# zixunh/vipe

Hardware: AMD Instinct MI355X
Metric: dense-BA+flow update iters/s, 512x384 48-KF graph (higher is better)
Workload: dtype f16 (correlation, GRU; fp32 accumulate) + f32 geometry/BA (fp64 reduced system)

## Files before the change

include/vipe_amd.h:

```cpp
#ifndef VIPE_AMD_H
#define VIPE_AMD_H

#include <stdint.h>

#ifdef __cplusplus
extern "C" {
#endif

#define VIPE_F16 0
#define VIPE_F32 1
#define VIPE_F64 2
#define VIPE_U8 3

#define VIPE_OK 0
#define VIPE_EINVAL (-1)
#define VIPE_ENOSPACE (-2)
#define VIPE_EUNSUPPORTED (-3)

#define VIPE_PYRAMID_REFERENCE 0
#define VIPE_PYRAMID_BLOCKED 1

#define VIPE_CAM_PINHOLE 0
#define VIPE_CAM_MEI 1

// ... 80 lines not shown
int vipe_lie_adjT_backward(int group_id, const void* grad, const void* X, const void* a, void* dX, void* da,
                           int64_t n, int dtype, int on_device, void* stream);
int vipe_lie_act_backward(int group_id, const void* grad, const void* X, const void* p, void* dX, void* dp,
                          int64_t n, int dtype, int on_device, void* stream);
int vipe_lie_act4_backward(int group_id, const void* grad, const void* X, const void* p, void* dX, void* dp,
                           int64_t n, int dtype, int on_device, void* stream);


int vipe_reproject(const float* d_poses, const float* d_disps, const float* d_intrinsics, const float* d_rig,
                   const int64_t* d_pi, const int64_t* d_qi, const int64_t* d_pj, const int64_t* d_qj,
                   const int64_t* d_di, float* d_coords, float* d_valid, int M, int ht, int wd, int n_views,
                   int camera, float intr_factor, void* stream);

int vipe_reproject_motion(const float* d_poses, const float* d_disps, const float* d_intrinsics, const float* d_rig,
                          const int64_t* d_pi, const int64_t* d_qi, const int64_t* d_pj, const int64_t* d_qj,
                          const int64_t* d_di, const float* d_target, float* d_coords, void* d_motn, int M, int ht,
                          int wd, int n_views, int camera, float intr_factor, int motn_dtype, void* stream);
int vipe_reproject_motion_nhwc(const float* d_poses, const float* d_disps, const float* d_intrinsics,
                               const float* d_rig, const int64_t* d_pi, const int64_t* d_qi, const int64_t* d_pj,
                               const int64_t* d_qj, const int64_t* d_di, const float* d_target, float* d_coords,
                               void* d_motn, int M, int ht, int wd, int n_views, int camera, float intr_factor,
                               void* stream);

typedef int (*vipe_overlap_fn)(void* user, int piece, int n_pieces, void* stream);

typedef struct {
  int n_poses;
  int n_views;
  int ht, wd;
  int M;
  int t0, t1;
  int n_iters;
  float pose_damping, pose_ep;
  int motion_only;
  int limited_disp;
  int optimize_intrinsics;
  int optimize_rig_rotation;
  int camera;
  float alpha;
  float weight_scale;
  float intr_factor;
  int reuse_plan;
  int path_hint;
  void* overlap_stream;
  vipe_overlap_fn overlap_fn;
  void* overlap_user;
  int solver_options;
  void* profile_ev0;
  void* profile_ev1;
  int profile_iter;
} vipe_ba_params;
#define VIPE_BA_OPT_ONE_CHAIN 1
#define VIPE_BA_OPT_GENERAL_ACCUMULATE 2

int64_t vipe_dense_ba_workspace_bytes(const vipe_ba_params* p);
int vipe_dense_ba(const vipe_ba_params* p, float* d_poses, float* d_disps, const float* d_disps_sens,
                  float* d_intrinsics, float* d_rig, const float* d_target, const float* d_weight,
                  const float* d_disp_damping, const int64_t* d_pi, const int64_t* d_qi, const int64_t* d_pj,
                  const int64_t* d_qj, const int64_t* d_di, void* d_workspace, int64_t workspace_bytes,
                  int* d_info, void* stream);

int vipe_dense_ba_linearize(const vipe_ba_params* p, const float* d_poses, const float* d_disps, const float* d_disps_sens,
                            const float* d_intrinsics, const float* d_rig, const float* d_target, const float* d_weight,
                            const float* d_disp_damping, const int64_t* d_pi, const int64_t* d_qi, const int64_t* d_pj,
                            const int64_t* d_qj, const int64_t* d_di, void* d_workspace, int64_t workspace_bytes,
                            double* d_S_out, int ld_out, int* d_info, void* stream);
int vipe_dense_ba_marginals(const vipe_ba_params* p, void* d_workspace, const double* d_Sinv, int ld, float* d_disp_var,
                            double* d_pose_cov, void* stream);

int64_t vipe_ba_workspace_bytes(int n_poses, int ht, int wd, int E);
int vipe_ba(float* d_poses, float* d_disps, const float* d_intrinsics, const float* d_disps_sens,
            const float* d_targets, const float* d_weights, const float* d_eta, const int64_t* d_ii,
            const int64_t* d_jj, int n_poses, int ht, int wd, int E, int n_eta, int t0, int t1, int iterations,
            float lm, float ep, int motion_only, float* d_dx, float* d_dz, void* d_workspace,
            int64_t workspace_bytes, void* stream);

int vipe_frame_distance(const float* d_poses, const float* d_disps, const float* d_intrinsics, const int64_t* d_pi,
                        const int64_t* d_pj, const int64_t* d_qi, const int64_t* d_qj, const int64_t* d_di,
                        float* d_dist, int M, int ht, int wd, float beta, void* stream);

int vipe_frame_distance_rig(const float* d_poses, const float* d_rig, const float* d_disps, const float* d_intrinsics,
                            int intr_dim, float intr_factor, const int64_t* d_pi, const int64_t* d_qi, const int64_t* d_pj,
                            const int64_t* d_qj, float* d_dist, int M, int n_views, int ht, int wd, float beta,
                            int bidirectional, void* stream);

int vipe_depth_filter(const float* d_poses, const float* d_disps, const float* d_intrinsics, const int64_t* d_inds,
                      const float* d_thresh, float* d_counter, int n, int num, int ht, int wd, void* stream);

int vipe_projmap(const float* d_poses, const float* d_disps, const float* d_intrinsics, const int64_t* d_ii,
                 const int64_t* d_jj, float* d_coords, float* d_valid, int E, int ht, int wd, void* stream);

int vipe_iproj(const float* d_poses, const float* d_disps, const float* d_intrinsics, float* d_points, int n, int ht,
               int wd, void* stream);

int vipe_scatter(const void* d_src, const int64_t* d_index, void* d_out, int64_t* d_arg_out, int64_t outer,
                 int64_t src_dim, int64_t inner, int64_t out_dim, int reduce, int dtype, void* stream);
int vipe_scatter_rows(const void* d_src, const int64_t* d_index, void* d_out, int64_t* d_arg_out, int64_t outer,
                      int64_t src_dim, int64_t inner, int64_t out_dim, int reduce, int dtype, void* stream);

int vipe_scatter_host(const void* h_src, const int64_t* h_index, void* h_out, int64_t* h_arg_out, int64_t outer,
                      int64_t src_dim, int64_t inner, int64_t out_dim, int reduce, int dtype);

int vipe_scatter_mean_rows_f16(const void* d_src, const int64_t* d_ix, void* d_out, int E, int n_out, int64_t inner,
                               void* stream);

int vipe_segment_mean_nhwc_f16(const void* d_src, int src_ctot, int src_coff, const int* d_order, const int* d_rowptr,
// ... 25 lines not shown
                                 void* d_grad_value, void* d_grad_sampling_loc, void* d_grad_attn_weight, int64_t bs,
                                 int64_t Lv, int heads, int C, int L, int64_t Lq, int P, int dtype, void* stream);

#define VIPE_ACT_NONE 0
#define VIPE_ACT_RELU 1
#define VIPE_ACT_SIGMOID 2
#define VIPE_ACT_TANH 3
int vipe_conv_pack_weights(const void* d_w_oihw, void* d_w_packed, int Cout, int Cin, int KH, int KW, int src_dtype,
                           void* stream);
int vipe_conv2d_nhwc_f16(const void* d_x, const void* d_w_packed, const float* d_bias, const float* d_extra,
                         void* d_y, int B, int H, int W, int Cin, int cin_total, int cin_off, int Cout,
                         int cout_total, int cout_off, int KH, int KW, int act, void* stream);

int vipe_conv_packed_dims(int Cout, int Cin, int KH, int KW, int* cout_pad, int* cin_pad, int* k_pad);

#define VIPE_CONV_PARTIAL 6
#define VIPE_CONV_ACCINIT_F32 0x100
int vipe_conv2d_fused(const void* d_x0, int x0_ctot, int x0_coff, const void* d_x1, int x1_ctot, int x1_coff,
                      int split, const void* d_w_packed, const float* d_bias, const float* d_extra, int extra_stride,
                      int extra_off, void* d_y, int y_ctot, int y_coff, void* d_y2, int y2_ctot, int y2_coff,
                      const void* d_net, int net_ctot, int net_coff, const void* d_z, float* d_fout,
                      const void* d_accinit, int ai_ctot, int ai_coff, int B, int H, int W, int Cin, int Cout, int KH,
                      int KW, int act, int mode, void* stream);

typedef struct {
  const void *corr0_w, *corr2_w, *flow0_w, *flow2_w, *gw_w, *zr_w, *q_w, *zr_s_w, *q_s_w, *heads0_w, *heads2_w, *agg2_w, *eta_w;
  const void *zr_n_w, *zr_x_w;
  const float *corr0_b, *corr2_b, *flow0_b, *flow2_b, *gw_b, *zr_b, *q_b, *heads0_b, *heads2_b, *agg2_b, *eta_b;
  const float* glo_wT;
  const float* glo_b;
} vipe_update_weights;
typedef struct {
  int E, H, W, n_src;
  const void* levels[4];
  const float* coords;
  const int* slots;
  int h2, w2, pyramid_layout;
  const void* corr;
  const void* motn;
  const void* net;
  void* net_out;
  void* xbuf;
  const void* pgate;
  void *c1, *f1, *zb, *rnet;
  void* hbuf;
  float* dw;
  float *glo, *extra;
  const int *order, *rowptr;
  void *agg, *a2;
  float* eta;
  void* side_stream;
  float* pzr;
  int gate_state;
} vipe_update_buffers;
int vipe_update_operator(const vipe_update_weights* weights, const vipe_update_buffers* buffers, void* stream);

int vipe_update_gate_state(const vipe_update_weights* weights, const vipe_update_buffers* buffers, const void* d_net,
                           int parts, void* stream);
typedef struct {
  const vipe_update_weights* weights;
  const vipe_update_buffers* buffers;
  const void* net;
  const int* bounds;
  int n_bounds;
} vipe_gate_state_job;
int vipe_update_gate_state_piece(void* user, int piece, int n_pieces, void* stream);

int vipe_glo_context(const float* d_glo_sum, const float* d_wT, const float* d_bias, float* d_extra, int E, int hw,
                     void* stream);

typedef struct {
  const void* src;
  void* dst;
  const int64_t* idx;
  int64_t src_row_pitch, dst_row_pitch;
  int64_t seg_bytes, seg_pitch;
  int n_seg;
  int n_rows;
  int dst_row0;
} vipe_rows_job;
int vipe_rows_gather(const vipe_rows_job* jobs, int n_jobs, void* stream);
typedef struct {
  const void* src;
  const int64_t* frame;
  void* dst;
  int64_t dst_row_pitch;
  int dst_ctot, dst_coff;
  int dst_row0;
} vipe_nhwc_job;
int vipe_gather_nchw_to_nhwc_f16(const vipe_nhwc_job* jobs, int n_jobs, int n_rows, int C, int P, void* stream);

int vipe_flow_score(const float* d_dw, const unsigned char* d_invalid, float* d_score, int n_views, int P, void* stream);

int vipe_update_finish(const float* d_coords1, const float* d_dw, const unsigned char* d_mask, float* d_target,
                       float* d_weight, const float* d_eta, const int64_t* d_du, float* d_damping, int E, int n_src, int ht,
                       int wd, void* stream);

int vipe_enc_prep(const float* d_img, void* d_x4, int V, int H, int W, void* stream);
int vipe_enc_stem(const void* d_x4, const void* d_w, const float* d_bias, void* d_y, float* d_out_stats, int B, int H,
                  int W, int relu, void* stream);
int vipe_enc_conv(const void* d_x, const float* d_in_stats, const void* d_w, const float* d_bias, const void* d_res,
                  void* d_y, float* d_out_stats, int B, int H, int W, int Cin, int Cout, int ksize, int stride,
                  int relu, int nchw, int tanh_split, void* stream);
int vipe_enc_finish(const void* d_raw, const float* d_raw_stats, const void* d_res, const float* d_res_stats,
                    void* d_out, int B, int HW, int C, void* stream);

// ... 12 lines not shown
```

vipe_amd/csrc/ba.hip:

```cpp
#include <stdlib.h>

#include "term_geom.cuh"

namespace {

#include "ba_common.cuh"
#include "ba_plan.inc"
#include "ba_accumulate.inc"
#include "ba_solve_band.inc"
#include "ba_solve_dense.inc"
#include "ba_solve_global.inc"
#include "ba_retract.inc"
#include "ba_marginals.inc"

hipEvent_t overlap_event() {
  static thread_local hipEvent_t ev[64] = {};
  int d = 0;
  (void)hipGetDevice(&d);
  hipEvent_t& e = ev[d & 63];
  if (!e && hipEventCreateWithFlags(&e, hipEventDisableTiming) != hipSuccess) e = nullptr;
  return e;
}

int overlap_piece(const vipe_ba_params& p, hipEvent_t ev, int piece, int n_pieces, bool gated) {
// ... 2 lines not shown
  return p.overlap_fn(p.overlap_user, piece, n_pieces, p.overlap_stream);
}

template <int CAM, int F>
void launch_accumulate(const BAArgs& a, hipStream_t s) {
  const int tiles = (a.P + TILE - 1) / TILE;
  static std::atomic<uint64_t> tmpl_set{0};
  vipe_once_per_device(tmpl_set, [] {
    (void)hipFuncSetAttribute((const void*)ba_accum_mfma_kernel<CAM, F>, hipFuncAttributeMaxDynamicSharedMemorySize, (int)accum_mfma_lds());
    (void)hipFuncSetAttribute((const void*)ba_walk_kernel<CAM, F>, hipFuncAttributeMaxDynamicSharedMemorySize, (int)walk_lds());
    (void)hipFuncSetAttribute((const void*)ba_walk_rig_kernel<CAM, 4>, hipFuncAttributeMaxDynamicSharedMemorySize, (int)walk_rig_lds());
    (void)hipFuncSetAttribute((const void*)ba_walk_rig_kernel<CAM, RG_VMAX>, hipFuncAttributeMaxDynamicSharedMemorySize, (int)walk_rig_lds());
  });
  if (a.mv) {
    if (a.p.n_views <= 4) ba_walk_rig_kernel<CAM, 4><<<dim3(tiles, a.nF), TILE, walk_rig_lds(), s>>>(a);
    else ba_walk_rig_kernel<CAM, RG_VMAX><<<dim3(tiles, a.nF), TILE, walk_rig_lds(), s>>>(a);
    ba_schur_kernel<0><<<dim3(SC_GRID, a.nF), TILE, 0, s>>>(a);
    return;
  }
  const int hint = a.force_general ? 0 : a.p.path_hint;
  if (!(hint & 2)) ba_accum_mfma_kernel<CAM, F><<<dim3(tiles, a.nF), TILE, accum_mfma_lds(), s>>>(a);
  if (!(hint & 1)) {
    ba_walk_kernel<CAM, F><<<dim3(tiles, a.nF), TILE, walk_lds(), s>>>(a);
    ba_schur_kernel<F><<<dim3(SC_GRID, a.nF), TILE, 0, s>>>(a);
  }
}

template <int CAM, int F>
int run_iters(const BAArgs& a, hipStream_t s, int* pieces_done) {
  const int tiles = (a.P + TILE - 1) / TILE;
  const size_t sbytes = sizeof(double) * (size_t)a.w.ld * a.w.ld;
  const size_t nmax = (size_t)a.w.ld - 1;
  const size_t fixed = ((sizeof(SolveLds) + 15) / 16) * 16;
  int panel_cap = (int)std::min<size_t>(nmax + 1, (150 * 1024 - fixed) / (NB * sizeof(double)));
  panel_cap = (panel_cap + 3) & ~3;
  const size_t solve_lds = fixed + (size_t)NB * panel_cap * sizeof(double);
  const size_t band_lds = 158 * 1024;
  static std::atomic<uint64_t> attr_set{0};
  vipe_once_per_device(attr_set, [] {
    (void)hipFuncSetAttribute((const void*)ba_solve_band_kernel, hipFuncAttributeMaxDynamicSharedMemorySize, 160 * 1024);
    (void)hipFuncSetAttribute((const void*)ba_solve_kernel, hipFuncAttributeMaxDynamicSharedMemorySize, 160 * 1024);
    (void)hipFuncSetAttribute((const void*)ba_solve_dense_kernel, hipFuncAttributeMaxDynamicSharedMemorySize, 160 * 1024);
    (void)hipFuncSetAttribute((const void*)chol_backsub_kernel, hipFuncAttributeMaxDynamicSharedMemorySize, 64 * 1024);
  });
  const bool retract_clears = !a.p.motion_only;
  const bool overlap = a.p.overlap_stream && a.p.overlap_fn;
  hipEvent_t ev = overlap ? overlap_event() : nullptr;
  for (int it = 0; it < a.p.n_iters; ++it) {
    if (!(retract_clears && (it > 0 || a.p.reuse_plan))) {
      hipError_t e1 = hipMemsetAsync(a.w.S, 0, sbytes, s);
      hipError_t e2 = hipMemsetAsync(a.w.Hd, 0, sizeof(double) * nmax, s);
      if (e1 != hipSuccess || e2 != hipSuccess) return (int)(e1 != hipSuccess ? e1 : e2);
    }
    if (a.mv) {
      launch_accumulate<CAM, F>(a, s);
      if (ev && hipEventRecord(ev, s) != hipSuccess) return VIPE_EINVAL;
      ba_solve_kernel<<<1, SOLVE_T, solve_lds, s>>>(a, panel_cap);
      launch_tiled_cholesky(a, s);
      if (overlap) {
        const int rc = overlap_piece(a.p, ev, it, a.p.n_iters, true);
        if (rc != VIPE_OK) return rc;
        ++*pieces_done;
      }
      if (!a.p.motion_only) ba_retract_kernel<0><<<dim3(tiles, a.nF), TILE, 0, s>>>(a);
      continue;
    }
    const int hint = a.force_general ? 0 : a.p.path_hint;
    const bool prof = a.p.profile_ev0 && a.p.profile_ev1 &&
                      it == (a.p.profile_iter < 0 || a.p.profile_iter >= a.p.n_iters ? a.p.n_iters - 1 : a.p.profile_iter);
    if (prof && hipEventRecord((hipEvent_t)a.p.profile_ev0, s) != hipSuccess) return VIPE_EINVAL;
    launch_accumulate<CAM, F>(a, s);
    if (prof && hipEventRecord((hipEvent_t)a.p.profile_ev1, s) != hipSuccess) return VIPE_EINVAL;
    if (ev && hipEventRecord(ev, s) != hipSuccess) return VIPE_EINVAL;
    if (!(hint & 8)) ba_solve_band_kernel<<<1, 2 * BAND_T, band_lds, s>>>(a, (int)(band_lds / sizeof(double)));
    if (!(hint & 16)) ba_solve_dense_kernel<<<1, DN_T, band_lds, s>>>(a, (int)(band_lds / sizeof(double)));
    if (!(hint & 4)) {
      ba_solve_kernel<<<1, SOLVE_T, solve_lds, s>>>(a, panel_cap);
      launch_tiled_cholesky(a, s);
    }
    if (overlap) {
      const int rc = overlap_piece(a.p, ev, it, a.p.n_iters, true);
      if (rc != VIPE_OK) return rc;
      ++*pieces_done;
    }
    if (!a.p.motion_only) ba_retract_kernel<F><<<dim3(tiles, a.nF), TILE, 0, s>>>(a);
  }
  return vipe_launch_status();
}

BAArgs live_args(const vipe_ba_params& p) {
  BAArgs a = {};
  a.p = p;
  a.P = p.ht * p.wd;
  a.nF = p.n_poses * p.n_views;
  a.D = p.camera == VIPE_CAM_MEI ? 1 : 0;
  a.mv = is_multiview(p) ? 1 : 0;
  a.nintr = tail_intr(p);
  a.ntail = a.nintr + tail_rig(p);
  a.force_general = (p.solver_options & VIPE_BA_OPT_GENERAL_ACCUMULATE) != 0;
  a.band2 = !(p.solver_options & VIPE_BA_OPT_ONE_CHAIN);
  a.droid = 0;
  a.dz_out = nullptr;
  return a;
}

}

VIPE_EXPORT int64_t vipe_dense_ba_workspace_bytes(const vipe_ba_params* p) {
  if (!p || p->n_poses <= 0 || p->n_views <= 0 || p->ht <= 0 || p->wd <= 0 || p->M < 0) return VIPE_EINVAL;
  return (int64_t)carve(*p, nullptr, nullptr);
}

VIPE_EXPORT int vipe_dense_ba(const vipe_ba_params* p, float* d_poses, float* d_disps, const float* d_disps_sens,
                              float* d_intrinsics, float* d_rig, const float* d_target, const float* d_weight,
                              const float* d_disp_damping, const int64_t* d_pi, const int64_t* d_qi,
                              const int64_t* d_pj, const int64_t* d_qj, const int64_t* d_di, void* d_workspace,
                              int64_t workspace_bytes, int* d_info, void* stream) {
  VIPE_CHECK_ARG(p && d_poses && d_disps && d_disps_sens && d_intrinsics && d_rig && d_disp_damping && d_workspace);
  VIPE_CHECK_ARG(p->n_poses > 0 && p->n_views > 0 && p->ht > 0 && p->wd > 0 && p->M >= 0 && p->n_iters >= 0);
  VIPE_CHECK_ARG(p->t0 <= p->t1 && p->intr_factor > 0);
  VIPE_CHECK_ARG(p->camera == VIPE_CAM_PINHOLE || p->camera == VIPE_CAM_MEI);
  VIPE_CHECK_ARG(p->M == 0 || (d_target && d_weight && d_pi && d_qi && d_pj && d_qj && d_di));
  if (is_multiview(*p) && p->n_views > RG_VMAX) return VIPE_EUNSUPPORTED;
  if ((int64_t)p->n_poses * p->n_views > 65535) return VIPE_EINVAL;
  BAArgs a = live_args(*p);
  if ((int64_t)carve(*p, (char*)d_workspace, &a.w) > workspace_bytes) return VIPE_ENOSPACE;
  a.poses = d_poses; a.disps = d_disps; a.intr = d_intrinsics; a.rig = d_rig;
  a.sens = d_disps_sens; a.target = d_target; a.weight = d_weight; a.eta = d_disp_damping;
  a.pi = d_pi; a.qi = d_qi; a.pj = d_pj; a.qj = d_qj; a.di = d_di;
  hipStream_t s = as_stream(stream);
  int rc = VIPE_OK, pieces_done = 0;
  if (p->M > 0 && p->n_iters > 0) {
    ba_sens_kernel<<<a.nF, 256, 0, s>>>(d_disps_sens, a.w.sens_sum, a.P, a.w.info);
    if (!p->reuse_plan) ba_plan_kernel<<<1, 1024, 0, s>>>(a);
    const int F = p->optimize_intrinsics ? 1 + a.D : 0;
    if (p->camera == VIPE_CAM_PINHOLE) rc = F ? run_iters<VIPE_CAM_PINHOLE, 1>(a, s, &pieces_done) : run_iters<VIPE_CAM_PINHOLE, 0>(a, s, &pieces_done);
    else rc = F ? run_iters<VIPE_CAM_MEI, 2>(a, s, &pieces_done) : run_iters<VIPE_CAM_MEI, 0>(a, s, &pieces_done);
    if (rc != VIPE_OK) return rc;
    if (d_info) {
      hipError_t e = hipMemcpyAsync(d_info, a.w.info, 8 * sizeof(int), hipMemcpyDeviceToDevice, s);
      if (e != hipSuccess) return (int)e;
    }
  }
  if (p->overlap_stream && p->overlap_fn) {
    const int n_pieces = p->n_iters > 0 ? p->n_iters : 1;
    for (; pieces_done < n_pieces; ++pieces_done) {
      rc = overlap_piece(*p, nullptr, pieces_done, n_pieces, false);
      if (rc != VIPE_OK) return rc;
    }
  }
  const int64_t nd = (int64_t)a.nF * a.P;
  clamp_min_kernel<<<(int)std::min<int64_t>((nd + 255) / 256, 2048), 256, 0, s>>>(d_disps, nd, 1e-3f);
  return vipe_launch_status();
}

VIPE_EXPORT int vipe_dense_ba_linearize(const vipe_ba_params* p, const float* d_poses, const float* d_disps,
                                        const float* d_disps_sens, const float* d_intrinsics, const float* d_rig,
                                        const float* d_target, const float* d_weight, const float* d_disp_damping,
                                        const int64_t* d_pi, const int64_t* d_qi, const int64_t* d_pj, const int64_t* d_qj,
                                        const int64_t* d_di, void* d_workspace, int64_t workspace_bytes, double* d_S_out,
                                        int ld_out, int* d_info, void* stream) {
  VIPE_CHECK_ARG(p && d_poses && d_disps && d_disps_sens && d_intrinsics && d_rig && d_disp_damping && d_workspace && d_S_out);
  VIPE_CHECK_ARG(p->n_poses > 0 && p->n_views > 0 && p->ht > 0 && p->wd > 0 && p->M >= 0);
  VIPE_CHECK_ARG(p->t0 <= p->t1 && p->intr_factor > 0);
  VIPE_CHECK_ARG(p->camera == VIPE_CAM_PINHOLE || p->camera == VIPE_CAM_MEI);
  VIPE_CHECK_ARG(p->M == 0 || (d_target && d_weight && d_pi && d_qi && d_pj && d_qj && d_di));
  if (is_multiview(*p) && p->n_views > RG_VMAX) return VIPE_EUNSUPPORTED;
  if ((int64_t)p->n_poses * p->n_views > 65535) return VIPE_EINVAL;
  BAArgs a = live_args(*p);
  if ((int64_t)carve(*p, (char*)d_workspace, &a.w) > workspace_bytes) return VIPE_ENOSPACE;
  VIPE_CHECK_ARG(ld_out >= 6 * p->n_poses + a.ntail);
  a.poses = const_cast<float*>(d_poses); a.disps = const_cast<float*>(d_disps);
  a.intr = const_cast<float*>(d_intrinsics); a.rig = const_cast<float*>(d_rig);
  a.sens = d_disps_sens; a.target = d_target; a.weight = d_weight; a.eta = d_disp_damping;
  a.pi = d_pi; a.qi = d_qi; a.pj = d_pj; a.qj = d_qj; a.di = d_di;
  hipStream_t s = as_stream(stream);
  ba_sens_kernel<<<a.nF, 256, 0, s>>>(d_disps_sens, a.w.sens_sum, a.P, a.w.info);
  if (!(p->reuse_plan && p->M > 0)) ba_plan_kernel<<<1, 1024, 0, s>>>(a);
  if (!(p->reuse_plan && !p->motion_only && p->M > 0)) {
    hipError_t e1 = hipMemsetAsync(a.w.S, 0, sizeof(double) * (size_t)a.w.ld * a.w.ld, s);
    hipError_t e2 = hipMemsetAsync(a.w.Hd, 0, sizeof(double) * ((size_t)a.w.ld - 1), s);
    if (e1 != hipSuccess || e2 != hipSuccess) return (int)(e1 != hipSuccess ? e1 : e2);
  }
  if (p->M > 0) {
    ba_term_slot_kernel<<<(p->M + 255) / 256, 256, 0, s>>>(a);
    const int F = p->optimize_intrinsics ? 1 + a.D : 0;
    if (p->camera == VIPE_CAM_PINHOLE) F ? launch_accumulate<VIPE_CAM_PINHOLE, 1>(a, s) : launch_accumulate<VIPE_CAM_PINHOLE, 0>(a, s);
    else F ? launch_accumulate<VIPE_CAM_MEI, 2>(a, s) : launch_accumulate<VIPE_CAM_MEI, 0>(a, s);
  }
  const int64_t nn = (int64_t)(a.w.ld - 1) * (a.w.ld - 1);
  ba_export_reduced_kernel<<<(int)std::min<int64_t>((nn + 255) / 256, 2048), 256, 0, s>>>(a, d_S_out, ld_out);
  if (d_info) {
    hipError_t e = hipMemcpyAsync(d_info, a.w.info, 8 * sizeof(int), hipMemcpyDeviceToDevice, s);
    if (e != hipSuccess) return (int)e;
  }
  return vipe_launch_status();
}

VIPE_EXPORT int vipe_dense_ba_marginals(const vipe_ba_params* p, void* d_workspace, const double* d_Sinv, int ld,
                                        float* d_disp_var, double* d_pose_cov, void* stream) {
  VIPE_CHECK_ARG(p && d_workspace);
  VIPE_CHECK_ARG(p->n_poses > 0 && p->n_views > 0 && p->ht > 0 && p->wd > 0 && p->M >= 0 && ld >= 0);
  VIPE_CHECK_ARG(p->camera == VIPE_CAM_PINHOLE || p->camera == VIPE_CAM_MEI);
  if (is_multiview(*p) && p->n_views > RG_VMAX) return VIPE_EUNSUPPORTED;
  if ((int64_t)p->n_poses * p->n_views > 65535) return VIPE_EINVAL;
  BAArgs a = live_args(*p);
  carve(*p, (char*)d_workspace, &a.w);
  hipStream_t s = as_stream(stream);
  const int tiles = (a.P + TILE - 1) / TILE;
  if (p->M > 0 && !p->motion_only && d_disp_var) {
    VIPE_CHECK_ARG(d_Sinv || ld == 0);
    ba_disp_variance_kernel<<<dim3(tiles, a.nF), TILE, 0, s>>>(a, d_Sinv, ld, d_disp_var);
  }
  const int64_t ns = (int64_t)a.w.ld * a.w.ld;
  ba_marginals_finish_kernel<<<(int)std::min<int64_t>((ns + 255) / 256, 2048), 256, 0, s>>>(a, ld > 0 ? d_Sinv : nullptr, ld, d_pose_cov);
  return vipe_launch_status();
}

namespace {
size_t droid_extra_bytes(int E) { return align_up(8 * (size_t)(E + 1)) + align_up(7 * 4); }
vipe_ba_params droid_params(int n_poses, int ht, int wd, int E, int t0, int t1, int iterations, float lm, float ep,
                            int motion_only) {
  vipe_ba_params p = {};
  p.n_poses = n_poses; p.n_views = 1; p.ht = ht; p.wd = wd; p.M = E; p.t0 = t0; p.t1 = t1; p.n_iters = iterations;
  p.pose_damping = lm; p.pose_ep = ep; p.motion_only = motion_only; p.limited_disp = 0; p.optimize_intrinsics = 0;
  p.optimize_rig_rotation = 0; p.camera = VIPE_CAM_PINHOLE; p.alpha = 0.05f; p.weight_scale = 0.001f; p.intr_factor = 1.0f;
  p.reuse_plan = 0; p.path_hint = 0;
  return p;
}
}

VIPE_EXPORT int64_t vipe_ba_workspace_bytes(int n_poses, int ht, int wd, int E) {
  if (n_poses <= 0 || ht <= 0 || wd <= 0 || E < 0) return VIPE_EINVAL;
  const vipe_ba_params p = droid_params(n_poses, ht, wd, E, 0, 0, 0, 0.f, 0.f, 0);
  return (int64_t)(carve(p, nullptr, nullptr) + droid_extra_bytes(E));
}

VIPE_EXPORT int vipe_ba(float* d_poses, float* d_disps, const float* d_intrinsics, const float* d_disps_sens,
                        const float* d_targets, const float* d_weights, const float* d_eta, const int64_t* d_ii,
                        const int64_t* d_jj, int n_poses, int ht, int wd, int E, int n_eta, int t0, int t1,
                        int iterations, float lm, float ep, int motion_only, float* d_dx, float* d_dz,
                        void* d_workspace, int64_t workspace_bytes, void* stream) {
  VIPE_CHECK_ARG(d_poses && d_disps && d_intrinsics && d_disps_sens && d_eta && d_workspace && d_dx && d_dz);
  VIPE_CHECK_ARG(n_poses > 0 && ht > 0 && wd > 0 && E >= 0 && iterations >= 0 && n_eta >= 0);
  VIPE_CHECK_ARG(0 <= t0 && t0 <= t1 && t1 <= n_poses);
  VIPE_CHECK_ARG(E == 0 || (d_targets && d_weights && d_ii && d_jj));
  if (n_poses > 65535) return VIPE_EINVAL;
  BAArgs a;
  a.p = droid_params(n_poses, ht, wd, E, t0, t1, iterations, lm, ep, motion_only);
  const size_t base = carve(a.p, (char*)d_workspace, &a.w);
  if ((int64_t)(base + droid_extra_bytes(E)) > workspace_bytes) return VIPE_ENOSPACE;
  int64_t* zeros = (int64_t*)((char*)d_workspace + base);
  float* rig = (float*)((char*)d_workspace + base + align_up(8 * (size_t)(E + 1)));
  hipStream_t s = as_stream(stream);
  const float rig_id[7] = {0, 0, 0, 0, 0, 0, 1};
  hipError_t e0 = hipMemsetAsync(zeros, 0, 8 * (size_t)(E + 1), s);
  hipError_t e1 = hipMemcpyAsync(rig, rig_id, sizeof(rig_id), hipMemcpyHostToDevice, s);
  const int64_t P = (int64_t)ht * wd;
  hipError_t e2 = hipMemsetAsync(d_dx, 0, sizeof(float) * 6 * (size_t)(t1 - t0), s);
  hipError_t e3 = hipMemsetAsync(d_dz, 0, sizeof(float) * (size_t)n_eta * P, s);
  if (e0 != hipSuccess || e1 != hipSuccess || e2 != hipSuccess || e3 != hipSuccess) return VIPE_EINVAL;
  a.poses = d_poses; a.disps = d_disps; a.intr = (float*)d_intrinsics; a.rig = rig;
  a.sens = d_disps_sens; a.target = d_targets; a.weight = d_weights; a.eta = d_eta;
  a.pi = d_ii; a.qi = zeros; a.pj = d_jj; a.qj = zeros; a.di = d_ii;
  a.P = ht * wd; a.nF = n_poses; a.D = 0;
  a.mv = 0; a.nintr = 0; a.ntail = 0;
  a.force_general = 0;
  a.band2 = 1;
  a.droid = 1;
  a.dz_out = d_dz;
  if (iterations == 0 || t1 == t0) return VIPE_OK;
  ba_sens_kernel<<<a.nF, 256, 0, s>>>(d_disps_sens, a.w.sens_sum, a.P, a.w.info);
  ba_plan_kernel<<<1, 1024, 0, s>>>(a);
  int pieces_done = 0;
  const int rc = run_iters<VIPE_CAM_PINHOLE, 0>(a, s, &pieces_done);
  if (rc != VIPE_OK) return rc;
  hipError_t e4 = hipMemcpyAsync(d_dx, a.w.dx, sizeof(float) * 6 * (size_t)(t1 - t0), hipMemcpyDeviceToDevice, s);
  return e4 == hipSuccess ? vipe_launch_status() : (int)e4;
}
```

vipe_amd/csrc/ba_accumulate.inc:

```
constexpr int AM_ROWS = 48;
constexpr int AM_P1 = 130;
constexpr int AM_P2 = 66;
constexpr int AM_P2H = 34;
constexpr int AM_WBUF = 16 * AM_P1;
static_assert(AM_ROWS * AM_P2H <= AM_WBUF, "R2 half image must fit the wave buffer");
constexpr int AM_SP = AM_ROWS + 1;

struct TermGeomM {
  TermGeom g;
  float Mi[36];
};

constexpr size_t accum_mfma_lds() {
  return sizeof(float) * (NWAVE * AM_WBUF + AM_ROWS * AM_SP + AM_DMAX * 256 + 64) + AM_DMAX * sizeof(TermGeomM);
}

typedef float float4m __attribute__((ext_vector_type(4)));


__device__ __forceinline__ void term_setup_m(const BAArgs& a, int e, TermGeomM& m) {
  TermGeom& g = m.g;
  term_setup(a, e, g);
#pragma unroll
  for (int c = 0; c < 6; ++c) {
// ... 221 lines not shown
        atomicAdd(&accI[42 + q * FF + f], hif);
      }
    } else if (F > 0 && lane < 42 + 6 * F + F * F) {
      const int i2 = lane - 42 - 6 * F, f = i2 / FF, f2 = i2 % FF;
      if (f >= f2) atomicAdd(&accI[42 + 6 * FF + f * FF + f2], Gm[(7 + f) * 16 + 7 + f2]);
    } else if (F > 0 && lane < 42 + 6 * F + F * F + F) {
      const int f = lane - 42 - 6 * F - F * F;
      atomicAdd(&accI[42 + 6 * FF + FF * FF + f], -Gm[(7 + f) * 16 + 6]);
    }
    __builtin_amdgcn_fence(__ATOMIC_RELEASE, "wavefront");
    __builtin_amdgcn_wave_barrier();
    if (fi && lane < 36) {
      const int r = lane / 6, c = lane % 6;
      float hii = 0.f;
#pragma unroll
      for (int q = 0; q < 6; ++q) hii += T1[r * 8 + q] * Mi[c * 6 + q];
      atomicAdd(&accI[r * 6 + c], hii);
    }
    __builtin_amdgcn_wave_barrier();
  }
}

template <int F>
__device__ __forceinline__ void flush_frame_blocks(const BAWs& w, const float* accI, int si, int nrow, int foff) {
  constexpr int FF = F > 0 ? F : 1;
  const int tid = threadIdx.x;
  const bool fi = si >= 0;
  const int bi = 6 * si;
  if (tid < 36) {
    const int r = tid / 6, c = tid % 6;
    if (fi && r >= c) {
      const double s = (double)accI[r * 6 + c];
      s_add(w, bi + r, bi + c, s);
      if (r == c) atomicAdd(&w.Hd[bi + r], s);
    }
  } else if (tid < 42) {
    if (fi) atomicAdd(&w.S[(int64_t)nrow * w.ld + bi + (tid - 36)], (double)accI[tid]);
  } else if (F > 0 && tid < 42 + 6 * F) {
    const int q = (tid - 42) / FF, f = (tid - 42) % FF;
    if (fi) s_add(w, foff + f, bi + q, (double)accI[tid]);
  } else if (F > 0 && tid < 42 + 6 * F + F * F) {
    const int i2 = tid - 42 - 6 * F, f = i2 / FF, f2 = i2 % FF;
    if (f >= f2) {
      const double s = (double)accI[tid];
      s_add(w, foff + f, foff + f2, s);
      if (f == f2) atomicAdd(&w.Hd[foff + f], s);
    }
  } else if (F > 0 && tid < 42 + 6 * F + F * F + F) {
    atomicAdd(&w.S[(int64_t)nrow * w.ld + foff + (tid - 42 - 6 * F - F * F)], (double)accI[tid]);
  }
}

template <int NF, int F>
__device__ __forceinline__ void store_disp_block(const BAArgs& a, int k, int flags, WalkPixel<F>& px) {
  static_assert(NF <= WalkPixel<F>::FF, "E_f rows come from px.Efr");
  const BAWs& w = a.w;
  const int P = a.P, p = px.p;
  const int64_t kp = (int64_t)k * P + p;
  finish_disp(a, k, p, P, flags, px.d, px.C, px.wz);
  if (px.inb) {
    w.C[kp] = px.C;
    w.wv[kp] = px.wz;
#pragma unroll
    for (int q = 0; q < 6; ++q) w.Ekk[((int64_t)k * 6 + q) * P + p] = px.Ei[q];
#pragma unroll
    for (int f = 0; f < NF; ++f) w.Ef[((int64_t)k * 2 + f) * P + p] = px.Efr[f];
  }
}

template <int CAM, int F>
__global__ __launch_bounds__(TILE) __attribute__((amdgpu_waves_per_eu(3, 3))) void ba_accum_mfma_kernel(BAArgs a) {
  const vipe_ba_params& prm = a.p;
  const BAWs& w = a.w;
  if (a.force_general || w.info[6] > AM_DMAX) return;
  const int k = blockIdx.y;
  const int beg = w.rowptr[k], end = w.rowptr[k + 1];
  if (beg == end) return;
  const int deg = end - beg;
  const int P = a.P, V = prm.n_views, tid = threadIdx.x, lane = tid & 63, wave = tid >> 6;
  const int flags = w.fflags[k];
  const bool dfree = flags & 2;
  const int pose_i = k / V, qi = k % V;
  const int si = w.pose_slot[pose_i];
  const bool fi = si >= 0;
  const int n_free = w.info[0], nrow = w.info[3];
  const int foff = 6 * n_free;

  extern __shared__ __align__(16) float am_smem[];
  float* wbuf = am_smem + wave * AM_WBUF;
  float* accS = am_smem + NWAVE * AM_WBUF;
  float* acc1 = accS + AM_ROWS * AM_SP;
  float* accI = acc1 + AM_DMAX * 256;
  TermGeomM* tg = reinterpret_cast<TermGeomM*>(accI + 64);

  for (int i = tid; i < AM_ROWS * AM_SP + AM_DMAX * 256 + 64; i += TILE) accS[i] = 0.0f;
  if (tid < deg) {
    TermGeomM m;
    term_setup_m(a, w.order[beg + tid], m);
    tg[tid] = m;
  }
  __syncthreads();

  WalkPixel<F> px = walk_pixel<CAM, F>(a, k, qi);
  const int l16 = lane & 15, kq = lane >> 4;
  walk_tile<CAM, F>(a, tg, deg, dfree, wbuf, acc1, px);

  const int NR = 6 * (deg + 1) + F + 1;
  if (dfree) {
    store_disp_block<F>(a, k, flags, px);
    const float sq = px.inb ? __builtin_amdgcn_rsqf(px.C) : 0.0f;
    float ej[AM_DMAX][6];
#pragma unroll
    for (int t = 0; t < AM_DMAX; ++t) {
      const bool on = t < deg && tg[min(t, deg - 1)].g.sj >= 0 && px.inb;
      const int64_t eb = (int64_t)tg[min(t, deg - 1)].g.e * 6 * P + px.p;
#pragma unroll
      for (int q = 0; q < 6; ++q) ej[t][q] = on ? w.Ej[eb + (int64_t)q * P] : 0.0f;
    }
    constexpr int NPAIR = 6;
    float4m g4[NPAIR];
#pragma unroll
    for (int i = 0; i < NPAIR; ++i) g4[i] = float4m{0.f, 0.f, 0.f, 0.f};
    const int RT = (NR + 15) >> 4;
#pragma unroll
    for (int half = 0; half < 2; ++half) {
      if ((lane >> 5) == half) {
        float* col = wbuf + (lane & 31);
#pragma unroll
        for (int q = 0; q < 6; ++q) col[q * AM_P2H] = fi ? px.Ei[q] * sq : 0.0f;
#pragma unroll
        for (int t = 0; t < AM_DMAX; ++t) {
          if (t < deg) {
#pragma unroll
            for (int q = 0; q < 6; ++q) col[(6 * (t + 1) + q) * AM_P2H] = ej[t][q] * sq;
          }
        }
        if constexpr (F > 0) {
#pragma unroll
          for (int f = 0; f < F; ++f) col[(6 * (deg + 1) + f) * AM_P2H] = px.Efr[f] * sq;
        }
        col[(NR - 1) * AM_P2H] = px.wz * sq;
        for (int r = NR; r < ((NR + 15) & ~15); ++r) col[r * AM_P2H] = 0.0f;
      }
      __builtin_amdgcn_fence(__ATOMIC_RELEASE, "wavefront");
      __builtin_amdgcn_wave_barrier();
#pragma unroll
      for (int ta = 0; ta < 3; ++ta)
#pragma unroll
        for (int tb = 0; tb <= ta; ++tb) {
          if (ta < RT) {
            const float* ar = wbuf + (16 * ta + l16) * AM_P2H + kq;
            const float* br = wbuf + (16 * tb + l16) * AM_P2H + kq;
            float4m acc = g4[ta * (ta + 1) / 2 + tb];
#pragma unroll
            for (int s = 0; s < 8; ++s) acc = __builtin_amdgcn_mfma_f32_16x16x4f32(ar[4 * s], br[4 * s], acc, 0, 0, 0);
            g4[ta * (ta + 1) / 2 + tb] = acc;
          }
        }
      __builtin_amdgcn_fence(__ATOMIC_RELEASE, "wavefront");
      __builtin_amdgcn_wave_barrier();
    }
#pragma unroll
    for (int ta = 0; ta < 3; ++ta)
#pragma unroll
      for (int tb = 0; tb <= ta; ++tb) {
        if (ta < RT) {
#pragma unroll
          for (int r = 0; r < 4; ++r) {
            const int row = 16 * ta + 4 * kq + r, cc = 16 * tb + l16;
            if (row < NR && cc <= row) atomicAdd(&accS[row * AM_SP + cc], g4[ta * (ta + 1) / 2 + tb][r]);
          }
        }
      }
  }
  __syncthreads();

  flush_term_blocks<F>(w, tg, deg, acc1, accI, wbuf, si, nrow, foff);
  __syncthreads();

  flush_frame_blocks<F>(w, accI, si, nrow, foff);
  if (dfree) {
    auto gmap = [&](int row) -> int {
      if (row >= 6 * (deg + 1)) return foff + (row - 6 * (deg + 1));
      const int m = row / 6, q = row % 6;
      const int sl = m == 0 ? si : tg[m - 1].g.sj;
      return sl >= 0 ? 6 * sl + q : -1;
    };
    for (int i = tid; i < NR * NR; i += TILE) {
      const int row = i / NR, cc = i % NR;
      if (cc > row || cc == NR - 1) continue;
      const int gc = gmap(cc);
      if (gc < 0) continue;
      const float val = accS[row * AM_SP + cc];
      if (row == NR - 1) {
        atomicAdd(&w.S[(int64_t)nrow * w.ld + gc], -(double)val);
      } else {
        const int gr = gmap(row);
        if (gr >= 0) s_add(w, gr, gc, (gr == gc && row != cc) ? -2.0 * (double)val : -(double)val);
      }
    }
  }
}

constexpr int WK_CH = 8;
constexpr int WK_CH1 = 12;
constexpr size_t walk_lds() {
  return sizeof(float) * (NWAVE * 16 * AM_P1 + WK_CH1 * 256 + 64) + WK_CH1 * sizeof(TermGeomM);
}

template <int CAM, int F>
__global__ __launch_bounds__(TILE) void ba_walk_kernel(BAArgs a) {
  constexpr int WBUF = 16 * AM_P1;
  const vipe_ba_params& prm = a.p;
  const BAWs& w = a.w;
  if (!a.force_general && w.info[6] <= AM_DMAX) return;
  const int k = blockIdx.y;
  const int beg = w.rowptr[k], end = w.rowptr[k + 1];
  if (beg == end) return;
  const int deg_all = end - beg;
  const int V = prm.n_views, tid = threadIdx.x, wave = tid >> 6;
  const int flags = w.fflags[k];
  const bool dfree = flags & 2;
  const int pose_i = k / V, qi = k % V;
  const int si = w.pose_slot[pose_i];
  const int n_free = w.info[0], nrow = w.info[3];
  const int foff = 6 * n_free;

  extern __shared__ __align__(16) float am_smem[];
  float* wbuf = am_smem + wave * WBUF;
  float* acc1 = am_smem + NWAVE * WBUF;
  float* accI = acc1 + WK_CH1 * 256;
  TermGeomM* tg = reinterpret_cast<TermGeomM*>(accI + 64);
  if (tid < 64) accI[tid] = 0.0f;

  WalkPixel<F> px = walk_pixel<CAM, F>(a, k, qi);

  for (int cb = 0; cb < deg_all; cb += WK_CH1) {
    const int deg = min(WK_CH1, deg_all - cb);
    __syncthreads();
    for (int i = tid; i < WK_CH1 * 256; i += TILE) acc1[i] = 0.0f;
    if (tid < deg) {
      TermGeomM m;
      term_setup_m(a, w.order[beg + cb + tid], m);
      tg[tid] = m;
    }
    __syncthreads();

    walk_tile<CAM, F>(a, tg, deg, dfree, wbuf, acc1, px);

    __syncthreads();
    flush_term_blocks<F>(w, tg, deg, acc1, accI, wbuf, si, nrow, foff);

  }
  __syncthreads();

  flush_frame_blocks<F>(w, accI, si, nrow, foff);
  if (dfree) store_disp_block<F>(a, k, flags, px);
}

constexpr int RG_NB = 10;
constexpr int RG_NL = 28;
struct TermGeomR {
  TermGeom g;
  int qj, same_view;
  int gcol[RG_NL];
  float Lm[RG_NL][RG_NB];
};
constexpr size_t walk_rig_lds() {
  return sizeof(float) * (NWAVE * 16 * AM_P1 + WK_CH * 256) + WK_CH * sizeof(TermGeomR);
}
__device__ __forceinline__ int rg_tile_row(int b) { return b < 6 ? b : b + 1; }

template <int CAM, int VM>
__global__ __launch_bounds__(TILE) void ba_walk_rig_kernel(BAArgs a) {
  constexpr int WBUF = 16 * AM_P1;
  constexpr int F = CAM == VIPE_CAM_MEI ? 2 : 1;
  const vipe_ba_params& prm = a.p;
  const BAWs& w = a.w;
  const int k = blockIdx.y;
  const int beg = w.rowptr[k], end = w.rowptr[k + 1];
  if (beg == end) return;
  const int deg_all = end - beg;
  const int P = a.P, V = prm.n_views, tid = threadIdx.x, lane = tid & 63, wave = tid >> 6;
  const int flags = w.fflags[k];
  const bool dfree = flags & 2;
  const int pose_i = k / V, qi = k % V;
  const int si = w.pose_slot[pose_i];
  const int n_free = w.info[0], nrow = w.info[3];
  const int foff = 6 * n_free, roff = foff + a.nintr;
  const bool oi = prm.optimize_intrinsics, orr = prm.optimize_rig_rotation;

  extern __shared__ __align__(16) float am_smem[];
  float* wbuf = am_smem + wave * WBUF;
  float* acc1 = am_smem + NWAVE * WBUF;
  TermGeomR* tg = reinterpret_cast<TermGeomR*>(acc1 + WK_CH * 256);

  WalkPixel<F> px = walk_pixel<CAM, F>(a, k, qi);
  const int p = px.p;
  const bool inb = px.inb;
  float ErA[6] = {0, 0, 0, 0, 0, 0};
  float Efv[VM][F] = {}, Erv[VM][6] = {};
  const int l16 = lane & 15, kq = lane >> 4;

  for (int cb = 0; cb < deg_all; cb += WK_CH) {
    const int deg = min(WK_CH, deg_all - cb);
    __syncthreads();
    for (int i = tid; i < WK_CH * 256; i += TILE) acc1[i] = 0.0f;
    if (tid < deg) {
      TermGeomR& m = tg[tid];
      const int e = w.order[beg + cb + tid];
      const int pi = (int)a.pi[e], pj = (int)a.pj[e], qj = (int)a.qj[e];
      term_transforms(a.poses, a.rig, pi, qi, pj, qj, m.g.T, m.g.G, m.g.Rr);
      m.g.Ij = cam::load_scaled(a.intr + qj * (4 + a.D), a.D, 1.0f / prm.intr_factor);
      m.g.e = e;
      m.g.merge = (pi == pj);
      m.g.rig_adj = !(m.g.Rr.t[0] == 0.f && m.g.Rr.t[1] == 0.f && m.g.Rr.t[2] == 0.f && m.g.Rr.R[0] == 1.f &&
                      m.g.Rr.R[4] == 1.f && m.g.Rr.R[8] == 1.f);
      m.g.sj = m.g.merge ? -1 : w.pose_slot[pj];
      m.qj = qj;
      m.same_view = (qj == qi);
      const int sjj = w.pose_slot[pj];
      for (int c = 0; c < RG_NL; ++c)
        for (int b = 0; b < RG_NB; ++b) m.Lm[c][b] = 0.0f;
      for (int c = 0; c < 6; ++c) {
        float ec[6] = {0, 0, 0, 0, 0, 0}, col[6];
        ec[c] = 1.0f;
        adjT_apply(m.g.G, ec, col);
        for (int r = 0; r < 6; ++r) {
          m.Lm[r][c] = -col[r];
          m.Lm[16 + r][c] = col[r];
        }
        m.Lm[6 + c][c] = 1.0f;
        m.Lm[22 + c][c] = -1.0f;
      }
      for (int f = 0; f < 2; ++f) {
        m.Lm[12 + f][6 + f] = 1.0f;
        m.Lm[14 + f][8 + f] = 1.0f;
      }
      for (int q = 0; q < 6; ++q) {
        m.gcol[q] = si >= 0 ? 6 * si + q : -1;
        m.gcol[6 + q] = sjj >= 0 ? 6 * sjj + q : -1;
        m.gcol[16 + q] = (orr && qi >= 1) ? roff + 6 * (qi - 1) + q : -1;
        m.gcol[22 + q] = (orr && qj >= 1) ? roff + 6 * (qj - 1) + q : -1;
      }
      for (int f = 0; f < 2; ++f) {
        m.gcol[12 + f] = (oi && f < F) ? foff + qi * F + f : -1;
        m.gcol[14 + f] = (oi && f < F && qj != qi) ? foff + qj * F + f : -1;
      }
    }
// ... 54 lines not shown
#pragma unroll
              for (int f = 0; f < F; ++f) Efv[vv][f] += JfB[f] * wJz;
#pragma unroll
              for (int q = 0; q < 6; ++q) Erv[vv][q] -= Jj[q] * wJz;
            }
          }
        }
      }
      if (dfree && G.sj >= 0 && inb) {
#pragma unroll
        for (int q = 0; q < 6; ++q) w.Ej[((int64_t)e * 6 + q) * P + p] = Ejv[q];
      }
      const float4m g4 = gram_r1(wbuf, l16, kq);
#pragma unroll
      for (int r = 0; r < 4; ++r) atomicAdd(&acc1[t * 256 + (4 * kq + r) * 16 + l16], g4[r]);
      __builtin_amdgcn_wave_barrier();
    }

    __syncthreads();
    for (int t = wave; t < deg; t += NWAVE) {
      const TermGeomR& TG = tg[t];
      const float* Gm = acc1 + t * 256;
      float* T1 = wbuf;
      for (int i = lane; i < RG_NL * RG_NB; i += 64) {
        const int c = i / RG_NB, b = i % RG_NB;
        float acc = 0.f;
#pragma unroll
        for (int b2 = 0; b2 < RG_NB; ++b2) acc += TG.Lm[c][b2] * Gm[rg_tile_row(b2) * 16 + rg_tile_row(b)];
        T1[i] = acc;
      }
      if (lane < RG_NL && TG.gcol[lane] >= 0) {
        float acc = 0.f;
#pragma unroll
        for (int b2 = 0; b2 < RG_NB; ++b2) acc += TG.Lm[lane][b2] * Gm[rg_tile_row(b2) * 16 + 6];
        atomicAdd(&w.S[(int64_t)nrow * w.ld + TG.gcol[lane]], -(double)acc);
      }
      __builtin_amdgcn_fence(__ATOMIC_RELEASE, "wavefront");
      __builtin_amdgcn_wave_barrier();
      for (int i = lane; i < RG_NL * RG_NL; i += 64) {
        const int ca = i / RG_NL, cb2 = i % RG_NL;
        const int ga = TG.gcol[ca], gb = TG.gcol[cb2];
        if (ga < 0 || gb < 0 || ga < gb) continue;
        float acc = 0.f;
#pragma unroll
        for (int b = 0; b < RG_NB; ++b) acc += T1[ca * RG_NB + b] * TG.Lm[cb2][b];
        atomicAdd(&w.S[(int64_t)ga * w.ld + gb], (double)acc);
        if (ga == gb) atomicAdd(&w.Hd[ga], (double)acc);
      }
      __builtin_amdgcn_wave_barrier();
    }
  }

  if (dfree) {
    store_disp_block<0>(a, k, flags, px);
    if (inb) {
      float* et = w.Et + (int64_t)k * a.ntail * P + p;
      if (oi) {
#pragma unroll
        for (int vv = 0; vv < VM; ++vv) {
          if (vv < V) {
#pragma unroll
            for (int f = 0; f < F; ++f) et[(int64_t)(vv * F + f) * P] = Efv[vv][f] + (vv == qi ? px.Efr[f] : 0.0f);
          }
        }
      }
      if (orr) {
#pragma unroll
        for (int vv = 1; vv < VM; ++vv) {
          if (vv < V) {
#pragma unroll
            for (int q = 0; q < 6; ++q)
              et[(int64_t)(a.nintr + 6 * (vv - 1) + q) * P] = Erv[vv][q] + (vv == qi ? ErA[q] : 0.0f);
          }
        }
      }
    }
  }
}

constexpr int SC_GRID = 96;

template <int F>
__global__ __launch_bounds__(TILE) void ba_schur_kernel(BAArgs a) {
  const BAWs& w = a.w;
  if (!a.mv && !a.force_general && w.info[6] <= AM_DMAX) return;
  const int k = blockIdx.y;
  const int flags = w.fflags[k];
  const int beg = w.rowptr[k], end = w.rowptr[k + 1];
  if (!(flags & 2) || beg == end) return;
  const int deg = end - beg, P = a.P, V = a.p.n_views;
  const int NT = a.mv ? a.ntail : F;
  const int NR = 6 * (deg + 1) + NT + 1, RT = (NR + 15) >> 4, npairs = RT * (RT + 1) / 2;
  const int tid = threadIdx.x, lane = tid & 63, wave = tid >> 6, l16 = lane & 15, kq = lane >> 4;
  const int si = w.pose_slot[k / V];
  const int n_free = w.info[0], nrow = w.info[3], foff = 6 * n_free;
  __shared__ float tile[NWAVE][2][16 * AM_P2];
  __shared__ float red[NWAVE][256];
  __shared__ const float* rowp[32];
  __shared__ float rowm[32];
  __shared__ int rowg[32];
  auto resolve = [&](int r, const float*& ptr, int& g) {
    ptr = nullptr; g = -1;
    if (r >= NR) return;
    if (r == NR - 1) { ptr = w.wv + (int64_t)k * P; g = -2; return; }
    if (r >= 6 * (deg + 1)) {
      const int f = r - 6 * (deg + 1);
      ptr = a.mv ? w.Et + ((int64_t)k * NT + f) * P : w.Ef + ((int64_t)k * 2 + f) * P;
// ... 81 lines not shown
```

vipe_amd/csrc/ba_common.cuh:

```cuda

constexpr int TILE = 256;
constexpr int NWAVE = TILE / WAVE;
constexpr int TCHUNK = 8;
constexpr int AM_DMAX = 6;

struct BAWs {
  int* rowptr;
  int* order;
  int* pose_slot;
  int* slot_pose;
  int* fflags;
  int* scratch;
  int* info;
  float* sens_sum;
  float* C;
  float* wv;
  float* Ekk;
  float* Ef;
  float* Et;
  float* Ej;
  double* S;
  double* Hd;
  float* dx;
  double* Wi;
  int* krow;
  int* mslot;
  int ld;
};

struct BAArgs {
  vipe_ba_params p;
  float *poses, *disps, *intr, *rig;
  const float *sens, *target, *weight, *eta;
  const int64_t *pi, *qi, *pj, *qj, *di;
  BAWs w;
  int P, nF, D;
  int mv, nintr, ntail;
  int force_general;
  int band2;
  int droid;
  float* dz_out;
};

inline size_t align_up(size_t x, size_t a = 256) { return (x + a - 1) / a * a; }

constexpr int RG_VMAX = 8;
inline bool is_multiview(const vipe_ba_params& p) { return p.n_views > 1; }
inline int tail_intr(const vipe_ba_params& p) {
  const int F = 1 + (p.camera == VIPE_CAM_MEI ? 1 : 0);
  return p.optimize_intrinsics ? (is_multiview(p) ? p.n_views * F : F) : 0;
}
inline int tail_rig(const vipe_ba_params& p) { return p.optimize_rig_rotation ? 6 * (p.n_views - 1) : 0; }

size_t carve(const vipe_ba_params& p, char* base, BAWs* out) {
  const size_t nP = p.n_poses, nF = (size_t)p.n_poses * p.n_views, P = (size_t)p.ht * p.wd, M = p.M;
  const size_t ntail_max = is_multiview(p) ? (size_t)p.n_views * 2 + 6 * (size_t)(p.n_views - 1) : 2;
  const size_t nmax = 6 * nP + ntail_max;
  size_t off = 0;
  auto take = [&](size_t bytes) {
    char* ptr = base ? base + off : nullptr;
    off += align_up(bytes);
    return ptr;
  };
  BAWs w;
  w.rowptr = (int*)take(4 * (nF + 1));
  w.order = (int*)take(4 * (M + 1));
  w.pose_slot = (int*)take(4 * nP);
  w.slot_pose = (int*)take(4 * nP);
  w.fflags = (int*)take(4 * nF);
  w.scratch = (int*)take(4 * (2 * nP + nF));
  w.info = (int*)take(4 * 8);
  w.sens_sum = (float*)take(4 * nF);
  w.C = (float*)take(4 * nF * P);
  w.wv = (float*)take(4 * nF * P);
  w.Ekk = (float*)take(4 * nF * 6 * P);
  w.Ef = (float*)take(4 * nF * 2 * P);
  w.Et = (float*)take(is_multiview(p) ? 4 * nF * ntail_max * P : 0);
  w.Ej = (float*)take(4 * (M + 1) * 6 * P);
  w.S = (double*)take(8 * (nmax + 1) * (nmax + 1));
  w.Hd = (double*)take(8 * (nmax + 16));
  w.dx = (float*)take(4 * nmax);
  w.Wi = (double*)take(8 * 64 * 64 * ((nmax + 63) / 64));
  w.krow = (int*)take(4 * (nF + 1));
  w.mslot = (int*)take(4 * (M + 1));
  w.ld = (int)(nmax + 1);
  if (out) *out = w;
  return off;
}

__device__ __forceinline__ void load_tw(const BAArgs& a, int e, int p, int P, float2& tgt, float2& wg) {
  if (a.droid) {
    const int64_t o = (int64_t)e * 2 * P + p;
    tgt = make_float2(a.target[o], a.target[o + P]);
    wg = make_float2(a.weight[o], a.weight[o + P]);
  } else {
    const int64_t o2 = ((int64_t)e * P + p) * 2;
    tgt = *reinterpret_cast<const float2*>(a.target + o2);
    wg = *reinterpret_cast<const float2*>(a.weight + o2);
  }
}
__device__ __forceinline__ float valid_weight(const BAArgs& a, float Z, bool inb) {
  const bool ok = a.droid ? !(Z < 0.25f) : (Z > cam::MIN_DEPTH);
  return (inb && ok) ? a.p.weight_scale : 0.0f;
}
__device__ __forceinline__ void term_setup(const BAArgs& a, int e, TermGeom& g) {
  const int pi = (int)a.pi[e], pj = (int)a.pj[e], qj = (int)a.qj[e];
  term_transforms(a.poses, a.rig, pi, (int)a.qi[e], pj, qj, g.T, g.G, g.Rr);
  g.Ij = cam::load_scaled(a.intr + qj * (4 + a.D), a.D, 1.0f / a.p.intr_factor);
  g.e = e;
  g.merge = (pi == pj);
  if (a.droid && pi == pj) {
    g.merge = 2;
    for (int i = 0; i < 9; ++i) g.T.R[i] = g.G.R[i] = (i % 4 == 0) ? 1.0f : 0.0f;
    g.T.t[0] = g.G.t[0] = -0.1f;
    g.T.t[1] = g.T.t[2] = g.G.t[1] = g.G.t[2] = 0.0f;
  }
  g.rig_adj = !(g.Rr.t[0] == 0.f && g.Rr.t[1] == 0.f && g.Rr.t[2] == 0.f && g.Rr.R[0] == 1.f &&
                g.Rr.R[4] == 1.f && g.Rr.R[8] == 1.f);
  g.sj = g.merge ? -1 : a.w.pose_slot[pj];
}
__device__ __forceinline__ void finish_disp(const BAArgs& a, int k, int p, int P, int flags, float d, float& C, float& wz) {
  const int64_t kp = (int64_t)k * P + p;
  if (a.droid) {
    const float sv = a.sens[kp];
    if (sv > 0.0f) { C += a.p.alpha; wz -= a.p.alpha * (d - sv); }
    else C += a.eta[(int64_t)a.w.krow[k] * P + p];
  } else {
    if (a.w.sens_sum[k] > 0.0f) {
      C += a.p.alpha;
      wz -= a.p.alpha * (d - a.sens[kp]);
    }
    C += 1e-7f + (0.2f * a.eta[kp] + 1e-7f);
  }
}

__device__ __forceinline__ void s_add(const BAWs& w, int row, int col, double v) {
  if (row < col) { int tmp = row; row = col; col = tmp; }
  atomicAdd(&w.S[(int64_t)row * w.ld + col], v);
}

__device__ __forceinline__ double rsqrt_nr(double x) {
  double r = __builtin_amdgcn_rsq(x);
  const double hx = 0.5 * x;
  r = r * __builtin_fma(-hx * r, r, 1.5);
  r = r * __builtin_fma(-hx * r, r, 1.5);
  return r;
}


__device__ __forceinline__ double readlane_f64(double v, int lane) {
  const unsigned long long u = __builtin_bit_cast(unsigned long long, v);
  const unsigned lo = (unsigned)__builtin_amdgcn_readlane((int)u, lane);
  const unsigned hi = (unsigned)__builtin_amdgcn_readlane((int)(u >> 32), lane);
  return __builtin_bit_cast(double, ((unsigned long long)hi << 32) | lo);
}

__device__ __forceinline__ void tri_index(int q, int& i, int& j) {
  i = (int)((sqrtf(8.0f * (float)q + 1.0f) - 1.0f) * 0.5f);
  while ((i + 1) * (i + 2) / 2 <= q) ++i;
  while (i * (i + 1) / 2 > q) --i;
  j = q - i * (i + 1) / 2;
}

__device__ __forceinline__ double damped_diag(const BAArgs& a, int r, int npr, double v, double hd) {
  const bool pose = r < npr, rigrow = a.mv && r >= npr + a.nintr;
  const double ep = pose ? (double)a.p.pose_ep : (rigrow ? 1e-4 : 1e-6);
  const double lam = pose ? (double)a.p.pose_damping : (rigrow ? 1e-4 : 1e-6);
  return v + (ep + lam * (a.droid ? v : hd));
}

__device__ __forceinline__ void store_step(const BAWs& w, int dd, double x, bool bad) {
  if (bad || !(x == x)) x = 0.0;
  w.dx[dd] = (float)x;
}

__device__ __forceinline__ void apply_retraction(const BAArgs& a, int t, int nthreads, int n_free) {
  const BAWs& w = a.w;
  for (int sl = t; sl < n_free; sl += nthreads) {
    const int pidx = w.slot_pose[sl];
    float xi[6];
    for (int q = 0; q < 6; ++q) xi[q] = w.dx[6 * sl + q];
    lie::SE3<float> X(a.poses + 7 * pidx);
    (lie::SE3<float>::exp(xi) * X).store(a.poses + 7 * pidx);
  }
  if (a.mv) {
    const int F = 1 + a.D, V = a.p.n_views;
// ... 22 lines not shown
```

vipe_amd/csrc/ba_plan.inc:

```

__global__ __launch_bounds__(256) void ba_sens_kernel(const float* __restrict__ sens, float* __restrict__ out, int P,
                                                      int* __restrict__ info) {
  const int k = blockIdx.x;
  if (k == 0 && threadIdx.x == 0) {
    info[2] = 0;
    info[5] = 0;
  }
  float s = 0.f;
  for (int p = threadIdx.x; p < P; p += blockDim.x) s += sens[(int64_t)k * P + p];
  s = wave_sum(s);
  __shared__ float red[NWAVE];
  if (lane_id() == 0) red[wave_id()] = s;
  __syncthreads();
  if (threadIdx.x == 0) out[k] = red[0] + red[1] + red[2] + red[3];
}

__device__ int block_scan_excl(int* v, int n, int* lds ) {
  const int t = threadIdx.x;
  const int per = (n + 1023) / 1024;
  const int b = t * per;
  int s = 0;
  for (int i = b; i < b + per && i < n; ++i) s += v[i];
  lds[t] = s;
  __syncthreads();
  for (int o = 1; o < 1024; o <<= 1) {
    int x = t >= o ? lds[t - o] : 0;
    __syncthreads();
    lds[t] += x;
    __syncthreads();
  }
  int run = t > 0 ? lds[t - 1] : 0;
  const int total = lds[1023];
  for (int i = b; i < b + per && i < n; ++i) {
    int c = v[i];
    v[i] = run;
    run += c;
  }
  __syncthreads();
  return total;
}

__global__ __launch_bounds__(1024) void ba_plan_kernel(BAArgs a) {
  const vipe_ba_params& p = a.p;
  const int t = threadIdx.x;
  const int nP = p.n_poses, nF = a.nF, M = p.M, V = p.n_views;
  int* cnt = a.w.scratch;
  int* is_src = cnt + nF;
  int* used = is_src + nP;
  __shared__ int lds[1024];
  __shared__ int stage[4096];
  for (int i = t; i < nF; i += 1024) cnt[i] = 0;
  for (int i = t; i < nP; i += 1024) { is_src[i] = 0; used[i] = 0; }
  __syncthreads();
  for (int e = t; e < M; e += 1024) {
    atomicAdd(&cnt[(int)a.di[e]], 1);
    is_src[(int)a.pi[e]] = 1;
    used[(int)a.pi[e]] = 1;
    used[(int)a.pj[e]] = 1;
  }
  __syncthreads();
  const bool all_fixed = !(p.t0 < p.t1);
  int nfd_local = 0;
  for (int k = t; k < nF; k += 1024) {
    const int pose = k / V;
    int f = cnt[k] > 0 ? 1 : 0;
    if (a.droid) {
      const bool inkx = f || (k >= p.t0 && k < p.t1);
// ... 72 lines not shown
```

vipe_amd/csrc/ba_retract.inc:

```

template <int F>
__global__ __launch_bounds__(TILE) void ba_retract_kernel(BAArgs a) {
  const BAWs& w = a.w;
  {
    const int64_t nthr = (int64_t)gridDim.x * gridDim.y * TILE;
    const int64_t gid = ((int64_t)blockIdx.y * gridDim.x + blockIdx.x) * TILE + threadIdx.x;
    const int64_t ns = (int64_t)w.ld * w.ld;
    for (int64_t i = gid; i < ns; i += nthr) w.S[i] = 0.0;
    for (int64_t i = gid; i < (int64_t)w.ld - 1; i += nthr) w.Hd[i] = 0.0;
  }
  const int k = blockIdx.y;
  const int flags = w.fflags[k];
  if (!(flags & 2)) return;
  const int P = a.P, V = a.p.n_views;
  const int p = blockIdx.x * TILE + threadIdx.x;
  if (p >= P) return;
  const int64_t kp = (int64_t)k * P + p;
  if (flags & 8) {
    float C = 0.f, wz = 0.f;
    finish_disp(a, k, p, P, flags, a.disps[kp], C, wz);
    const float dz = wz / C;
    a.disps[kp] += dz;
    if (a.dz_out) a.dz_out[(int64_t)w.krow[k] * P + p] = dz;
    return;
  }
  const int beg = w.rowptr[k], end = w.rowptr[k + 1];
  float rhs = w.wv[kp];
  const int si = w.pose_slot[k / V];
  const int n_free = w.info[0];
  const int smin = a.droid ? 1 : 0;
  if (si >= smin) {
#pragma unroll
    for (int q = 0; q < 6; ++q) rhs -= w.Ekk[((int64_t)k * 6 + q) * P + p] * w.dx[6 * si + q];
  }
  for (int c = beg; c < end; ++c) {
    const int e = w.order[c];
    const int pj = (int)a.pj[e];
    const int sj = ((int)a.pi[e] == pj) ? -1 : w.pose_slot[pj];
    if (sj < smin) continue;
#pragma unroll
    for (int q = 0; q < 6; ++q) rhs -= w.Ej[((int64_t)e * 6 + q) * P + p] * w.dx[6 * sj + q];
  }
  if constexpr (F > 0) {
#pragma unroll
    for (int f = 0; f < F; ++f) rhs -= w.Ef[((int64_t)k * 2 + f) * P + p] * w.dx[6 * n_free + f];
  }
  if (a.mv) {
    for (int f = 0; f < a.ntail; ++f) rhs -= w.Et[((int64_t)k * a.ntail + f) * P + p] * w.dx[6 * n_free + f];
  }
  float dz = rhs / w.C[kp];
  if (!a.droid && dz > 10.0f) dz = 0.0f;
  a.disps[kp] += dz;
  if (a.dz_out) a.dz_out[(int64_t)w.krow[k] * P + p] = dz;
}

__global__ void clamp_min_kernel(float* __restrict__ x, int64_t n, float lo) {
  for (int64_t i = (int64_t)blockIdx.x * blockDim.x + threadIdx.x; i < n; i += (int64_t)gridDim.x * blockDim.x)
    x[i] = fmaxf(x[i], lo);
}
```

vipe_amd/csrc/common.cuh:

```cuda
#pragma once
#include <hip/hip_runtime.h>
#include <hip/hip_fp16.h>
#include <stdint.h>

#include <atomic>
#include <mutex>

#include "../../include/vipe_amd.h"

#define VIPE_EXPORT extern "C" __attribute__((visibility("default")))

#define VIPE_CHECK_ARG(cond) \
  do {                       \
    if (!(cond)) return VIPE_EINVAL; \
  } while (0)

static inline int vipe_launch_status() {
  hipError_t e = hipGetLastError();
  return e == hipSuccess ? VIPE_OK : (int)e;
}

template <typename F>
static inline void vipe_once_per_device(std::atomic<uint64_t>& done, F&& fn) {
  int d = 0;
  (void)hipGetDevice(&d);
  const uint64_t bit = 1ull << (d & 63);
  if (done.load(std::memory_order_acquire) & bit) return;
  static std::mutex mu;
  std::lock_guard<std::mutex> lock(mu);
  if (done.load(std::memory_order_relaxed) & bit) return;
  fn();
  done.fetch_or(bit, std::memory_order_release);
}

static inline hipStream_t as_stream(void* s) { return (hipStream_t)s; }

constexpr int WAVE = 64;

template <typename T>
__device__ __forceinline__ T wave_sum(T v) {
#pragma unroll
  for (int o = 32; o > 0; o >>= 1) v += __shfl_xor(v, o, WAVE);
  return v;
}

__device__ __forceinline__ float wave_sum_to_lane63(float v) {
#define VIPE_DPP_ADD(ctrl, rmask)                                                                          \
  v += __builtin_bit_cast(float, __builtin_amdgcn_update_dpp(0, __builtin_bit_cast(int, v), ctrl, rmask, 0xf, true))
  VIPE_DPP_ADD(0xB1, 0xf);
  VIPE_DPP_ADD(0x4E, 0xf);
  VIPE_DPP_ADD(0x141, 0xf);
  VIPE_DPP_ADD(0x140, 0xf);
  VIPE_DPP_ADD(0x142, 0xa);
  VIPE_DPP_ADD(0x143, 0xc);
#undef VIPE_DPP_ADD
  return v;
}

__device__ __forceinline__ int lane_id() { return threadIdx.x & (WAVE - 1); }
__device__ __forceinline__ int wave_id() { return threadIdx.x >> 6; }

using half_t = _Float16;
__device__ __forceinline__ float h2f(half_t h) { return (float)h; }
__device__ __forceinline__ half_t f2h(float f) { return (half_t)f; }

__device__ __forceinline__ int xcd_remap(int bid, int nwg) {
  const int nx = 8;
  int q = nwg / nx, r = nwg % nx;
  int xcd = bid % nx;
  int base = xcd < r ? xcd * (q + 1) : r * (q + 1) + (xcd - r) * q;
  return base + bid / nx;
}
```

vipe_amd/csrc/conv_epilogue.inc:

```
#pragma unroll
  for (int j = 0; j < TN; ++j) {
    const int64_t m = pix0 + (wn * TN + j) * 32 + lrow;
    const bool mok = m < M;
    const int e = mok ? (int)(m / HW) : 0;
#pragma unroll
    for (int i = 0; i < TM; ++i) {
#pragma unroll
      for (int g = 0; g < 4; ++g) {
        const int co = cout0 + (wm * TM + i) * 32 + 8 * g + 4 * lhalf;
        float v[4];
#pragma unroll
        for (int q = 0; q < 4; ++q) {
          v[q] = acc[i][j][4 * g + q];
          if (co + q < a.Cout) {
            v[q] += a.bias[co + q];
            if (a.extra) v[q] += a.extra[(int64_t)e * a.extra_stride + a.extra_off + co + q];
          }
        }
        if (a.epi == EPI_PLAIN) {
          if (mok && co < a.Cout) {
            half4 o;
#pragma unroll
            for (int q = 0; q < 4; ++q) o[q] = (half_t)act_apply(v[q], a.act);
            if (co + 3 < a.Cout) {
// ... 3 lines not shown
            }
          }
        } else if (a.epi == EPI_GLO) {
          float s4[4] = {0, 0, 0, 0};
          if (mok) {
            const half4 nv = *reinterpret_cast<const half4*>(a.net + m * a.net_ctot + a.net_coff + co);
#pragma unroll
            for (int q = 0; q < 4; ++q) s4[q] = (float)(half_t)act_apply(v[q], VIPE_ACT_SIGMOID) * (float)nv[q];
          }
          const int e_first = (int)(pix0 / HW);
          const int64_t last = (pix0 + BNP - 1 < M ? pix0 + BNP - 1 : M - 1);
          const bool one_image = (int)(last / HW) == e_first;
          if (one_image) {
#pragma unroll
            for (int q = 0; q < 4; ++q) {
              float t = s4[q];
#pragma unroll
              for (int o = 16; o > 0; o >>= 1) t += __shfl_xor(t, o, WAVE);
              if (lrow == 0) atomicAdd(a.fout + (int64_t)e_first * a.Cout + co + q, t);
            }
          } else if (mok) {
#pragma unroll
            for (int q = 0; q < 4; ++q) atomicAdd(a.fout + (int64_t)e * a.Cout + co + q, s4[q]);
          }
        } else if (a.epi == EPI_ZR) {
          if (mok) {
            half4 o;
            if (co < 128) {
#pragma unroll
              for (int q = 0; q < 4; ++q) o[q] = (half_t)act_apply(v[q], VIPE_ACT_SIGMOID);
              *reinterpret_cast<half4*>(a.y + m * a.y_ctot + a.y_coff + co) = o;
            } else {
              const half4 nv = *reinterpret_cast<const half4*>(a.net + m * a.net_ctot + a.net_coff + co - 128);
#pragma unroll
              for (int q = 0; q < 4; ++q)
                o[q] = (half_t)((float)(half_t)act_apply(v[q], VIPE_ACT_SIGMOID) * (float)nv[q]);
              *reinterpret_cast<half4*>(a.y2 + m * a.y2_ctot + a.y2_coff + co - 128) = o;
            }
          }
        } else if (a.epi == EPI_Q) {
          if (mok) {
            const half4 nv = *reinterpret_cast<const half4*>(a.net + m * a.net_ctot + a.net_coff + co);
            const half4 zv = *reinterpret_cast<const half4*>(a.zbuf + m * 128 + co);
            half4 o;
#pragma unroll
            for (int q = 0; q < 4; ++q) {
              const float qq = (float)(half_t)tanhf(v[q]);
              const float z = (float)zv[q];
              o[q] = (half_t)((1.0f - z) * (float)nv[q] + z * qq);
            }
            *reinterpret_cast<half4*>(a.y + m * a.y_ctot + a.y_coff + co) = o;
          }
        } else if (a.epi == EPI_HEADS) {
          if (mok && co == 0) {
            float4 o = make_float4((float)(half_t)v[0], (float)(half_t)v[1],
                                   (float)(half_t)act_apply(v[2], VIPE_ACT_SIGMOID),
                                   (float)(half_t)act_apply(v[3], VIPE_ACT_SIGMOID));
            *reinterpret_cast<float4*>(a.fout + m * 4) = o;
          }
        } else if (a.epi == EPI_ETA) {
          if (mok && co == 0) {
            const float x = v[0];
            const float sp = x > 20.0f ? x : log1pf(__expf(x));
            a.fout[m] = 0.01f * (float)(half_t)sp;
          }
        }
      }
    }
  }
```

vipe_amd/csrc/conv_mfma.hip:

```cpp
#include <stdlib.h>

#include <type_traits>

#include "common.cuh"

namespace {

typedef _Float16 half8 __attribute__((ext_vector_type(8)));
typedef _Float16 half4 __attribute__((ext_vector_type(4)));
typedef float float16v __attribute__((ext_vector_type(16)));
typedef float float4v __attribute__((ext_vector_type(4)));

enum Epi { EPI_PLAIN = 0, EPI_GLO = 1, EPI_ZR = 2, EPI_Q = 3, EPI_HEADS = 4, EPI_ETA = 5, EPI_PARTIAL = 6 };

struct ConvArgs {
  const half_t* x0; int x0_ctot, x0_coff;
  const half_t* x1; int x1_ctot, x1_coff;
  int split;
  const half_t* w;
  const float* bias;
  const float* extra;
  int extra_stride, extra_off;
  half_t* y; int y_ctot, y_coff;
  int B, H, W, Cin, Cin_pad, Cout, Cout_pad, KH, KW, nsteps;
  int act, epi;
  const half_t* net; int net_ctot, net_coff;
  const half_t* zbuf;
  half_t* y2; int y2_ctot, y2_coff;
  float* fout;
  const half_t* accinit; int ai_ctot, ai_coff;
  int ai_f32;
  int f_wp, f_hwp, f_tiles, f_pieces, f_xbytes, f_p1lo, f_p1hi;
  unsigned f_magic;
};

constexpr int BNP = 128;
constexpr int BK = 64;

__device__ __forceinline__ int swz(int row, int k8) { return row * 128 + ((k8 ^ ((row >> 1) & 7)) << 4); }

__device__ __forceinline__ float act_apply(float v, int act) {
  switch (act) {
    case VIPE_ACT_RELU: return fmaxf(v, 0.0f);
    case VIPE_ACT_SIGMOID: return 1.0f / (1.0f + __expf(-v));
    case VIPE_ACT_TANH: return tanhf(v);
    default: return v;
  }
}

template <int BMC, int WAVES_M, int WAVES_N, bool SMALLCIN>
__global__ __launch_bounds__(256) void conv_mfma_kernel(ConvArgs a) {
  constexpr int TM = BMC / (WAVES_M * 32);
  constexpr int TN = BNP / (WAVES_N * 32);
  static_assert(WAVES_M * WAVES_N == 4, "4 waves");
  constexpr int W_ITEMS = BMC * 8 / 256;
  constexpr int X_ITEMS = BNP * 8 / 256;

  extern __shared__ __align__(16) unsigned char lds[];
  unsigned char* ldsW = lds;
  unsigned char* ldsX = lds + 2 * BMC * 128;

  const int tid = threadIdx.x, lane = tid & 63, wave = tid >> 6;
  const int wm = wave / WAVES_N, wn = wave % WAVES_N;
  const int64_t M = (int64_t)a.B * a.H * a.W;
  const int64_t pix0 = (int64_t)blockIdx.x * BNP;
  const int cout0 = blockIdx.y * BMC;
  const int HW = a.H * a.W;

  const int k8 = tid & 7;
  int xe[X_ITEMS], xy[X_ITEMS], xx[X_ITEMS];
  bool xvalid[X_ITEMS];
#pragma unroll
  for (int j = 0; j < X_ITEMS; ++j) {
    const int64_t m = pix0 + (tid >> 3) + 32 * j;
    xvalid[j] = m < M;
    const int64_t mm = xvalid[j] ? m : 0;
    xe[j] = (int)(mm / HW);
    const int rem = (int)(mm % HW);
    xy[j] = rem / a.W;
    xx[j] = rem % a.W;
  }
  const int ph = a.KH / 2, pw = a.KW / 2;
  const int csteps = a.Cin_pad / BK;

  half8 wreg[W_ITEMS], xreg[X_ITEMS];

  auto issue_loads = [&](int s) {
    const half_t* wb = a.w + ((int64_t)s * a.Cout_pad + cout0) * BK;
#pragma unroll
    for (int j = 0; j < W_ITEMS; ++j) {
      const int row = (tid >> 3) + 32 * j;
      wreg[j] = *reinterpret_cast<const half8*>(wb + row * BK + k8 * 8);
    }
    if constexpr (!SMALLCIN) {
      const int tap = s / csteps, c0 = (s % csteps) * BK;
      const int dy = tap / a.KW - ph, dx = tap % a.KW - pw;
      const int c = c0 + k8 * 8;
      const bool cok = c < a.Cin;
      const bool s0 = c < a.split;
// ... 587 lines not shown
#pragma unroll
        for (int q = 0; q < 8; ++q) {
          const float z = (float)zvv[it][q];
          o[q] = (half_t)((1.0f - z) * (float)nvv[it][q] + z * (float)sv[q]);
        }
        dst = a.y + m * a.y_ctot + a.y_coff + co;
      }
      if (dst) {
        if (co + 8 <= a.Cout) {
          *reinterpret_cast<half8*>(dst) = o;
        } else {
          for (int q = 0; q < 8 && co + q < a.Cout; ++q) dst[q] = o[q];
        }
      }
    }
    if (a.epi == EPI_GLO) {
      float* red = reinterpret_cast<float*>(lds);
      __syncthreads();
#pragma unroll
      for (int q = 0; q < 8; ++q) red[(tid / CPP) * (BMC + 1) + ch + q] = gsum[q];
      __syncthreads();
      if (tid < BMC) {
        float t = 0.0f;
        for (int r = 0; r < 512 / CPP; ++r) t += red[r * (BMC + 1) + tid];
        if (cout0 + tid < a.Cout) atomicAdd(a.fout + (int64_t)e * a.Cout + cout0 + tid, t);
      }
    }
  } else {
    constexpr int PITCH = BMC + 4;
    float* stage = reinterpret_cast<float*>(lds);
#pragma unroll
    for (int i = 0; i < MI; ++i)
#pragma unroll
      for (int j = 0; j < NJ; ++j)
        *reinterpret_cast<float4*>(stage + (wn * 64 + pxh + j * 16 + l16) * PITCH + i * 16 + 4 * lk) =
            make_float4(acc16[i][j][0], acc16[i][j][1], acc16[i][j][2], acc16[i][j][3]);
    __syncthreads();
    float bv[8];
#pragma unroll
    for (int q = 0; q < 8; ++q) {
      bv[q] = a.bias[co + q];
      if (a.extra && co + q < a.Cout) bv[q] += a.extra[(int64_t)e * a.extra_stride + a.extra_off + co + q];
    }
#pragma unroll
    for (int it = 0; it < NIT; ++it) {
      const int pl = pl0 + PSTEP * it;
      const int64_t m = pix_of(pl);
      if (FLAT && m < 0) continue;
      const float4 v0 = *reinterpret_cast<const float4*>(stage + pl * PITCH + ch);
      const float4 v1 = *reinterpret_cast<const float4*>(stage + pl * PITCH + ch + 4);
      const float v[8] = {v0.x + bv[0], v0.y + bv[1], v0.z + bv[2], v0.w + bv[3],
                          v1.x + bv[4], v1.y + bv[5], v1.z + bv[6], v1.w + bv[7]};
      if (a.epi == EPI_HEADS) {
        if (ch == 0)
          *reinterpret_cast<float4*>(a.fout + m * 4) =
              make_float4((float)(half_t)v[0], (float)(half_t)v[1], (float)(half_t)act_apply(v[2], VIPE_ACT_SIGMOID),
                          (float)(half_t)act_apply(v[3], VIPE_ACT_SIGMOID));
      } else if (a.epi == EPI_ETA) {
        if (ch == 0) {
          const float sp = v[0] > 20.0f ? v[0] : log1pf(__expf(v[0]));
          a.fout[m] = 0.01f * (float)(half_t)sp;
        }
      } else {
        half_t* dst = a.y + m * a.y_ctot + a.y_coff + co;
        half8 o;
#pragma unroll
        for (int q = 0; q < 8; ++q) o[q] = (half_t)act_apply(v[q], a.act);
        if (co + 8 <= a.Cout) {
          *reinterpret_cast<half8*>(dst) = o;
        } else {
          for (int q = 0; q < 8 && co + q < a.Cout; ++q) dst[q] = o[q];
        }
      }
    }
  }
}

constexpr int NRW_WBYTES = 9 * 1024;

template <bool FLAT>
__global__ __launch_bounds__(512) __attribute__((amdgpu_waves_per_eu(4, 4))) void conv_halo32_narrow_kernel(ConvArgs a) {
  extern __shared__ __align__(16) unsigned char lds[];
  const int tid = threadIdx.x, lane = tid & 63, wave = __builtin_amdgcn_readfirstlane(tid >> 6);
  const int wn = wave & 3, pxh = (wave >> 2) * 32;
  const int tile = xcd_remap(blockIdx.x, gridDim.x);
  const int xsegs = a.W / HALO_TW, tiles_per_img = FLAT ? a.f_tiles : (a.H / HALO_TH) * xsegs;
  const int e = tile / tiles_per_img, trem = tile % tiles_per_img;
  const int y0 = (trem / xsegs) * HALO_TH, x0 = (trem % xsegs) * HALO_TW;
  const int q0 = trem * (HALO_TH * HALO_TW);
  const int pitch = FLAT ? a.f_wp : HALO_PITCH, xbytes = FLAT ? a.f_xbytes : H32_XBYTES;
  const int npieces = FLAT ? a.f_pieces : H32_PIECES;
  auto pix_of = [&](int pl) -> int64_t {
    if constexpr (FLAT) return flat_pixel(q0 + pl, e, a.H, a.W, a.f_wp, a.f_hwp, a.f_magic);
    else return ((int64_t)(e * a.H + y0 + (pl >> 6))) * a.W + x0 + (pl & 63);
  };
  const int cs32 = a.Cin_pad / H32_BK, cs64 = a.Cin_pad / 64;
  const int r16 = lane >> 2, sl = lane & 3, l16 = lane & 15, lk = lane >> 4;
  const unsigned ldsW_a = lds_address(lds), ldsX_a = ldsW_a + 2 * NRW_WBYTES;
  const unsigned char* ldsW = lds;
  const unsigned char* ldsX = lds + 2 * NRW_WBYTES;
  const half_t* zp = reinterpret_cast<const half_t*>(g_zero_page);

  int xpix[H32_XP];
  const int xk = (sl ^ swzf(r16)) * 8;
#pragma unroll
  for (int i = 0; i < H32_XP; ++i) {
    const int pce = wave + 8 * i;
    const int r = pce * 16 + r16;
    if constexpr (FLAT) {
      xpix[i] = pce < npieces ? flat_pixel(q0 - pitch - 1 + r, e, a.H, a.W, a.f_wp, a.f_hwp, a.f_magic) : -1;
    } else {
      const int hy = r / HALO_PITCH, hx = r % HALO_PITCH;
      const int y = y0 + hy - 1, x = x0 + hx - 1;
      const bool ok = pce < H32_PIECES && r < HALO_ROWS && y >= 0 && y < a.H && x >= 0 && x < a.W;
      xpix[i] = ok ? (e * a.H + y) * a.W + x : -1;
// ... 17 lines not shown
    const half_t* wb = a.w + ((int64_t)(wave * cs64 + (c >> 1)) * a.Cout_pad) * BK + (c & 1) * H32_BK;
    glds16_off(wb, woff, ldsW_a + buf * NRW_WBYTES + wave * 1024);
    if (wave == 0) {
      const half_t* w8 = a.w + ((int64_t)(8 * cs64 + (c >> 1)) * a.Cout_pad) * BK + (c & 1) * H32_BK;
      glds16_off(w8, woff, ldsW_a + buf * NRW_WBYTES + 8 * 1024);
    }
  };

  float4v acc[2] = {float4v{0.f, 0.f, 0.f, 0.f}, float4v{0.f, 0.f, 0.f, 0.f}};
  const int wa0 = swz32(l16, lk);
  const int Rl0 = (FLAT ? wn * HALO_TW : wn * HALO_PITCH) + pxh + l16;
  issue(0, 0);
  asm volatile("s_waitcnt vmcnt(0)" ::: "memory");
  __syncthreads();
  for (int c = 0; c < cs32; ++c) {
    if (c + 1 < cs32) issue(c + 1, (c + 1) & 1);
    const unsigned char* bw = ldsW + (c & 1) * NRW_WBYTES;
    const unsigned char* bx = ldsX + (c & 1) * xbytes;
#pragma unroll
    for (int tap = 0; tap < 9; ++tap) {
      const int rb = Rl0 + (tap / 3) * pitch + (tap % 3);
      const int xa0 = swz32(rb, lk);
      const half8 wf = *reinterpret_cast<const half8*>(bw + (wa0 + tap * 1024));
#pragma unroll
      for (int j = 0; j < 2; ++j) {
        const half8 xf = *reinterpret_cast<const half8*>(bx + (xa0 + j * 1024));
        acc[j] = __builtin_amdgcn_mfma_f32_16x16x32_f16(wf, xf, acc[j], 0, 0, 0);
      }
    }
    asm volatile("s_waitcnt vmcnt(0)" ::: "memory");
    __syncthreads();
  }
  constexpr int PITCH = 20;
  float* stage = reinterpret_cast<float*>(lds);
#pragma unroll
  for (int j = 0; j < 2; ++j)
    *reinterpret_cast<float4*>(stage + (wn * 64 + pxh + j * 16 + l16) * PITCH + 4 * lk) =
        make_float4(acc[j][0], acc[j][1], acc[j][2], acc[j][3]);
  __syncthreads();
  const int64_t m = tid < HALO_TH * HALO_TW ? pix_of(tid) : -1;
  if (tid < HALO_TH * HALO_TW && (!FLAT || m >= 0)) {
    float v[16];
#pragma unroll
    for (int q = 0; q < 4; ++q) {
      const float4 t4 = *reinterpret_cast<const float4*>(stage + tid * PITCH + 4 * q);
      v[4 * q] = t4.x; v[4 * q + 1] = t4.y; v[4 * q + 2] = t4.z; v[4 * q + 3] = t4.w;
    }
#pragma unroll
    for (int q = 0; q < 16; ++q) {
      v[q] += a.bias[q];
      if (a.extra && q < a.Cout) v[q] += a.extra[(int64_t)e * a.extra_stride + a.extra_off + q];
    }
    if (a.epi == EPI_HEADS) {
      *reinterpret_cast<float4*>(a.fout + m * 4) =
          make_float4((float)(half_t)v[0], (float)(half_t)v[1], (float)(half_t)act_apply(v[2], VIPE_ACT_SIGMOID),
                      (float)(half_t)act_apply(v[3], VIPE_ACT_SIGMOID));
    } else if (a.epi == EPI_ETA) {
      const float sp = v[0] > 20.0f ? v[0] : log1pf(__expf(v[0]));
      a.fout[m] = 0.01f * (float)(half_t)sp;
    } else {
      half_t* dst = a.y + m * a.y_ctot + a.y_coff;
      for (int q = 0; q < a.Cout; ++q) dst[q] = (half_t)act_apply(v[q], a.act);
    }
  }
}

constexpr int GLO_PITCH = 136;
constexpr size_t GLO_LDS = 256 * GLO_PITCH * 2 + 128 * 4;

__global__ __launch_bounds__(512) __attribute__((amdgpu_waves_per_eu(4, 4))) void conv1x1_glo_kernel(ConvArgs a) {
  extern __shared__ __align__(16) unsigned char lds[];
  half_t* xt = reinterpret_cast<half_t*>(lds);
  float* gacc = reinterpret_cast<float*>(lds + 256 * GLO_PITCH * 2);
  const int tid = threadIdx.x, lane = tid & 63, wave = tid >> 6;
  const int l16 = lane & 15, kg = lane >> 4;
  const int wq = wave & 3, wp = wave >> 2;
  const int HW = a.H * a.W;
  const int tpi = (HW + 255) / 256;
  const int e = blockIdx.x / tpi, p0 = (blockIdx.x % tpi) * 256;
  const int64_t pix0 = (int64_t)e * HW + p0;
  if (tid < 128) gacc[tid] = 0.0f;
#pragma unroll
  for (int it = 0; it < 8; ++it) {
    const int i = tid + 512 * it, px = i >> 4, ck = i & 15;
    half8 v = {0, 0, 0, 0, 0, 0, 0, 0};
    if (p0 + px < HW) v = *reinterpret_cast<const half8*>(a.x0 + (pix0 + px) * a.x0_ctot + a.x0_coff + ck * 8);
    *reinterpret_cast<half8*>(xt + px * GLO_PITCH + ck * 8) = v;
  }
  half8 af[2][4];
#pragma unroll
  for (int i = 0; i < 2; ++i)
#pragma unroll
    for (int s2 = 0; s2 < 4; ++s2) {
      const int k = 32 * s2 + 8 * kg, r = 32 * wq + 16 * i + l16;
      af[i][s2] = *reinterpret_cast<const half8*>(a.w + ((int64_t)(k >> 6) * a.Cout_pad + r) * 64 + (k & 63));
    }
  float4 bv[2];
#pragma unroll
  for (int i = 0; i < 2; ++i) bv[i] = *reinterpret_cast<const float4*>(a.bias + 32 * wq + 16 * i + 4 * kg);
  __syncthreads();
  float gs[2][4] = {{0, 0, 0, 0}, {0, 0, 0, 0}};
#pragma unroll 2
  for (int j = 0; j < 8; ++j) {
    const int pxb = wp * 128 + j * 16 + l16;
    float4v acc[2] = {float4v{0.f, 0.f, 0.f, 0.f}, float4v{0.f, 0.f, 0.f, 0.f}};
#pragma unroll
    for (int s2 = 0; s2 < 4; ++s2) {
      const half8 xf = *reinterpret_cast<const half8*>(xt + pxb * GLO_PITCH + 32 * s2 + 8 * kg);
#pragma unroll
      for (int i = 0; i < 2; ++i) acc[i] = __builtin_amdgcn_mfma_f32_16x16x32_f16(af[i][s2], xf, acc[i], 0, 0, 0);
    }
#pragma unroll
// ... 303 lines not shown
      conv7x7_c4_kernel<true><<<dim3(a.B * a.f_tiles * gy), 512, lds, s>>>(a, gy);
      return vipe_launch_status();
    }
  }
  const bool glds = !small && a.KH * a.KW <= 32;
  static std::atomic<uint64_t> s1{0}, s2{0}, s3{0};
  allow_lds(conv_mfma_kernel<128, 2, 2, false>, s1, 65536);
  allow_lds(conv_mfma_kernel<128, 2, 2, true>, s2, 65536);
  allow_lds(conv_mfma_glds_kernel<128, 2, 2>, s3, 65536);
  if (cp >= 128) {
    const size_t lds = 2 * (128 + BNP) * 128;
    const int gy = cp / 128;
    if (small) conv_mfma_kernel<128, 2, 2, true><<<dim3(gx, gy), 256, lds, s>>>(a);
    else if (glds) conv_mfma_glds_kernel<128, 2, 2><<<dim3(gx * gy), 256, lds, s>>>(a, gy);
    else conv_mfma_kernel<128, 2, 2, false><<<dim3(gx, gy), 256, lds, s>>>(a);
  } else if (cp == 64) {
    const size_t lds = 2 * (64 + BNP) * 128;
    if (small) return VIPE_EUNSUPPORTED;
    if (glds) conv_mfma_glds_kernel<64, 1, 4><<<dim3(gx), 256, lds, s>>>(a, 1);
    else conv_mfma_kernel<64, 1, 4, false><<<dim3(gx, 1), 256, lds, s>>>(a);
  } else {
    const size_t lds = 2 * (32 + BNP) * 128;
    if (small) return VIPE_EUNSUPPORTED;
    if (glds) conv_mfma_glds_kernel<32, 1, 4><<<dim3(gx), 256, lds, s>>>(a, 1);
    else conv_mfma_kernel<32, 1, 4, false><<<dim3(gx, 1), 256, lds, s>>>(a);
  }
  return vipe_launch_status();
}

}

extern "C" {

VIPE_EXPORT int vipe_conv2d_nhwc_f16(const void* d_x, const void* d_w_packed, const float* d_bias,
                                     const float* d_extra, void* d_y, int B, int H, int W, int Cin, int cin_total,
                                     int cin_off, int Cout, int cout_total, int cout_off, int KH, int KW, int act,
                                     void* stream) {
  VIPE_CHECK_ARG(d_x && d_w_packed && d_bias && d_y);
  VIPE_CHECK_ARG(B >= 0 && H > 0 && W > 0 && Cin > 0 && Cout > 0 && (KH & 1) && (KW & 1));
  VIPE_CHECK_ARG((Cin == 4 || Cin % 8 == 0) && cin_total % 4 == 0 && cin_off % 4 == 0 && cout_total % 4 == 0 &&
                 cout_off % 4 == 0);
  VIPE_CHECK_ARG(Cin == 4 || (cin_total % 8 == 0 && cin_off % 8 == 0));
  VIPE_CHECK_ARG(act >= 0 && act <= 3);
  ConvArgs a = {};
  a.x0 = (const half_t*)d_x; a.x0_ctot = cin_total; a.x0_coff = cin_off;
  a.x1 = a.x0; a.x1_ctot = cin_total; a.x1_coff = cin_off; a.split = Cin;
  a.w = (const half_t*)d_w_packed; a.bias = d_bias; a.extra = d_extra; a.extra_stride = Cout; a.extra_off = 0;
  a.y = (half_t*)d_y; a.y_ctot = cout_total; a.y_coff = cout_off;
  a.B = B; a.H = H; a.W = W; a.Cin = Cin; a.Cout = Cout; a.KH = KH; a.KW = KW;
  a.act = act; a.epi = EPI_PLAIN;
  return launch_conv(a, as_stream(stream));
}

VIPE_EXPORT int vipe_conv2d_fused(const void* d_x0, int x0_ctot, int x0_coff, const void* d_x1, int x1_ctot,
                                  int x1_coff, int split, const void* d_w_packed, const float* d_bias,
                                  const float* d_extra, int extra_stride, int extra_off, void* d_y, int y_ctot,
                                  int y_coff, void* d_y2, int y2_ctot, int y2_coff, const void* d_net, int net_ctot,
                                  int net_coff, const void* d_z, float* d_fout, const void* d_accinit, int ai_ctot,
                                  int ai_coff, int B, int H, int W, int Cin, int Cout, int KH, int KW, int act, int mode,
                                  void* stream) {
  VIPE_CHECK_ARG(d_x0 && d_w_packed && d_bias);
  VIPE_CHECK_ARG(!d_accinit || (ai_ctot % 4 == 0 && ai_coff % 4 == 0 && ai_coff + Cout <= ai_ctot));
  VIPE_CHECK_ARG(B >= 0 && H > 0 && W > 0 && Cin > 0 && Cout > 0 && (KH & 1) && (KW & 1));
  if (Cin == 4) {
    VIPE_CHECK_ARG(split >= Cin && x0_ctot % 4 == 0 && x0_coff % 4 == 0);
  } else {
    VIPE_CHECK_ARG(Cin % 8 == 0 && x0_ctot % 8 == 0 && x0_coff % 8 == 0);
    VIPE_CHECK_ARG(split >= Cin || (split % 64 == 0 && d_x1 && x1_ctot % 8 == 0 && x1_coff % 8 == 0));
  }
  const int ai_f32 = (mode & VIPE_CONV_ACCINIT_F32) != 0;
  mode &= ~VIPE_CONV_ACCINIT_F32;
  VIPE_CHECK_ARG(mode >= EPI_PLAIN && mode <= EPI_PARTIAL);
  if (mode == EPI_PARTIAL) VIPE_CHECK_ARG(d_fout && y_ctot % 4 == 0 && y_coff % 4 == 0 && y_coff + Cout <= y_ctot && !d_extra);
  if (mode == EPI_PLAIN) VIPE_CHECK_ARG(d_y && y_ctot % 4 == 0 && y_coff % 4 == 0);
  if (mode == EPI_GLO) VIPE_CHECK_ARG(d_net && d_fout);
  if (mode == EPI_ZR) VIPE_CHECK_ARG(d_y && d_y2 && d_net && Cout == 256);
  if (mode == EPI_Q) VIPE_CHECK_ARG(d_y && d_net && d_z && Cout == 128);
  if (mode == EPI_HEADS) VIPE_CHECK_ARG(d_fout && Cout == 4);
  if (mode == EPI_ETA) VIPE_CHECK_ARG(d_fout && Cout == 1);
  ConvArgs a = {};
  a.x0 = (const half_t*)d_x0; a.x0_ctot = x0_ctot; a.x0_coff = x0_coff;
  a.x1 = (const half_t*)(d_x1 ? d_x1 : d_x0); a.x1_ctot = d_x1 ? x1_ctot : x0_ctot; a.x1_coff = d_x1 ? x1_coff : x0_coff;
  a.split = split > Cin ? Cin : split;
  a.w = (const half_t*)d_w_packed; a.bias = d_bias; a.extra = d_extra; a.extra_stride = extra_stride; a.extra_off = extra_off;
  a.y = (half_t*)d_y; a.y_ctot = y_ctot; a.y_coff = y_coff;
  a.y2 = (half_t*)d_y2; a.y2_ctot = y2_ctot; a.y2_coff = y2_coff;
  a.net = (const half_t*)d_net; a.net_ctot = net_ctot; a.net_coff = net_coff;
  a.zbuf = (const half_t*)d_z; a.fout = d_fout;
  a.accinit = (const half_t*)d_accinit; a.ai_ctot = ai_ctot; a.ai_coff = ai_coff; a.ai_f32 = ai_f32;
  a.B = B; a.H = H; a.W = W; a.Cin = Cin; a.Cout = Cout; a.KH = KH; a.KW = KW;
  a.act = act; a.epi = mode;
  return launch_conv(a, as_stream(stream));
}

}
```

vipe_amd/csrc/update_op.hip:

```cpp
#include "common.cuh"

namespace {

__global__ __launch_bounds__(384) void glo_gemm_kernel(const float* __restrict__ glo, const float* __restrict__ wT ,
                                                       const float* __restrict__ b, float* __restrict__ extra, float inv_hw) {
  __shared__ float g[128];
  const int e = blockIdx.x, t = threadIdx.x;
  if (t < 128) g[t] = glo[(int64_t)e * 128 + t] * inv_hw;
  __syncthreads();
  float acc = b[t];
#pragma unroll 8
  for (int k = 0; k < 128; ++k) acc = __builtin_fmaf(g[k], wT[k * 384 + t], acc);
  extra[(int64_t)e * 384 + t] = acc;
}

__global__ __launch_bounds__(256) void update_finish_kernel(const float* __restrict__ coords1, const float* __restrict__ dw,
                                                            const unsigned char* __restrict__ mask, float* __restrict__ target,
                                                            float* __restrict__ weight, const float* __restrict__ eta,
                                                            const int64_t* __restrict__ du, float* __restrict__ damping,
                                                            int64_t n_px, int64_t n_eta, int P) {
  const int64_t i = (int64_t)blockIdx.x * 256 + threadIdx.x;
  if (i < n_px) {
    const float2 c = reinterpret_cast<const float2*>(coords1)[i];
    const float4 d = reinterpret_cast<const float4*>(dw)[i];
    const bool m = mask && mask[i];
    reinterpret_cast<float2*>(target)[i] = make_float2(c.x + d.x, c.y + d.y);
    reinterpret_cast<float2*>(weight)[i] = m ? make_float2(0.f, 0.f) : make_float2(d.z, d.w);
  }
  if (i < n_eta) damping[du[i / P] * P + i % P] = eta[i];
}

}

namespace {
hipEvent_t* operator_events() {
  static thread_local hipEvent_t ev[64][4] = {};
  int d = 0;
  (void)hipGetDevice(&d);
  hipEvent_t* e = ev[d & 63];
  for (int i = 0; i < 4; ++i)
    if (!e[i] && hipEventCreateWithFlags(&e[i], hipEventDisableTiming) != hipSuccess) return nullptr;
  return e;
}
}

extern "C" {

VIPE_EXPORT int vipe_update_operator(const vipe_update_weights* wt, const vipe_update_buffers* b, void* stream) {
  VIPE_CHECK_ARG(wt && b && b->E >= 0 && b->H > 0 && b->W > 0);
  if (b->E == 0) return VIPE_OK;
  const int E = b->E, H = b->H, W = b->W;
  hipStream_t s = as_stream(stream);
  int rc;
#define RUN(call)              \
  do {                         \
    rc = (call);               \
    if (rc != VIPE_OK) return rc; \
  } while (0)
  hipStream_t s2 = (hipStream_t)b->side_stream;
  hipEvent_t* ev = s2 ? operator_events() : nullptr;
  if (s2 && !ev) return VIPE_EINVAL;
  void* const stream2 = s2 ? b->side_stream : stream;
#define FORK(i)                                                                                              \
  do {                                                                                                       \
    if (s2 && (hipEventRecord(ev[i], s) != hipSuccess || hipStreamWaitEvent(s2, ev[i], 0) != hipSuccess)) return VIPE_EINVAL; \
  } while (0)
#define JOIN(i)                                                                                              \
  do {                                                                                                       \
    if (s2 && (hipEventRecord(ev[i], s2) != hipSuccess || hipStreamWaitEvent(s, ev[i], 0) != hipSuccess)) return VIPE_EINVAL; \
  } while (0)
  FORK(0);
  if (b->levels[0]) {
    RUN(vipe_corr_lookup_conv1x1(b->levels, b->coords, wt->corr0_w, wt->corr0_b, b->c1, 128, 0, E, H, W, b->h2, b->w2, 128,
                                 VIPE_ACT_RELU, b->slots, b->pyramid_layout, stream));
  } else {
    VIPE_CHECK_ARG(b->corr);
    RUN(vipe_conv2d_fused(b->corr, 200, 0, nullptr, 0, 0, 200, wt->corr0_w, wt->corr0_b, nullptr, 0, 0, b->c1, 128, 0, nullptr,
                          0, 0, nullptr, 0, 0, nullptr, nullptr, nullptr, 0, 0, E, H, W, 200, 128, 1, 1, VIPE_ACT_RELU, 0, stream));
  }
  RUN(vipe_conv2d_fused(b->c1, 128, 0, nullptr, 0, 0, 128, wt->corr2_w, wt->corr2_b, nullptr, 0, 0, b->xbuf, 320, 128, nullptr,
                        0, 0, nullptr, 0, 0, nullptr, nullptr, nullptr, 0, 0, E, H, W, 128, 128, 3, 3, VIPE_ACT_RELU, 0, stream));
  RUN(vipe_conv2d_fused(b->motn, 4, 0, nullptr, 0, 0, 4, wt->flow0_w, wt->flow0_b, nullptr, 0, 0, b->f1, 128, 0, nullptr, 0, 0,
                        nullptr, 0, 0, nullptr, nullptr, nullptr, 0, 0, E, H, W, 4, 128, 7, 7, VIPE_ACT_RELU, 0, stream2));
  RUN(vipe_conv2d_fused(b->f1, 128, 0, nullptr, 0, 0, 128, wt->flow2_w, wt->flow2_b, nullptr, 0, 0, b->xbuf, 320, 256, nullptr,
                        0, 0, nullptr, 0, 0, nullptr, nullptr, nullptr, 0, 0, E, H, W, 128, 64, 3, 3, VIPE_ACT_RELU, 0, stream2));
  JOIN(1);
  const int Es = b->gate_state;
  const bool staged = Es != 0;
  if (staged) VIPE_CHECK_ARG(Es > 0 && Es <= E && b->pgate && b->pzr && wt->zr_x_w);
  if (!staged) {
    if (hipMemsetAsync(b->glo, 0, sizeof(float) * 128 * (size_t)E, s) != hipSuccess) return VIPE_EINVAL;
    RUN(vipe_conv2d_fused(b->net, 128, 0, nullptr, 0, 0, 128, wt->gw_w, wt->gw_b, nullptr, 0, 0, nullptr, 0, 0, nullptr, 0, 0,
                          b->net, 128, 0, nullptr, b->glo, nullptr, 0, 0, E, H, W, 128, 128, 1, 1, VIPE_ACT_NONE, 1, stream));
    glo_gemm_kernel<<<E, 384, 0, s>>>(b->glo, wt->glo_wT, wt->glo_b, b->extra, 1.0f / (float)(H * W));
  }
  if (staged) {
    RUN(vipe_conv2d_fused(b->xbuf, 320, 128, nullptr, 0, 0, 192, wt->zr_x_w, wt->zr_b, b->extra, 384, 0, b->zb, 128, 0, b->rnet,
                          128, 0, b->net, 128, 0, nullptr, nullptr, b->pzr, 256, 0, Es, H, W, 192, 256, 3, 3, VIPE_ACT_NONE,
                          2 | VIPE_CONV_ACCINIT_F32, stream));
    if (Es < E) {
      const int64_t px = (int64_t)Es * H * W;
      auto h16 = [&](const void* p, int c) { return (const void*)((const char*)p + px * c * 2); };
      RUN(vipe_conv2d_fused(h16(b->net, 128), 128, 0, h16(b->xbuf, 320), 320, 128, 128, wt->zr_s_w, wt->zr_b,
                            b->extra + (int64_t)Es * 384, 384, 0, (void*)h16(b->zb, 128), 128, 0, (void*)h16(b->rnet, 128), 128, 0,
                            h16(b->net, 128), 128, 0, nullptr, nullptr, h16(b->pgate, 384), 384, 0, E - Es, H, W, 320, 256, 3, 3,
                            VIPE_ACT_NONE, 2, stream));
    }
    RUN(vipe_conv2d_fused(b->rnet, 128, 0, b->xbuf, 320, 128, 128, wt->q_s_w, wt->q_b, b->extra, 384, 256, b->net_out, 128, 0,
                          nullptr, 0, 0, b->net, 128, 0, b->zb, nullptr, b->pgate, 384, 256, E, H, W, 320, 128, 3, 3,
                          VIPE_ACT_NONE, 3, stream));
  } else if (b->pgate) {
    RUN(vipe_conv2d_fused(b->net, 128, 0, b->xbuf, 320, 128, 128, wt->zr_s_w, wt->zr_b, b->extra, 384, 0, b->zb, 128, 0, b->rnet,
                          128, 0, b->net, 128, 0, nullptr, nullptr, b->pgate, 384, 0, E, H, W, 320, 256, 3, 3, VIPE_ACT_NONE, 2,
                          stream));
    RUN(vipe_conv2d_fused(b->rnet, 128, 0, b->xbuf, 320, 128, 128, wt->q_s_w, wt->q_b, b->extra, 384, 256, b->net_out, 128, 0,
                          nullptr, 0, 0, b->net, 128, 0, b->zb, nullptr, b->pgate, 384, 256, E, H, W, 320, 128, 3, 3,
                          VIPE_ACT_NONE, 3, stream));
  } else {
    RUN(vipe_conv2d_fused(b->net, 128, 0, b->xbuf, 320, 0, 128, wt->zr_w, wt->zr_b, b->extra, 384, 0, b->zb, 128, 0, b->rnet, 128,
                          0, b->net, 128, 0, nullptr, nullptr, nullptr, 0, 0, E, H, W, 448, 256, 3, 3, VIPE_ACT_NONE, 2, stream));
    RUN(vipe_conv2d_fused(b->rnet, 128, 0, b->xbuf, 320, 0, 128, wt->q_w, wt->q_b, b->extra, 384, 256, b->net_out, 128, 0, nullptr,
                          0, 0, b->net, 128, 0, b->zb, nullptr, nullptr, 0, 0, E, H, W, 448, 128, 3, 3, VIPE_ACT_NONE, 3, stream));
  }
  RUN(vipe_conv2d_fused(b->net_out, 128, 0, nullptr, 0, 0, 128, wt->heads0_w, wt->heads0_b, nullptr, 0, 0, b->hbuf, 384, 0,
                        nullptr, 0, 0, nullptr, 0, 0, nullptr, nullptr, nullptr, 0, 0, E, H, W, 128, 384, 3, 3, VIPE_ACT_RELU, 0,
                        stream));
  const bool two_tails = s2 && b->n_src > 0;
  if (two_tails) FORK(2);
  RUN(vipe_conv2d_fused(b->hbuf, 384, 0, nullptr, 0, 0, 256, wt->heads2_w, wt->heads2_b, nullptr, 0, 0, nullptr, 0, 0, nullptr, 0,
                        0, nullptr, 0, 0, nullptr, b->dw, nullptr, 0, 0, E, H, W, 256, 4, 3, 3, VIPE_ACT_NONE, 4,
                        two_tails ? stream2 : stream));
  if (b->n_src > 0) {
    VIPE_CHECK_ARG(b->order && b->rowptr && b->agg && b->a2 && b->eta);
    RUN(vipe_segment_mean_nhwc_f16(b->hbuf, 384, 256, b->order, b->rowptr, b->agg, b->n_src, (int64_t)H * W, 128, stream));
    RUN(vipe_conv2d_fused(b->agg, 128, 0, nullptr, 0, 0, 128, wt->agg2_w, wt->agg2_b, nullptr, 0, 0, b->a2, 128, 0, nullptr, 0, 0,
                          nullptr, 0, 0, nullptr, nullptr, nullptr, 0, 0, b->n_src, H, W, 128, 128, 3, 3, VIPE_ACT_RELU, 0,
                          stream));
    RUN(vipe_conv2d_fused(b->a2, 128, 0, nullptr, 0, 0, 128, wt->eta_w, wt->eta_b, nullptr, 0, 0, nullptr, 0, 0, nullptr, 0, 0,
                          nullptr, 0, 0, nullptr, b->eta, nullptr, 0, 0, b->n_src, H, W, 128, 1, 3, 3, VIPE_ACT_NONE, 5, stream));
  }
  if (two_tails) JOIN(3);
#undef FORK
#undef JOIN
#undef RUN
  return vipe_launch_status();
}

VIPE_EXPORT int vipe_update_gate_state(const vipe_update_weights* wt, const vipe_update_buffers* b, const void* d_net,
                                       int parts, void* stream) {
  VIPE_CHECK_ARG(wt && b && b->E >= 0 && b->H > 0 && b->W > 0 && parts >= 1 && parts <= 3);
  if (b->E == 0) return VIPE_OK;
  VIPE_CHECK_ARG(d_net && (!(parts & 1) || (b->glo && b->extra)) && (!(parts & 2) || (b->pgate && b->pzr && wt->zr_n_w)));
  const int E = b->E, H = b->H, W = b->W;
  hipStream_t s = as_stream(stream);
  int rc;
  if (parts & 1) {
    if (hipMemsetAsync(b->glo, 0, sizeof(float) * 128 * (size_t)E, s) != hipSuccess) return VIPE_EINVAL;
    rc = vipe_conv2d_fused(d_net, 128, 0, nullptr, 0, 0, 128, wt->gw_w, wt->gw_b, nullptr, 0, 0, nullptr, 0, 0, nullptr, 0, 0,
                           d_net, 128, 0, nullptr, b->glo, nullptr, 0, 0, E, H, W, 128, 128, 1, 1, VIPE_ACT_NONE, 1, stream);
    if (rc != VIPE_OK) return rc;
    glo_gemm_kernel<<<E, 384, 0, s>>>(b->glo, wt->glo_wT, wt->glo_b, b->extra, 1.0f / (float)(H * W));
  }
  if (parts & 2) {
    rc = vipe_conv2d_fused(d_net, 128, 0, nullptr, 0, 0, 128, wt->zr_n_w, wt->zr_b, nullptr, 0, 0, nullptr, 256, 0, nullptr, 0,
                           0, nullptr, 0, 0, nullptr, b->pzr, b->pgate, 384, 0, E, H, W, 128, 256, 3, 3, VIPE_ACT_NONE,
                           VIPE_CONV_PARTIAL, stream);
    if (rc != VIPE_OK) return rc;
  }
  return vipe_launch_status();
}

VIPE_EXPORT int vipe_update_gate_state_piece(void* user, int piece, int n_pieces, void* stream) {
  const vipe_gate_state_job* j = (const vipe_gate_state_job*)user;
  VIPE_CHECK_ARG(j && j->weights && j->buffers && j->net && n_pieces > 0 && piece >= 0 && piece < n_pieces);
  const vipe_update_buffers* b = j->buffers;
  VIPE_CHECK_ARG(b->E >= 0 && b->H > 0 && b->W > 0 && b->pgate && b->pzr);
  int64_t e0 = (int64_t)b->E * piece / n_pieces, e1 = (int64_t)b->E * (piece + 1) / n_pieces;
  if (j->bounds && j->n_bounds == n_pieces + 1) {
    e0 = j->bounds[piece];
    e1 = j->bounds[piece + 1];
    VIPE_CHECK_ARG(j->bounds[0] == 0 && j->bounds[n_pieces] == b->E && e0 >= 0 && e0 <= e1 && e1 <= b->E);
  }
  if (e1 <= e0) return VIPE_OK;
  const int64_t px = (int64_t)b->H * b->W;
  vipe_update_buffers sub = *b;
  sub.E = (int)(e1 - e0);
  sub.pgate = (const char*)b->pgate + e0 * px * 384 * 2;
  sub.pzr = b->pzr + e0 * px * 256;
  return vipe_update_gate_state(j->weights, &sub, (const char*)j->net + e0 * px * 128 * 2, 2, stream);
}

VIPE_EXPORT int vipe_glo_context(const float* d_glo_sum, const float* d_wT, const float* d_bias, float* d_extra, int E, int hw,
                                 void* stream) {
  VIPE_CHECK_ARG(E >= 0 && hw > 0);
  if (E == 0) return VIPE_OK;
  VIPE_CHECK_ARG(d_glo_sum && d_wT && d_bias && d_extra);
  glo_gemm_kernel<<<E, 384, 0, as_stream(stream)>>>(d_glo_sum, d_wT, d_bias, d_extra, 1.0f / (float)hw);
  return vipe_launch_status();
}

VIPE_EXPORT int vipe_update_finish(const float* d_coords1, const float* d_dw, const unsigned char* d_mask, float* d_target,
                                   float* d_weight, const float* d_eta, const int64_t* d_du, float* d_damping, int E,
                                   int n_src, int ht, int wd, void* stream) {
  VIPE_CHECK_ARG(E >= 0 && n_src >= 0 && ht > 0 && wd > 0);
  if (E == 0) return VIPE_OK;
  VIPE_CHECK_ARG(d_coords1 && d_dw && d_target && d_weight && (n_src == 0 || (d_eta && d_du && d_damping)));
  const int P = ht * wd;
  const int64_t n_px = (int64_t)E * P, n_eta = (int64_t)n_src * P;
  const int64_t n = n_px > n_eta ? n_px : n_eta;
  update_finish_kernel<<<(unsigned)((n + 255) / 256), 256, 0, as_stream(stream)>>>(d_coords1, d_dw, d_mask, d_target, d_weight,
                                                                                  d_eta, d_du, d_damping, n_px, n_eta, P);
  return vipe_launch_status();
}

// ... 2 lines not shown
```

vipe_amd/ext/slam_ext.py:

```python

import ctypes

import torch

from .._lib import CAMERA_CODE, BAParams, check, check_gpu_contig, lib, ptr, require, stream_ptr

_WS = {}


def _workspace(device, nbytes):
    key = (device.type, device.index)
    ws = _WS.get(key)
    if ws is None or ws.numel() < nbytes:
        ws = torch.empty(int(nbytes * 1.25) + 1024, dtype=torch.uint8, device=device)
        _WS[key] = ws
    return ws


def _i64(t):
    require(t.dtype == torch.int64, "index tensors must be int64")
    return t


def reproject(poses, disps, intrinsics, rig, pi, qi, pj, qj, di, camera="pinhole", intr_factor=8.0, want_valid=True):
    check_gpu_contig(poses, disps, intrinsics, rig, pi, qi, pj, qj, di)
    M = pi.shape[0]
    _, ht, wd = disps.shape
    coords = torch.empty((M, ht, wd, 2), dtype=torch.float32, device=poses.device)
    valid = torch.empty((M, ht, wd, 1), dtype=torch.float32, device=poses.device) if want_valid else None
    check(lib().vipe_reproject(ptr(poses), ptr(disps), ptr(intrinsics), ptr(rig), ptr(_i64(pi)), ptr(_i64(qi)),
                               ptr(_i64(pj)), ptr(_i64(qj)), ptr(_i64(di)), ptr(coords), ptr(valid), M, ht, wd,
                               rig.shape[0], CAMERA_CODE[camera], float(intr_factor), stream_ptr(poses)), "reproject")
    return coords, valid


def reproject_motion(poses, disps, intrinsics, rig, pi, qi, pj, qj, di, target, camera="pinhole", intr_factor=8.0,
                     motn_dtype=torch.float16):
    check_gpu_contig(poses, disps, intrinsics, rig, pi, qi, pj, qj, di, target)
    M = pi.shape[0]
    _, ht, wd = disps.shape
    require(target.numel() == M * ht * wd * 2 and target.dtype == torch.float32, "target must be [M,ht,wd,2] float32")
    coords = torch.empty((M, ht, wd, 2), dtype=torch.float32, device=poses.device)
    motn = torch.empty((M, 4, ht, wd), dtype=motn_dtype, device=poses.device)
    code = {torch.float16: 0, torch.float32: 1}[motn_dtype]
    check(lib().vipe_reproject_motion(ptr(poses), ptr(disps), ptr(intrinsics), ptr(rig), ptr(_i64(pi)), ptr(_i64(qi)),
                                      ptr(_i64(pj)), ptr(_i64(qj)), ptr(_i64(di)), ptr(target), ptr(coords), ptr(motn),
                                      M, ht, wd, rig.shape[0], CAMERA_CODE[camera], float(intr_factor), code,
                                      stream_ptr(poses)), "reproject_motion")
    return coords, motn


def reproject_motion_nhwc(poses, disps, intrinsics, rig, pi, qi, pj, qj, di, target, camera="pinhole", intr_factor=8.0,
                          out=None):
    check_gpu_contig(poses, disps, intrinsics, rig, pi, qi, pj, qj, di, target)
    M = pi.shape[0]
    _, ht, wd = disps.shape
    require(target.numel() == M * ht * wd * 2 and target.dtype == torch.float32, "target must be [M,ht,wd,2] float32")
    if out is not None:
        coords, motn = out
        require(tuple(coords.shape) == (M, ht, wd, 2) and coords.dtype == torch.float32 and coords.is_contiguous()
                and tuple(motn.shape) == (M, ht, wd, 4) and motn.dtype == torch.float16 and motn.is_contiguous(), "bad out buffers")
    else:
        coords = torch.empty((M, ht, wd, 2), dtype=torch.float32, device=poses.device)
        motn = torch.empty((M, ht, wd, 4), dtype=torch.float16, device=poses.device)
    check(lib().vipe_reproject_motion_nhwc(ptr(poses), ptr(disps), ptr(intrinsics), ptr(rig), ptr(_i64(pi)),
                                           ptr(_i64(qi)), ptr(_i64(pj)), ptr(_i64(qj)), ptr(_i64(di)), ptr(target),
                                           ptr(coords), ptr(motn), M, ht, wd, rig.shape[0], CAMERA_CODE[camera],
                                           float(intr_factor), stream_ptr(poses)), "reproject_motion_nhwc")
    return coords, motn


def update_finish(coords1, dw, mask, target, weight, eta, du, damping):
    E, ht, wd, _ = coords1.shape
    n_src = 0 if eta is None else int(eta.shape[0])
    require(target.is_contiguous() and weight.is_contiguous() and target.numel() == E * ht * wd * 2, "target / weight: contiguous [1,E,h,w,2]")
    check(lib().vipe_update_finish(ptr(coords1), ptr(dw), ptr(mask), ptr(target), ptr(weight), ptr(eta), ptr(du), ptr(damping),
                                   E, n_src, ht, wd, stream_ptr(coords1)), "update_finish")


BA_OPT_ONE_CHAIN, BA_OPT_GENERAL_ACCUMULATE = 1, 2
PROFILE_EVENTS = None
PLAN_REUSE = True


def dense_ba(poses, disps, disps_sens, intrinsics, rig, target, weight, disp_damping, pi, qi, pj, qj, di, t0, t1,
             n_iters, pose_damping, pose_ep, motion_only=False, limited_disp=False, optimize_intrinsics=False,
             optimize_rig_rotation=False, camera="pinhole", alpha=0.001, n_poses=None, want_info=False, state=None,
             plan_key=None, overlap=None, solver_options=0, profile_events=None):
    check_gpu_contig(poses, disps, disps_sens, intrinsics, rig, target, weight, disp_damping, pi, qi, pj, qj, di)
    for t in (poses, disps, disps_sens, intrinsics, rig, target, weight, disp_damping):
        require(t.dtype == torch.float32, "dense_ba works in float32 (the reference's BA dtype)")
    V = rig.shape[0]
    n_poses = poses.shape[0] if n_poses is None else int(n_poses)
    require(disps.dim() == 3 and disps.shape[0] >= n_poses * V, "disps must be [n_poses*V,ht,wd]")
    _, ht, wd = disps.shape
    M = pi.shape[0]
    require(target.numel() == M * ht * wd * 2 and weight.numel() == M * ht * wd * 2, "target/weight must be [M,P,2]")
    p = BAParams(n_poses=n_poses, n_views=V, ht=ht, wd=wd, M=M, t0=int(t0), t1=int(t1), n_iters=int(n_iters),
                 pose_damping=float(pose_damping), pose_ep=float(pose_ep), motion_only=int(motion_only),
                 limited_disp=int(limited_disp), optimize_intrinsics=int(optimize_intrinsics),
                 optimize_rig_rotation=int(optimize_rig_rotation), camera=CAMERA_CODE[camera], alpha=float(alpha),
                 weight_scale=0.001, intr_factor=8.0, reuse_plan=0, path_hint=0, solver_options=int(solver_options))
    if overlap is not None:
        p.overlap_stream, p.overlap_fn, p.overlap_user = overlap
    if profile_events is None:
        profile_events = PROFILE_EVENTS
    if profile_events is not None:
        p.profile_ev0, p.profile_ev1 = (int(e.cuda_event) for e in profile_events[:2])
        p.profile_iter = int(profile_events[2]) if len(profile_events) > 2 else -1
    L = lib()
    nbytes = L.vipe_dense_ba_workspace_bytes(ctypes.byref(p))
    require(nbytes > 0, "bad BA parameters")
    ws, key = _plan_workspace(p, nbytes, state, plan_key, camera, (pi, qi, pj, qj, di), poses.device,
                              launches=M > 0 and int(n_iters) > 0)
    learn = state is not None and key is not None and p.path_hint == 0 and "pending" not in state and M > 0 and n_iters > 0 \
        and not torch.cuda.is_current_stream_capturing() and PLAN_REUSE
    info = torch.zeros(8, dtype=torch.int32, device=poses.device) if (want_info or learn) else None
    check(L.vipe_dense_ba(ctypes.byref(p), ptr(poses), ptr(disps), ptr(disps_sens), ptr(intrinsics), ptr(rig),
                          ptr(target), ptr(weight), ptr(disp_damping), ptr(_i64(pi)), ptr(_i64(qi)), ptr(_i64(pj)),
                          ptr(_i64(qj)), ptr(_i64(di)), ptr(ws), ws.numel(), ptr(info), stream_ptr(poses)), "dense_ba")
    if learn:
        host = torch.empty(8, dtype=torch.int32, pin_memory=True)
        host.copy_(info, non_blocking=True)
        ev = torch.cuda.Event()
        ev.record()
        state["pending"] = (key, host, ev)
    return info


def _plan_workspace(p, nbytes, state, plan_key, camera, index_arrays, device, launches):
    if state is None:
        return _workspace(device, nbytes), None
    ws = state.get("ws")
    if ws is None or ws.numel() < nbytes or ws.device != device:
        ws = torch.empty(int(nbytes * 1.25) + 1024, dtype=torch.uint8, device=device)
        state["ws"], state["key"] = ws, None
    key = None if plan_key is None else (plan_key, ws.data_ptr(), p.n_poses, p.n_views, p.ht, p.wd, p.M, p.t0, p.t1, p.motion_only,
                                         p.limited_disp, p.optimize_intrinsics, p.optimize_rig_rotation, camera,
                                         tuple(int(x.data_ptr()) for x in index_arrays))
    p.reuse_plan = int(key is not None and state.get("key") == key and PLAN_REUSE)
    state["key"] = key if launches else None
    p.path_hint = _path_hint(state, key)
    return ws, key


def dense_ba_linearize(poses, disps, disps_sens, intrinsics, rig, target, weight, disp_damping, pi, qi, pj, qj, di, t0, t1,
                       pose_damping, pose_ep, motion_only=False, limited_disp=False, optimize_intrinsics=False,
                       optimize_rig_rotation=False, camera="pinhole", alpha=0.001, n_poses=None, state=None, plan_key=None,
                       solver_options=0):
    check_gpu_contig(poses, disps, disps_sens, intrinsics, rig, target, weight, disp_damping, pi, qi, pj, qj, di)
    for t in (poses, disps, disps_sens, intrinsics, rig, target, weight, disp_damping):
        require(t.dtype == torch.float32, "dense_ba_marginals works in float32 (the reference's BA dtype)")
    V = rig.shape[0]
    n_poses = poses.shape[0] if n_poses is None else int(n_poses)
    require(disps.dim() == 3 and disps.shape[0] >= n_poses * V, "disps must be [n_poses*V,ht,wd]")
# ... 133 lines not shown
```

vipe_amd/slam/factor_graph.py:

```python

import ctypes
import os

import numpy as np
import torch

from .._lib import check, check_gpu_contig, lib, parse_struct, require, stream_ptr, upload, upload_many
from ..ext import slam_ext
from .edge_index import NAMES, EdgeIndex, as_host
from .networks import AltCorrBlock, CorrBlock, CorrPool

WORK = {"edge_updates": 0, "pyramids_built": 0}


def warm_volume_pool(device, gigabytes=None):
    if torch.device(device).type != "cuda":
        return 0
    want = float(gigabytes if gigabytes is not None else os.environ.get("VIPE_AMD_BACKEND_VOLUME_GB", "160")) * 2**30
    free, _ = torch.cuda.mem_get_info(device)
    n = int(min(want, 0.85 * free))
    if n <= 0:
        return 0
    x = torch.empty(n, dtype=torch.uint8, device=device)
    x[::1 << 21].zero_()
# ... 104 lines not shown
            check_gpu_contig(src, frames, dst)
            jobs[j].src, jobs[j].frame, jobs[j].dst = src.data_ptr(), frames.data_ptr(), dst.data_ptr()
            jobs[j].dst_row_pitch, jobs[j].dst_ctot, jobs[j].dst_coff, jobs[j].dst_row0 = P * ctot, ctot, 0, n_live
        check(lib().vipe_gather_nchw_to_nhwc_f16(ctypes.addressof(jobs), 2, k, 128, P, stream_ptr(frames)), "gather_nchw_to_nhwc")
        n = n_live + k
        return self.net[nb][:n], self.xb[self.cur][:n], self.xb[self.cur][n_live:n]

    def compact(self, keep, n_keep, net_n, extra_jobs=()):
        P = self.ht * self.wd
        nb = self.bank_of(net_n)
        jobs = []
        if n_keep:
            jobs.append((self.net[nb], self.net[1 - nb], keep, n_keep, P * 128 * 2, 0))
            jobs.append((self.xb[self.cur], self.xb[1 - self.cur], keep, n_keep, P * 320 * 2, 0, (256, 640, P)))
            if self.with_pgate:
                jobs.append((self.pg[self.cur], self.pg[1 - self.cur], keep, n_keep, P * 384 * 2, 0))
        rows_gather(jobs + list(extra_jobs))
        self.cur ^= 1
        return (self.net[1 - nb][:n_keep], self.xb[self.cur][:n_keep], self.pg[self.cur][:n_keep] if self.with_pgate else None)


def _index_property(name):
    def put(self, tensor):
        self._index.assign(name, tensor)
        if name != "age":
            self._edges_changed()

    return property(lambda self: self._index.device(name), put)


class FactorGraph:
    upsample = False
    _last_ba = None

    def __init__(self, update_module, buffer, device, max_factors=48, incremental=True, cross_view=False):
        self.update_op = update_module
        self.buffer = buffer
        self.device = device
        self.max_factors = max_factors
        self.incremental = incremental
        self.cross_view = cross_view and buffer.n_views > 1
        ht, wd = buffer.height // 8, buffer.width // 8
        self.ht, self.wd = ht, wd
        self.damping = 1e-6 * torch.ones_like(buffer.flattened_disps)
        self.target = torch.zeros([1, 0, ht, wd, 2], device=device, dtype=torch.float)
        self.weight = torch.zeros([1, 0, ht, wd, 2], device=device, dtype=torch.float)
        self.corr, self.net_n, self.xbuf = None, None, None
        self.pgate = None
        self._stores = None
        self._gate_state = None
        self._side = None
        self.gate_overlap_min_edges = int(os.environ.get("VIPE_AMD_GATE_OVERLAP_MIN_EDGES", "64"))
        self.gate_overlap_mode = "gated"
        self.gate_overlap_share = 0.5
        self.gate_overlap_fractions = [0.4, 0.4, 0.2]
        self.target_inac = torch.zeros([1, 0, ht, wd, 2], device=device, dtype=torch.float)
        self.weight_inac = torch.zeros([1, 0, ht, wd, 2], device=device, dtype=torch.float)
        self._plan = None
        self._plan_serial = 0
        self._ba_state = {}
        self._spare = None
        self._inac_cap = None

    ii, jj, age, ii_inac, jj_inac = (_index_property(n) for n in NAMES)

    @property
    def _index(self):
        index = self.__dict__.get("_edge_index")
        if index is None:
            index = self.__dict__["_edge_index"] = EdgeIndex(self.device)
        return index

    def host_edges(self):
        return dict(self._index.host)

    def _edges_changed(self):
        self._plan = None
        self._gate_state = None

    @torch.no_grad()
    def add_factors(self, ii, jj, remove=False):
        ii_h, jj_h = self._index.absent(as_host(ii), as_host(jj))
        if ii_h.shape[0] == 0:
            return
        if (self.max_factors > 0 and self._index.host["ii"].shape[0] + ii_h.shape[0] > self.max_factors and self.corr is not None
                and remove):
            ix = np.argsort(self._index.host["age"], kind="stable")
            self.rm_factors(ix >= self.max_factors - ii_h.shape[0], store=True)
        ii, jj = upload_many([ii_h, jj_h], self.device)
        pi, qi, _, pj, qj, _ = self.buffer.expand_edge_multiview(ii, jj)
        V = self.buffer.n_views
        n_live = 0 if self.net_n is None else int(self.net_n.shape[0])
        f1, f2 = (pi, pj) if V == 1 else (pi * V + qi, pj * V + qj)
        if self.incremental:
            if self.corr is None:
                self.corr = CorrPool(capacity=max(64, self.max_factors + 16))
            lo, hi = int(min(ii_h.min(), jj_h.min())), int(max(ii_h.max(), jj_h.max()))
            rng = (0, self.buffer.n_frames * V) if (self.cross_view and V > 1) else (lo * V, (hi + 1) * V)
            self.corr.add_edges(self.buffer.flattened_fmaps, f1, f2, frame_range=rng)
            WORK["pyramids_built"] += int(pi.shape[0])
            eng = self.update_op.engine(self.device)
            if self._stores is None:
                self._stores = _EdgeStores(self.ht, self.wd, self.device, eng.supports_gate_split(self.ht, self.wd))
            self.net_n, self.xbuf, xb_new = self._stores.append(self.buffer.flattened_nets, self.buffer.flattened_inps,
                                                                f1.contiguous(), self.net_n, n_live)
            if self._stores.with_pgate:
# ... 172 lines not shown
                              t0=int(max(1, ii_h.min() + 1)), t1=int(max(ii_h.max(), jj_h.max()) + 1))
        return self._plan

    def _inactive_room(self, k):
        n = self.target_inac.shape[1]
        cap = self._inac_cap
        if cap is None or cap[0].shape[1] < n + k or cap[0].data_ptr() != self.target_inac.data_ptr():
            size = max(2 * (n + k), 256)
            cap = tuple(torch.empty((1, size) + tuple(x.shape[2:]), dtype=x.dtype, device=x.device)
                        for x in (self.target_inac, self.weight_inac))
            cap[0][:, :n] = self.target_inac
            cap[1][:, :n] = self.weight_inac
            self._inac_cap = cap
        self.target_inac, self.weight_inac = cap[0][:, :n + k], cap[1][:, :n + k]
        return cap[0], cap[1], n

    def _upsample_disps(self, mask, du):
        from ..ext import droid_net_ext
        buf = self.buffer
        require(buf.disps_up is not None, "FactorGraph.upsample needs GraphBuffer(upsample_disps=True)")
        droid_net_ext.cvx_upsample(buf.flattened_disps[..., None], mask, rows=du, out=buf.flattened_disps_up[..., None])
        buf.disps_up_valid.view(-1)[du] = True

    def _shift_plan(self, plan5, base):
        pi, qi, di, pj, qj = plan5
        if self.cross_view or base <= 0:
            return (pi, qi, di, pj, qj, 0)
        V = self.buffer.n_views
        return (pi - base, qi, di - base * V, pj - base, qj, base)

    @torch.no_grad()
    def update(self, t0=None, t1=None, itrs=3, use_inactive=False, motion_only=False, fixed_motion=False,
               limited_disp=False):
        assert self.incremental and self.corr is not None and self.xbuf is not None and self.net_n is not None
        assert not (motion_only and fixed_motion)
        P = self._edge_plan()
        t0 = P["t0"] if t0 is None else t0
        t1 = P["t1"] if t1 is None else t1
        buf = self.buffer
        E_act = int(P["pi"].shape[0])
        WORK["edge_updates"] += E_act
        if "io" not in P:
            P["io"] = (torch.empty((E_act, self.ht, self.wd, 2), dtype=torch.float32, device=self.device),
                       torch.empty((E_act, self.ht, self.wd, 4), dtype=torch.float16, device=self.device))
            P["mask"] = buf.masks[P["pi"], P["qi"]].contiguous()
        if not self.weight.is_contiguous() or not self.target.is_contiguous():
            self.weight, self.target = self.weight.contiguous(), self.target.contiguous()
        coords1, motn = slam_ext.reproject_motion_nhwc(buf.poses, buf.flattened_disps, buf.intrinsics, buf.rig,
                                                       P["pi"], P["qi"], P["pj"], P["qj"], P["di"],
                                                       self.target[0], camera=buf.camera_type, out=P["io"])
        eng = self.update_op.engine(self.device)
        corr = self.corr.lookup_deferred(coords1)
        up = {"want_upmask": True} if self.upsample else {}
        self.net_n, dw, eta, upmask = eng.forward_nhwc(self.net_n, self.xbuf, corr, motn, ix=P["dix"], n_src=P["n_src"],
                                                       net_out=self._net_spare(), csr=P["csr"], pgate=self.pgate,
                                                       gate_state=self._gate_state, **up)
        self._gate_state = None
        overlap = self.pgate is not None and E_act >= self.gate_overlap_min_edges
        ba_overlap = None
        if overlap:
            main = torch.cuda.current_stream(self.device)
            if self._side is None:
                self._side = torch.cuda.Stream(device=self.device)
            self._side.wait_stream(main)
            n_staged = max(1, int(round(self.gate_overlap_share * E_act)))
            if self.gate_overlap_mode == "gated":
                with torch.cuda.stream(self._side):
                    eng.hidden_gate_state(self.net_n, self.pgate, parts=1)
                fr = self.gate_overlap_fractions if len(self.gate_overlap_fractions) == itrs else None
                gate_state, ov = eng.gate_state_job(self.net_n, self.pgate, fractions=fr, n_staged=n_staged)
                ba_overlap = ov(self._side)
            else:
                with torch.cuda.stream(self._side):
                    gate_state = eng.hidden_gate_state(self.net_n, self.pgate, n_staged=n_staged)
        slam_ext.update_finish(coords1, dw, P["mask"], self.target, self.weight, eta, P["du"], self.damping)
        if use_inactive:
            key = ("inac", t0)
            if key not in P:
                h = self._index.host
                sel_h = np.flatnonzero((h["ii_inac"] >= t0 - 3) & (h["jj_inac"] >= t0 - 3))
                ii, jj, sel_exp = upload_many([np.concatenate([h["ii_inac"][sel_h], h["ii"]]),
                                               np.concatenate([h["jj_inac"][sel_h], h["jj"]]),
                                               per_view(sel_h, buf.n_views)], self.device)
                base = int(min(h["ii"].min(), h["jj"].min(), *(h[k][sel_h].min() for k in ("ii_inac", "jj_inac") if sel_h.size)))
                plan = self._shift_plan(buf.expand_edge_multiview(ii, jj)[:5], base)
                n_sel = int(sel_exp.shape[0])
                comb = tuple(torch.empty((1, n_sel + E_act) + tuple(x.shape[2:]), dtype=x.dtype, device=x.device)
                             for x in (self.target, self.weight))
                comb[0][:, :n_sel] = self.target_inac.index_select(1, sel_exp)
                comb[1][:, :n_sel] = self.weight_inac.index_select(1, sel_exp)
                P[key] = (ii, jj, plan, comb, n_sel)
            ii, jj, plan, comb, n_sel = P[key]
            plan_key = (self._plan_serial, "inac", t0)
            if self.target.data_ptr() != comb[0][:, n_sel:].data_ptr():
                comb[0][:, n_sel:] = self.target
                comb[1][:, n_sel:] = self.weight
                self.target, self.weight = comb[0][:, n_sel:], comb[1][:, n_sel:]
            target, weight = comb
        else:
            ii, jj, target, weight = self.ii, self.jj, self.target, self.weight
            if "ba_plan" not in P:
                P["ba_plan"] = self._shift_plan((P["pi"], P["qi"], P["di"], P["pj"], P["qj"]),
                                                int(min(self._index.host["ii"].min(), self._index.host["jj"].min())))
            plan = P["ba_plan"]
            plan_key = (self._plan_serial, "act")
        E = target.shape[1]
        self._last_ba = dict(t0=t0, t1=t1 if not fixed_motion else t0, pose_damping=1e-3, pose_ep=0.1, motion_only=motion_only,
                             limited_disp=limited_disp, optimize_intrinsics=False, optimize_rig_rotation=False)
        buf.bundle_adjustment(target.view(E, -1, 2), weight.view(E, -1, 2), self.damping, ii, jj, n_iters=itrs,
                              **self._last_ba, plan=plan, ba_state=self._ba_state, plan_key=plan_key, overlap=ba_overlap)
        if self.upsample:
            self._upsample_disps(upmask, P["du"])
        if overlap:
            main.wait_stream(self._side)
            self._gate_state = gate_state
        self._index.tick()

    @torch.no_grad()
    def marginals(self, t0=None, t1=None, **flags):
        P = self._edge_plan() if int(self.ii.shape[0]) else None
        ba = dict(self._last_ba or dict(t0=P["t0"] if P else 0, t1=P["t1"] if P else 0, pose_damping=1e-3, pose_ep=0.1,
                                        motion_only=False, limited_disp=False, optimize_intrinsics=False,
                                        optimize_rig_rotation=False))
        ba.update(flags)
        ba.update({k: v for k, v in (("t0", t0), ("t1", t1)) if v is not None})
        plan = None
        if P is not None:
            if "ba_plan" not in P:
# ... 118 lines not shown
```

vipe_amd/slam/update_engine.py:

```python

import ctypes
import os

import torch

from .._lib import check, lib, parse_struct, ptr, stream_ptr

UpdateWeights = parse_struct("vipe_update_weights")
UpdateBuffers = parse_struct("vipe_update_buffers")
GateStateJob = parse_struct("vipe_gate_state_job")

ACT = {"none": 0, "relu": 1, "sigmoid": 2, "tanh": 3}
EPI = {"plain": 0, "glo": 1, "zr": 2, "q": 3, "heads": 4, "eta": 5, "partial": 6}
ACCINIT_F32 = 0x100
CORR_CH = 200


class _Packed:

    def __init__(self, w_oihw, bias, device):
        w = w_oihw.detach().to(device=device, dtype=torch.float16).contiguous()
        self.cout, self.cin, self.kh, self.kw = w.shape
        cp, cinp, kp = ctypes.c_int(), ctypes.c_int(), ctypes.c_int()
        check(lib().vipe_conv_packed_dims(self.cout, self.cin, self.kh, self.kw, ctypes.addressof(cp),
                                          ctypes.addressof(cinp), ctypes.addressof(kp)), "conv_packed_dims")
        self.packed = torch.empty(kp.value * cp.value, dtype=torch.float16, device=device)
        check(lib().vipe_conv_pack_weights(ptr(w), ptr(self.packed), self.cout, self.cin, self.kh, self.kw, 0,
                                           stream_ptr(w)), "conv_pack_weights")
        self.bias = bias.detach().to(device=device, dtype=torch.float32).contiguous()
        self.flops_per_pixel = 2.0 * self.cout * self.cin * self.kh * self.kw


def segment_csr(ix, n_src):
    order = torch.argsort(ix, stable=True).to(torch.int32).contiguous()
    counts = torch.bincount(ix, minlength=n_src)
    rowptr = torch.zeros(n_src + 1, dtype=torch.int32, device=ix.device)
    rowptr[1:] = torch.cumsum(counts, 0).to(torch.int32)
    return order, rowptr


class UpdateEngine:
    def __init__(self, module, device):
        self.device = device
        self.m = module
        self._bufs = {}
        self._op_side = None
        self.op_side_min_edges = int(os.environ.get("VIPE_AMD_OP_SIDE_MIN_EDGES", "64"))
        self._gate_gen = 0
        self._pack_all()

    def _pack_all(self):
        m, d = self.m, self.device
        f16 = torch.float16

        def wb(conv):
            return conv.weight.detach().to(d, f16), conv.bias.detach().to(d, torch.float32)

        w, b = wb(m.corr_encoder[0])
        w = torch.cat([w, torch.zeros(128, CORR_CH - 196, 1, 1, device=d, dtype=f16)], 1)
        self.corr0 = _Packed(w, b, d)
        self.corr2 = _Packed(*wb(m.corr_encoder[2]), d)
        self.flow0 = _Packed(*wb(m.flow_encoder[0]), d)
        self.flow2 = _Packed(*wb(m.flow_encoder[2]), d)
        self.gw = _Packed(*wb(m.gru.w), d)
        wz, bz = wb(m.gru.convz)
        wr, br = wb(m.gru.convr)
        self.zr = _Packed(torch.cat([wz, wr], 0), torch.cat([bz, br], 0), d)
        wq, bq = wb(m.gru.convq)
        self.q = _Packed(wq, bq, d)
        rest = list(range(0, 128)) + list(range(256, 448))
        self.zr_s = _Packed(torch.cat([wz, wr], 0)[:, rest].contiguous(), torch.cat([bz, br], 0), d)
        self.q_s = _Packed(wq[:, rest].contiguous(), bq, d)
        self.gates_inp = _Packed(torch.cat([wz, wr, wq], 0)[:, 128:256].contiguous(), torch.zeros(384, device=d), d)
        self.zr_n = _Packed(torch.cat([wz, wr], 0)[:, 0:128].contiguous(), torch.cat([bz, br], 0), d)
        self.zr_x = _Packed(torch.cat([wz, wr], 0)[:, 256:448].contiguous(), torch.cat([bz, br], 0), d)
        wd0, bd0 = wb(m.delta[0])
        ww0, bw0 = wb(m.weight[0])
        wa1, ba1 = wb(m.agg.conv1)
        self.heads0 = _Packed(torch.cat([wd0, ww0, wa1], 0), torch.cat([bd0, bw0, ba1], 0), d)
        wd2, bd2 = wb(m.delta[2])
        ww2, bw2 = wb(m.weight[2])
        h2 = torch.zeros(4, 256, 3, 3, device=d, dtype=f16)
        h2[0:2, 0:128] = wd2[:2]
        h2[2:4, 128:256] = ww2[:2]
        self.heads2 = _Packed(h2, torch.cat([bd2[:2], bw2[:2]], 0), d)
        self.agg2 = _Packed(*wb(m.agg.conv2), d)
        self.eta = _Packed(*wb(m.agg.eta[0]), d)
        self.upmask = _Packed(*wb(m.agg.upmask[0]), d)
        g = m.gru
        self.glo_w = torch.cat([g.convz_glo.weight, g.convr_glo.weight, g.convq_glo.weight], 0).detach().to(d).float() \
            .reshape(384, 128).t().contiguous()
        self.glo_b = torch.cat([g.convz_glo.bias, g.convr_glo.bias, g.convq_glo.bias], 0).detach().to(d).float()
        wd_ = UpdateWeights()
        for name, pk in dict(corr0=self.corr0, corr2=self.corr2, flow0=self.flow0, flow2=self.flow2, gw=self.gw, zr=self.zr,
                             q=self.q, heads0=self.heads0, heads2=self.heads2, agg2=self.agg2, eta=self.eta).items():
            setattr(wd_, name + "_w", pk.packed.data_ptr())
            setattr(wd_, name + "_b", pk.bias.data_ptr())
        wd_.zr_s_w, wd_.q_s_w = self.zr_s.packed.data_ptr(), self.q_s.packed.data_ptr()
        wd_.zr_n_w, wd_.zr_x_w = self.zr_n.packed.data_ptr(), self.zr_x.packed.data_ptr()
        wd_.glo_wT, wd_.glo_b = self.glo_w.data_ptr(), self.glo_b.data_ptr()
        self._wdesc = wd_
# ... 42 lines not shown
                    b.E = n
                    check(lib().vipe_update_gate_state(ctypes.addressof(self._wdesc), ctypes.addressof(b), ptr(net), part,
                                                       stream_ptr(net)), "update_gate_state")
        else:
            if parts & 1:
                glo.zero_()
                self._conv(self.gw, net, 0, E, H, W, mode="glo", net=net, fout=glo)
                check(lib().vipe_glo_context(ptr(glo), ptr(self.glo_w), ptr(self.glo_b), ptr(extra), E, H * W,
                                             stream_ptr(glo)), "glo_context")
            if parts & 2:
                self._conv(self.zr_n, net, 0, Es, H, W, mode="partial", fout=pzr, accinit=pgate, ai_coff=0)
        return dict(net_ptr=net.data_ptr(), pgate_ptr=pgate.data_ptr(), shape=tuple(net.shape), pzr=pzr, extra=extra,
                    n_staged=Es, gen=self._gate_gen)

    def gate_state_job(self, net, pgate, fractions=None, n_staged=None):
        E_all, H, W, _ = net.shape
        E = E_all if n_staged is None else max(1, min(E_all, int(n_staged)))
        self._gate_gen += 1
        glo = self._buf("glo", (E_all, 128), torch.float32)
        extra = self._buf("extra", (E_all, 384), torch.float32)
        pzr = self._buf("pzr", (E, H, W, 256), torch.float32)
        b = UpdateBuffers()
        b.E, b.H, b.W = E, H, W
        b.pgate, b.pzr, b.glo, b.extra = pgate.data_ptr(), pzr.data_ptr(), glo.data_ptr(), extra.data_ptr()
        job = GateStateJob()
        job.weights, job.buffers, job.net = ctypes.addressof(self._wdesc), ctypes.addressof(b), net.data_ptr()
        bounds = None
        if fractions:
            cum, acc = [0], 0.0
            for f in fractions[:-1]:
                acc += f
                cum.append(min(E, int(round(E * acc / sum(fractions)))))
            cum.append(E)
            bounds = (ctypes.c_int * len(cum))(*cum)
            job.bounds, job.n_bounds = ctypes.addressof(bounds), len(cum)
        fn = ctypes.cast(lib().vipe_update_gate_state_piece, ctypes.c_void_p).value
        gs = dict(net_ptr=net.data_ptr(), pgate_ptr=pgate.data_ptr(), shape=tuple(net.shape), pzr=pzr, extra=extra,
                  n_staged=E, keep=(b, job, bounds), gen=self._gate_gen)
        return gs, (lambda stream: (stream.cuda_stream, fn, ctypes.addressof(job)))

    def gate_state_matches(self, gs, net, pgate):
        return (gs is not None and pgate is not None and gs["net_ptr"] == net.data_ptr() and
                gs["pgate_ptr"] == pgate.data_ptr() and gs["shape"] == tuple(net.shape) and gs.get("gen") == self._gate_gen)

    def _buf(self, name, shape, dtype=torch.float16):
        t = self._bufs.get(name)
        if t is None or tuple(t.shape) != tuple(shape) or t.dtype != dtype:
            t = torch.empty(shape, dtype=dtype, device=self.device)
            self._bufs[name] = t
        return t

    @torch.no_grad()
    def forward_nhwc(self, net, xbuf, corr, motn, ix=None, n_src=None, net_out=None, want_upmask=False, csr=None,
                     pgate=None, native=True, gate_state=None):
        E, H, W, _ = net.shape
        if not self.gate_state_matches(gate_state, net, pgate):
            gate_state = None
        if gate_state is None:
            self._gate_gen += 1
        c1 = self._buf("c1", (E, H, W, 128))
        f1 = self._buf("f1", (E, H, W, 128))
        zb = self._buf("z", (E, H, W, 128))
        rnet = self._buf("rnet", (E, H, W, 128))
        hbuf = self._buf("h", (E, H, W, 384))
        dw = self._buf("dw", (E, H, W, 4), torch.float32)
        glo = self._buf("glo", (E, 128), torch.float32)
        if net_out is None:
            net_out = torch.empty_like(net)
        if native:
            return self._forward_native(net, xbuf, corr, motn, ix, n_src, net_out, want_upmask, csr, pgate,
                                        (c1, f1, zb, rnet, hbuf, dw, glo), gate_state)
        if isinstance(corr, tuple):
            from ..ext import droid_net_ext
            droid_net_ext.corr_lookup_conv1x1(corr[1], corr[2], self.corr0.packed, self.corr0.bias, c1, act="relu",
                                              slots=corr[3] if len(corr) > 3 else None,
                                              grid=corr[4] if len(corr) > 4 else None)
        else:
            self._conv(self.corr0, corr, 0, E, H, W, y=c1, act="relu", cin=CORR_CH)
        self._conv(self.corr2, c1, 0, E, H, W, y=xbuf, y_coff=128, act="relu")
        self._conv(self.flow0, motn, 0, E, H, W, y=f1, act="relu")
        self._conv(self.flow2, f1, 0, E, H, W, y=xbuf, y_coff=256, act="relu")
        extra = self._buf("extra", (E, 384), torch.float32)
        if gate_state is None:
            glo.zero_()
            self._conv(self.gw, net, 0, E, H, W, mode="glo", net=net, fout=glo)
            check(lib().vipe_glo_context(ptr(glo), ptr(self.glo_w), ptr(self.glo_b), ptr(extra), E, H * W, stream_ptr(glo)),
                  "glo_context")
        if gate_state is not None:
            Es = gate_state["n_staged"]
            self._conv(self.zr_x, xbuf, 128, Es, H, W, y=zb, y2=rnet, net=net, mode="zr", extra=extra,
                       accinit=gate_state["pzr"], ai_coff=0, cin=192)
            if Es < E:
                self._conv(self.zr_s, net[Es:], 0, E - Es, H, W, x1=xbuf[Es:], x1_coff=128, split=128, y=zb[Es:], y2=rnet[Es:],
                           net=net[Es:], mode="zr", extra=extra[Es:], accinit=pgate[Es:], ai_coff=0)
            self._conv(self.q_s, rnet, 0, E, H, W, x1=xbuf, x1_coff=128, split=128, y=net_out, net=net, z=zb, mode="q",
                       extra=extra, extra_off=256, accinit=pgate, ai_coff=256)
        elif pgate is not None:
            self._conv(self.zr_s, net, 0, E, H, W, x1=xbuf, x1_coff=128, split=128, y=zb, y2=rnet, net=net, mode="zr",
                       extra=extra, accinit=pgate, ai_coff=0)
            self._conv(self.q_s, rnet, 0, E, H, W, x1=xbuf, x1_coff=128, split=128, y=net_out, net=net, z=zb, mode="q",
                       extra=extra, extra_off=256, accinit=pgate, ai_coff=256)
        else:
            self._conv(self.zr, net, 0, E, H, W, x1=xbuf, split=128, y=zb, y2=rnet, net=net, mode="zr", extra=extra)
            self._conv(self.q, rnet, 0, E, H, W, x1=xbuf, split=128, y=net_out, net=net, z=zb, mode="q", extra=extra,
                       extra_off=256)
        self._conv(self.heads0, net_out, 0, E, H, W, y=hbuf, act="relu")
        self._conv(self.heads2, hbuf, 0, E, H, W, mode="heads", fout=dw, cin=256)
        eta = upmask = None
        if ix is not None:
            if n_src is None:
                n_src = int(ix.max().item()) + 1 if ix.numel() else 0
            if csr is None:
                csr = segment_csr(ix, n_src)
            order, rowptr = csr
            agg = self._buf("agg", (n_src, H, W, 128))
            check(lib().vipe_segment_mean_nhwc_f16(ptr(hbuf), 384, 256, ptr(order), ptr(rowptr), ptr(agg), n_src, H * W,
                                                   128, stream_ptr(hbuf)), "segment_mean")
            a2 = self._buf("a2", (n_src, H, W, 128))
            eta = self._buf("eta", (n_src, H, W), torch.float32)
            self._conv(self.agg2, agg, 0, n_src, H, W, y=a2, act="relu")
            self._conv(self.eta, a2, 0, n_src, H, W, mode="eta", fout=eta)
            if want_upmask:
                upmask = torch.empty((n_src, H, W, 576), dtype=torch.float16, device=self.device)
                self._conv(self.upmask, a2, 0, n_src, H, W, y=upmask)
        return net_out, dw, eta, upmask

    def _forward_native(self, net, xbuf, corr, motn, ix, n_src, net_out, want_upmask, csr, pgate, scratch,
                        gate_state=None):
        c1, f1, zb, rnet, hbuf, dw, glo = scratch
        E, H, W, _ = net.shape
        extra = self._buf("extra", (E, 384), torch.float32)
        eta = agg = a2 = order = rowptr = None
        if ix is not None:
            if n_src is None:
                n_src = int(ix.max().item()) + 1 if ix.numel() else 0
            if csr is None:
                csr = segment_csr(ix, n_src)
            order, rowptr = csr
            agg = self._buf("agg", (n_src, H, W, 128))
            a2 = self._buf("a2", (n_src, H, W, 128))
            eta = self._buf("eta", (n_src, H, W), torch.float32)
        lookup = isinstance(corr, tuple)
        tensors = (net, net_out, xbuf, motn, pgate, c1, f1, zb, rnet, hbuf, dw, glo, extra, order, rowptr, agg, a2, eta) + \
            ((tuple(corr[1]) + (corr[2],) + ((corr[3],) if len(corr) > 3 and corr[3] is not None else ())) if lookup else (corr,))
        pzr = gate_state["pzr"] if gate_state is not None else None
        two_streams = E >= self.op_side_min_edges
        if two_streams and self._op_side is None:
            self._op_side = torch.cuda.Stream(device=self.device)
        key = tuple(0 if t is None else t.data_ptr() for t in tensors) + (E, H, W, n_src or 0, two_streams,
                                                                         0 if pzr is None else pzr.data_ptr(),
                                                                         0 if pzr is None else int(gate_state["n_staged"]))
        b = self._bdesc.get(key)
        if b is None:
            if len(self._bdesc) > 16:
                self._bdesc.clear()
            b = UpdateBuffers()
            b.E, b.H, b.W, b.n_src = E, H, W, int(n_src or 0) if ix is not None else 0
            if lookup:
                lv = corr[1]
                for i in range(4):
                    b.levels[i] = lv[i].data_ptr()
                b.coords = corr[2].data_ptr()
                b.slots = corr[3].data_ptr() if len(corr) > 3 and corr[3] is not None else None
                if len(corr) > 4 and corr[4] is not None:
                    b.h2, b.w2 = int(corr[4][0]), int(corr[4][1])
                else:
                    b.h2, b.w2 = int(lv[2].shape[3]) << 2, int(lv[2].shape[4]) << 2
                b.pyramid_layout = 1 if lv[0].dim() == 7 else 0
            else:
                b.corr = corr.data_ptr()
            for name, t in dict(motn=motn, net=net, net_out=net_out, xbuf=xbuf, pgate=pgate, c1=c1, f1=f1, zb=zb, rnet=rnet,
                                hbuf=hbuf, dw=dw, glo=glo, extra=extra, order=order, rowptr=rowptr, agg=agg, a2=a2,
                                eta=eta).items():
                setattr(b, name, None if t is None else t.data_ptr())
            if pzr is not None:
                b.pzr, b.gate_state = pzr.data_ptr(), int(gate_state["n_staged"])
            if two_streams:
                b.side_stream = self._op_side.cuda_stream
            self._bdesc[key] = b
        check(lib().vipe_update_operator(ctypes.addressof(self._wdesc), ctypes.addressof(b), stream_ptr(net)),
              "update_operator")
        upmask = None
        if want_upmask and ix is not None:
            upmask = torch.empty((n_src, H, W, 576), dtype=torch.float16, device=self.device)
            self._conv(self.upmask, a2, 0, n_src, H, W, y=upmask)
        return net_out, dw, eta, upmask

    @torch.no_grad()
    def forward(self, net, inp, corr, flow=None, ix=None, skip_upmask=False, n_src=None):
        batch, num, ch, ht, wd = net.shape
        E = batch * num
        dev = net.device
        f16 = torch.float16
        net_n = net.reshape(E, 128, ht, wd).to(f16).permute(0, 2, 3, 1).contiguous()
        xbuf = torch.empty((E, ht, wd, 320), dtype=f16, device=dev)
        xbuf[..., 0:128] = inp.reshape(E, 128, ht, wd).permute(0, 2, 3, 1)
        corr_n = torch.zeros((E, ht, wd, CORR_CH), dtype=f16, device=dev)
        corr_n[..., :196] = corr.reshape(E, 196, ht, wd).permute(0, 2, 3, 1)
        if flow is None:
            motn_n = torch.zeros((E, ht, wd, 4), dtype=f16, device=dev)
        else:
            motn_n = flow.reshape(E, 4, ht, wd).to(f16).permute(0, 2, 3, 1).contiguous()
        ixd = ix.to(dev) if ix is not None else None
        pgate = self.gate_context(xbuf) if self.supports_gate_split(ht, wd) else None
        net_o, dw, eta, upmask = self.forward_nhwc(net_n, xbuf, corr_n, motn_n, ixd, n_src, want_upmask=not skip_upmask,
                                                   pgate=pgate)
        net_out = net_o.permute(0, 3, 1, 2).reshape(batch, num, 128, ht, wd)
        dwv = dw.view(batch, num, ht, wd, 4).to(f16)
        delta, weight = dwv[..., 0:2].contiguous(), dwv[..., 2:4].contiguous()
        if ix is None:
            return net_out, delta, weight
        n_src = eta.shape[0]
        if upmask is not None:
            upmask = upmask.permute(0, 3, 1, 2).reshape(batch, n_src, 576, ht, wd)
        return net_out, delta, weight, eta.clone().view(batch, n_src, ht, wd), upmask
```

Before: 264.0.

## Fuse BA glue kernels and update-finish into accumulate, retract and conv epilogues

Folds the per-frame sensor-prior sum and call-flag reset into the first accumulate launch, and folds the final disparity clamp and info copy into the last retract launch. The update_finish step (target, weight and damping writeback) moves into the conv heads and eta epilogues. An optional global-context-ahead path is added to overlap the gate state. Together these cut several small kernel launches and extra passes per update at the cost of more complex kernels, redundant per-block sensor sums, and an env flag that restores the separate path.

```diff
diff --git a/include/vipe_amd.h b/include/vipe_amd.h
--- a/include/vipe_amd.h
+++ b/include/vipe_amd.h
@@ -156,6 +156,7 @@
 } vipe_ba_params;
 #define VIPE_BA_OPT_ONE_CHAIN 1
 #define VIPE_BA_OPT_GENERAL_ACCUMULATE 2
+#define VIPE_BA_OPT_SEPARATE_GLUE 4
 
 int64_t vipe_dense_ba_workspace_bytes(const vipe_ba_params* p);
 int vipe_dense_ba(const vipe_ba_params* p, float* d_poses, float* d_disps, const float* d_disps_sens,
@@ -287,6 +288,12 @@
   void* side_stream;
   float* pzr;
   int gate_state;
+  int glo_ahead;
+  const float* coords1;
+  const unsigned char* mask;
+  float *target, *weight;
+  const int64_t* du;
+  float* damping;
 } vipe_update_buffers;
 int vipe_update_operator(const vipe_update_weights* weights, const vipe_update_buffers* buffers, void* stream);
 
diff --git a/vipe_amd/csrc/ba.hip b/vipe_amd/csrc/ba.hip
--- a/vipe_amd/csrc/ba.hip
+++ b/vipe_amd/csrc/ba.hip
@@ -78,8 +78,11 @@
       hipError_t e2 = hipMemsetAsync(a.w.Hd, 0, sizeof(double) * nmax, s);
       if (e1 != hipSuccess || e2 != hipSuccess) return (int)(e1 != hipSuccess ? e1 : e2);
     }
+    BAArgs af = a, al = a;
+    af.first_iter = a.fuse_sens && it == 0;
+    al.last_iter = a.fuse_tail && it == a.p.n_iters - 1;
     if (a.mv) {
-      launch_accumulate<CAM, F>(a, s);
+      launch_accumulate<CAM, F>(af, s);
       if (ev && hipEventRecord(ev, s) != hipSuccess) return VIPE_EINVAL;
       ba_solve_kernel<<<1, SOLVE_T, solve_lds, s>>>(a, panel_cap);
       launch_tiled_cholesky(a, s);
@@ -88,14 +91,14 @@
         if (rc != VIPE_OK) return rc;
         ++*pieces_done;
       }
-      if (!a.p.motion_only) ba_retract_kernel<0><<<dim3(tiles, a.nF), TILE, 0, s>>>(a);
+      if (!a.p.motion_only) ba_retract_kernel<0><<<dim3(tiles, a.nF), TILE, 0, s>>>(al);
       continue;
     }
     const int hint = a.force_general ? 0 : a.p.path_hint;
     const bool prof = a.p.profile_ev0 && a.p.profile_ev1 &&
                       it == (a.p.profile_iter < 0 || a.p.profile_iter >= a.p.n_iters ? a.p.n_iters - 1 : a.p.profile_iter);
     if (prof && hipEventRecord((hipEvent_t)a.p.profile_ev0, s) != hipSuccess) return VIPE_EINVAL;
-    launch_accumulate<CAM, F>(a, s);
+    launch_accumulate<CAM, F>(af, s);
     if (prof && hipEventRecord((hipEvent_t)a.p.profile_ev1, s) != hipSuccess) return VIPE_EINVAL;
     if (ev && hipEventRecord(ev, s) != hipSuccess) return VIPE_EINVAL;
     if (!(hint & 8)) ba_solve_band_kernel<<<1, 2 * BAND_T, band_lds, s>>>(a, (int)(band_lds / sizeof(double)));
@@ -109,7 +112,7 @@
       if (rc != VIPE_OK) return rc;
       ++*pieces_done;
     }
-    if (!a.p.motion_only) ba_retract_kernel<F><<<dim3(tiles, a.nF), TILE, 0, s>>>(a);
+    if (!a.p.motion_only) ba_retract_kernel<F><<<dim3(tiles, a.nF), TILE, 0, s>>>(al);
   }
   return vipe_launch_status();
 }
@@ -156,14 +159,17 @@
   a.pi = d_pi; a.qi = d_qi; a.pj = d_pj; a.qj = d_qj; a.di = d_di;
   hipStream_t s = as_stream(stream);
   int rc = VIPE_OK, pieces_done = 0;
+  a.fuse_sens = a.fuse_tail = !(p->solver_options & VIPE_BA_OPT_SEPARATE_GLUE);
+  a.info_out = d_info;
+  const bool tail_done = a.fuse_tail && p->M > 0 && p->n_iters > 0 && !p->motion_only;
   if (p->M > 0 && p->n_iters > 0) {
-    ba_sens_kernel<<<a.nF, 256, 0, s>>>(d_disps_sens, a.w.sens_sum, a.P, a.w.info);
+    if (!a.fuse_sens) ba_sens_kernel<<<a.nF, TILE, 0, s>>>(d_disps_sens, a.w.sens_sum, a.P, a.w.info);
     if (!p->reuse_plan) ba_plan_kernel<<<1, 1024, 0, s>>>(a);
     const int F = p->optimize_intrinsics ? 1 + a.D : 0;
     if (p->camera == VIPE_CAM_PINHOLE) rc = F ? run_iters<VIPE_CAM_PINHOLE, 1>(a, s, &pieces_done) : run_iters<VIPE_CAM_PINHOLE, 0>(a, s, &pieces_done);
     else rc = F ? run_iters<VIPE_CAM_MEI, 2>(a, s, &pieces_done) : run_iters<VIPE_CAM_MEI, 0>(a, s, &pieces_done);
     if (rc != VIPE_OK) return rc;
-    if (d_info) {
+    if (d_info && !tail_done) {
       hipError_t e = hipMemcpyAsync(d_info, a.w.info, 8 * sizeof(int), hipMemcpyDeviceToDevice, s);
       if (e != hipSuccess) return (int)e;
     }
@@ -176,7 +182,7 @@
     }
   }
   const int64_t nd = (int64_t)a.nF * a.P;
-  clamp_min_kernel<<<(int)std::min<int64_t>((nd + 255) / 256, 2048), 256, 0, s>>>(d_disps, nd, 1e-3f);
+  if (!tail_done) clamp_min_kernel<<<(int)std::min<int64_t>((nd + 255) / 256, 2048), 256, 0, s>>>(d_disps, nd, 1e-3f);
   return vipe_launch_status();
 }
 
@@ -201,7 +207,7 @@
   a.sens = d_disps_sens; a.target = d_target; a.weight = d_weight; a.eta = d_disp_damping;
   a.pi = d_pi; a.qi = d_qi; a.pj = d_pj; a.qj = d_qj; a.di = d_di;
   hipStream_t s = as_stream(stream);
-  ba_sens_kernel<<<a.nF, 256, 0, s>>>(d_disps_sens, a.w.sens_sum, a.P, a.w.info);
+  ba_sens_kernel<<<a.nF, TILE, 0, s>>>(d_disps_sens, a.w.sens_sum, a.P, a.w.info);
   if (!(p->reuse_plan && p->M > 0)) ba_plan_kernel<<<1, 1024, 0, s>>>(a);
   if (!(p->reuse_plan && !p->motion_only && p->M > 0)) {
     hipError_t e1 = hipMemsetAsync(a.w.S, 0, sizeof(double) * (size_t)a.w.ld * a.w.ld, s);
@@ -295,8 +301,9 @@
   a.band2 = 1;
   a.droid = 1;
   a.dz_out = d_dz;
+  a.fuse_sens = 1; a.first_iter = 0;
+  a.fuse_tail = 0; a.last_iter = 0; a.info_out = nullptr;
   if (iterations == 0 || t1 == t0) return VIPE_OK;
-  ba_sens_kernel<<<a.nF, 256, 0, s>>>(d_disps_sens, a.w.sens_sum, a.P, a.w.info);
   ba_plan_kernel<<<1, 1024, 0, s>>>(a);
   int pieces_done = 0;
   const int rc = run_iters<VIPE_CAM_PINHOLE, 0>(a, s, &pieces_done);
diff --git a/vipe_amd/csrc/ba_accumulate.inc b/vipe_amd/csrc/ba_accumulate.inc
--- a/vipe_amd/csrc/ba_accumulate.inc
+++ b/vipe_amd/csrc/ba_accumulate.inc
@@ -297,12 +297,12 @@
 }
 
 template <int NF, int F>
-__device__ __forceinline__ void store_disp_block(const BAArgs& a, int k, int flags, WalkPixel<F>& px) {
+__device__ __forceinline__ void store_disp_block(const BAArgs& a, int k, int flags, float sens_k, WalkPixel<F>& px) {
   static_assert(NF <= WalkPixel<F>::FF, "E_f rows come from px.Efr");
   const BAWs& w = a.w;
   const int P = a.P, p = px.p;
   const int64_t kp = (int64_t)k * P + p;
-  finish_disp(a, k, p, P, flags, px.d, px.C, px.wz);
+  finish_disp(a, k, p, P, flags, sens_k, px.d, px.C, px.wz);
   if (px.inb) {
     w.C[kp] = px.C;
     w.wv[kp] = px.wz;
@@ -317,6 +317,7 @@
 __global__ __launch_bounds__(TILE) __attribute__((amdgpu_waves_per_eu(3, 3))) void ba_accum_mfma_kernel(BAArgs a) {
   const vipe_ba_params& prm = a.p;
   const BAWs& w = a.w;
+  if (a.first_iter && blockIdx.x == 0 && blockIdx.y == 0 && threadIdx.x == 0) clear_call_flags(w.info);
   if (a.force_general || w.info[6] > AM_DMAX) return;
   const int k = blockIdx.y;
   const int beg = w.rowptr[k], end = w.rowptr[k + 1];
@@ -338,6 +339,7 @@
   float* accI = acc1 + AM_DMAX * 256;
   TermGeomM* tg = reinterpret_cast<TermGeomM*>(accI + 64);
 
+  const float sens_k = dfree ? sensor_prior_sum(a, k, am_smem, AM_WBUF) : 0.f;
   for (int i = tid; i < AM_ROWS * AM_SP + AM_DMAX * 256 + 64; i += TILE) accS[i] = 0.0f;
   if (tid < deg) {
     TermGeomM m;
@@ -352,7 +354,7 @@
 
   const int NR = 6 * (deg + 1) + F + 1;
   if (dfree) {
-    store_disp_block<F>(a, k, flags, px);
+    store_disp_block<F>(a, k, flags, sens_k, px);
     const float sq = px.inb ? __builtin_amdgcn_rsqf(px.C) : 0.0f;
     float ej[AM_DMAX][6];
 #pragma unroll
@@ -458,6 +460,7 @@
   constexpr int WBUF = 16 * AM_P1;
   const vipe_ba_params& prm = a.p;
   const BAWs& w = a.w;
+  if (a.first_iter && blockIdx.x == 0 && blockIdx.y == 0 && threadIdx.x == 0) clear_call_flags(w.info);
   if (!a.force_general && w.info[6] <= AM_DMAX) return;
   const int k = blockIdx.y;
   const int beg = w.rowptr[k], end = w.rowptr[k + 1];
@@ -476,6 +479,7 @@
   float* acc1 = am_smem + NWAVE * WBUF;
   float* accI = acc1 + WK_CH1 * 256;
   TermGeomM* tg = reinterpret_cast<TermGeomM*>(accI + 64);
+  const float sens_k = dfree ? sensor_prior_sum(a, k, am_smem, WBUF) : 0.f;
   if (tid < 64) accI[tid] = 0.0f;
 
   WalkPixel<F> px = walk_pixel<CAM, F>(a, k, qi);
@@ -500,7 +504,7 @@
   __syncthreads();
 
   flush_frame_blocks<F>(w, accI, si, nrow, foff);
-  if (dfree) store_disp_block<F>(a, k, flags, px);
+  if (dfree) store_disp_block<F>(a, k, flags, sens_k, px);
 }
 
 constexpr int RG_NB = 10;
@@ -522,6 +526,7 @@
   constexpr int F = CAM == VIPE_CAM_MEI ? 2 : 1;
   const vipe_ba_params& prm = a.p;
   const BAWs& w = a.w;
+  if (a.first_iter && blockIdx.x == 0 && blockIdx.y == 0 && threadIdx.x == 0) clear_call_flags(w.info);
   const int k = blockIdx.y;
   const int beg = w.rowptr[k], end = w.rowptr[k + 1];
   if (beg == end) return;
@@ -540,6 +545,7 @@
   float* acc1 = am_smem + NWAVE * WBUF;
   TermGeomR* tg = reinterpret_cast<TermGeomR*>(acc1 + WK_CH * 256);
 
+  const float sens_k = dfree ? sensor_prior_sum(a, k, am_smem, WBUF) : 0.f;
   WalkPixel<F> px = walk_pixel<CAM, F>(a, k, qi);
   const int p = px.p;
   const bool inb = px.inb;
@@ -700,7 +706,7 @@
   }
 
   if (dfree) {
-    store_disp_block<0>(a, k, flags, px);
+    store_disp_block<0>(a, k, flags, sens_k, px);
     if (inb) {
       float* et = w.Et + (int64_t)k * a.ntail * P + p;
       if (oi) {
diff --git a/vipe_amd/csrc/ba_common.cuh b/vipe_amd/csrc/ba_common.cuh
--- a/vipe_amd/csrc/ba_common.cuh
+++ b/vipe_amd/csrc/ba_common.cuh
@@ -40,6 +40,9 @@
   int band2;
   int droid;
   float* dz_out;
+  int fuse_sens, first_iter;
+  int fuse_tail, last_iter;
+  int* info_out;
 };
 
 inline size_t align_up(size_t x, size_t a = 256) { return (x + a - 1) / a * a; }
@@ -119,19 +122,42 @@
                 g.Rr.R[4] == 1.f && g.Rr.R[8] == 1.f);
   g.sj = g.merge ? -1 : a.w.pose_slot[pj];
 }
-__device__ __forceinline__ void finish_disp(const BAArgs& a, int k, int p, int P, int flags, float d, float& C, float& wz) {
+__device__ __forceinline__ void finish_disp(const BAArgs& a, int k, int p, int P, int flags, float sens_k, float d, float& C,
+                                            float& wz) {
   const int64_t kp = (int64_t)k * P + p;
   if (a.droid) {
     const float sv = a.sens[kp];
     if (sv > 0.0f) { C += a.p.alpha; wz -= a.p.alpha * (d - sv); }
     else C += a.eta[(int64_t)a.w.krow[k] * P + p];
   } else {
-    if (a.w.sens_sum[k] > 0.0f) {
+    if (sens_k > 0.0f) {
       C += a.p.alpha;
       wz -= a.p.alpha * (d - a.sens[kp]);
     }
     C += 1e-7f + (0.2f * a.eta[kp] + 1e-7f);
   }
+}
+
+__device__ __forceinline__ float frame_sens_sum(const float* __restrict__ sens, int k, int P, float* red, int stride) {
+  float s = 0.f;
+  for (int p = threadIdx.x; p < P; p += TILE) s += sens[(int64_t)k * P + p];
+  s = wave_sum(s);
+  if (lane_id() == 0) red[wave_id() * stride] = s;
+  __syncthreads();
+  const float t = red[0] + red[stride] + red[2 * stride] + red[3 * stride];
+  __syncthreads();
+  return t;
+}
+__device__ __forceinline__ float sensor_prior_sum(const BAArgs& a, int k, float* red, int stride) {
+  if (a.droid) return 0.f;
+  if (!a.first_iter) return a.w.sens_sum[k];
+  const float t = frame_sens_sum(a.sens, k, a.P, red, stride);
+  if (blockIdx.x == 0 && threadIdx.x == 0) a.w.sens_sum[k] = t;
+  return t;
+}
+__device__ __forceinline__ void clear_call_flags(int* info) {
+  info[2] = 0;
+  info[5] = 0;
 }
 
 __device__ __forceinline__ void s_add(const BAWs& w, int row, int col, double v) {
diff --git a/vipe_amd/csrc/ba_plan.inc b/vipe_amd/csrc/ba_plan.inc
--- a/vipe_amd/csrc/ba_plan.inc
+++ b/vipe_amd/csrc/ba_plan.inc
@@ -2,17 +2,10 @@
 __global__ __launch_bounds__(256) void ba_sens_kernel(const float* __restrict__ sens, float* __restrict__ out, int P,
                                                       int* __restrict__ info) {
   const int k = blockIdx.x;
-  if (k == 0 && threadIdx.x == 0) {
-    info[2] = 0;
-    info[5] = 0;
-  }
-  float s = 0.f;
-  for (int p = threadIdx.x; p < P; p += blockDim.x) s += sens[(int64_t)k * P + p];
-  s = wave_sum(s);
+  if (k == 0 && threadIdx.x == 0) clear_call_flags(info);
   __shared__ float red[NWAVE];
-  if (lane_id() == 0) red[wave_id()] = s;
-  __syncthreads();
-  if (threadIdx.x == 0) out[k] = red[0] + red[1] + red[2] + red[3];
+  const float t = frame_sens_sum(sens, k, P, red, 1);
+  if (threadIdx.x == 0) out[k] = t;
 }
 
 __device__ int block_scan_excl(int* v, int n, int* lds ) {
diff --git a/vipe_amd/csrc/ba_retract.inc b/vipe_amd/csrc/ba_retract.inc
--- a/vipe_amd/csrc/ba_retract.inc
+++ b/vipe_amd/csrc/ba_retract.inc
@@ -1,26 +1,23 @@
 
 template <int F>
-__global__ __launch_bounds__(TILE) void ba_retract_kernel(BAArgs a) {
+__device__ __forceinline__ void retract_pixel(const BAArgs& a) {
   const BAWs& w = a.w;
-  {
-    const int64_t nthr = (int64_t)gridDim.x * gridDim.y * TILE;
-    const int64_t gid = ((int64_t)blockIdx.y * gridDim.x + blockIdx.x) * TILE + threadIdx.x;
-    const int64_t ns = (int64_t)w.ld * w.ld;
-    for (int64_t i = gid; i < ns; i += nthr) w.S[i] = 0.0;
-    for (int64_t i = gid; i < (int64_t)w.ld - 1; i += nthr) w.Hd[i] = 0.0;
-  }
   const int k = blockIdx.y;
   const int flags = w.fflags[k];
-  if (!(flags & 2)) return;
   const int P = a.P, V = a.p.n_views;
   const int p = blockIdx.x * TILE + threadIdx.x;
   if (p >= P) return;
   const int64_t kp = (int64_t)k * P + p;
+  auto put = [&](float d) { a.disps[kp] = a.last_iter ? fmaxf(d, 1e-3f) : d; };
+  if (!(flags & 2)) {
+    if (a.last_iter) put(a.disps[kp]);
+    return;
+  }
   if (flags & 8) {
     float C = 0.f, wz = 0.f;
-    finish_disp(a, k, p, P, flags, a.disps[kp], C, wz);
+    finish_disp(a, k, p, P, flags, 0.f, a.disps[kp], C, wz);
     const float dz = wz / C;
-    a.disps[kp] += dz;
+    put(a.disps[kp] + dz);
     if (a.dz_out) a.dz_out[(int64_t)w.krow[k] * P + p] = dz;
     return;
   }
@@ -50,8 +47,20 @@
   }
   float dz = rhs / w.C[kp];
   if (!a.droid && dz > 10.0f) dz = 0.0f;
-  a.disps[kp] += dz;
+  put(a.disps[kp] + dz);
   if (a.dz_out) a.dz_out[(int64_t)w.krow[k] * P + p] = dz;
+}
+
+template <int F>
+__global__ __launch_bounds__(TILE) void ba_retract_kernel(BAArgs a) {
+  const BAWs& w = a.w;
+  const int64_t nthr = (int64_t)gridDim.x * gridDim.y * TILE;
+  const int64_t gid = ((int64_t)blockIdx.y * gridDim.x + blockIdx.x) * TILE + threadIdx.x;
+  const int64_t ns = (int64_t)w.ld * w.ld;
+  for (int64_t i = gid; i < ns; i += nthr) w.S[i] = 0.0;
+  for (int64_t i = gid; i < (int64_t)w.ld - 1; i += nthr) w.Hd[i] = 0.0;
+  retract_pixel<F>(a);
+  if (a.last_iter && a.info_out && gid < 8) a.info_out[gid] = w.info[gid];
 }
 
 __global__ void clamp_min_kernel(float* __restrict__ x, int64_t n, float lo) {
diff --git a/vipe_amd/csrc/common.cuh b/vipe_amd/csrc/common.cuh
--- a/vipe_amd/csrc/common.cuh
+++ b/vipe_amd/csrc/common.cuh
@@ -35,6 +35,20 @@
 
 static inline hipStream_t as_stream(void* s) { return (hipStream_t)s; }
 
+struct vipe_conv_tail {
+  const float* coords1;
+  const unsigned char* mask;
+  float *target, *weight;
+  const int64_t* du;
+  float* damping;
+};
+int vipe_conv2d_fused_tail(const void* d_x0, int x0_ctot, int x0_coff, const void* d_x1, int x1_ctot, int x1_coff, int split,
+                           const void* d_w_packed, const float* d_bias, const float* d_extra, int extra_stride,
+                           int extra_off, void* d_y, int y_ctot, int y_coff, void* d_y2, int y2_ctot, int y2_coff,
+                           const void* d_net, int net_ctot, int net_coff, const void* d_z, float* d_fout,
+                           const void* d_accinit, int ai_ctot, int ai_coff, int B, int H, int W, int Cin, int Cout, int KH,
+                           int KW, int act, int mode, const vipe_conv_tail* tail, void* stream);
+
 constexpr int WAVE = 64;
 
 template <typename T>
diff --git a/vipe_amd/csrc/conv_epilogue.inc b/vipe_amd/csrc/conv_epilogue.inc
--- a/vipe_amd/csrc/conv_epilogue.inc
+++ b/vipe_amd/csrc/conv_epilogue.inc
@@ -79,18 +79,9 @@
             *reinterpret_cast<half4*>(a.y + m * a.y_ctot + a.y_coff + co) = o;
           }
         } else if (a.epi == EPI_HEADS) {
-          if (mok && co == 0) {
-            float4 o = make_float4((float)(half_t)v[0], (float)(half_t)v[1],
-                                   (float)(half_t)act_apply(v[2], VIPE_ACT_SIGMOID),
-                                   (float)(half_t)act_apply(v[3], VIPE_ACT_SIGMOID));
-            *reinterpret_cast<float4*>(a.fout + m * 4) = o;
-          }
+          if (mok && co == 0) store_heads(a, m, v[0], v[1], v[2], v[3]);
         } else if (a.epi == EPI_ETA) {
-          if (mok && co == 0) {
-            const float x = v[0];
-            const float sp = x > 20.0f ? x : log1pf(__expf(x));
-            a.fout[m] = 0.01f * (float)(half_t)sp;
-          }
+          if (mok && co == 0) store_eta(a, m, e, v[0]);
         }
       }
     }
diff --git a/vipe_amd/csrc/conv_mfma.hip b/vipe_amd/csrc/conv_mfma.hip
--- a/vipe_amd/csrc/conv_mfma.hip
+++ b/vipe_amd/csrc/conv_mfma.hip
@@ -32,6 +32,8 @@
   int ai_f32;
   int f_wp, f_hwp, f_tiles, f_pieces, f_xbytes, f_p1lo, f_p1hi;
   unsigned f_magic;
+  const float* coords1; const unsigned char* mask; float* target; float* weight;
+  const int64_t* du; float* damping;
 };
 
 constexpr int BNP = 128;
@@ -45,6 +47,28 @@
     case VIPE_ACT_SIGMOID: return 1.0f / (1.0f + __expf(-v));
     case VIPE_ACT_TANH: return tanhf(v);
     default: return v;
+  }
+}
+
+__device__ __forceinline__ void store_heads(const ConvArgs& a, int64_t m, float v0, float v1, float v2, float v3) {
+  const float4 o = make_float4((float)(half_t)v0, (float)(half_t)v1, (float)(half_t)act_apply(v2, VIPE_ACT_SIGMOID),
+                               (float)(half_t)act_apply(v3, VIPE_ACT_SIGMOID));
+  *reinterpret_cast<float4*>(a.fout + m * 4) = o;
+  if (a.target) {
+    const float2 c = reinterpret_cast<const float2*>(a.coords1)[m];
+    const bool msk = a.mask && a.mask[m];
+    reinterpret_cast<float2*>(a.target)[m] = make_float2(c.x + o.x, c.y + o.y);
+    reinterpret_cast<float2*>(a.weight)[m] = msk ? make_float2(0.f, 0.f) : make_float2(o.z, o.w);
+  }
+}
+
+__device__ __forceinline__ void store_eta(const ConvArgs& a, int64_t m, int e, float x) {
+  const float sp = x > 20.0f ? x : log1pf(__expf(x));
+  const float o = 0.01f * (float)(half_t)sp;
+  a.fout[m] = o;
+  if (a.damping) {
+    const int64_t hw = (int64_t)a.H * a.W;
+    a.damping[a.du[e] * hw + (m - e * hw)] = o;
   }
 }
 
@@ -738,15 +762,9 @@
       const float v[8] = {v0.x + bv[0], v0.y + bv[1], v0.z + bv[2], v0.w + bv[3],
                           v1.x + bv[4], v1.y + bv[5], v1.z + bv[6], v1.w + bv[7]};
       if (a.epi == EPI_HEADS) {
-        if (ch == 0)
-          *reinterpret_cast<float4*>(a.fout + m * 4) =
-              make_float4((float)(half_t)v[0], (float)(half_t)v[1], (float)(half_t)act_apply(v[2], VIPE_ACT_SIGMOID),
-                          (float)(half_t)act_apply(v[3], VIPE_ACT_SIGMOID));
+        if (ch == 0) store_heads(a, m, v[0], v[1], v[2], v[3]);
       } else if (a.epi == EPI_ETA) {
-        if (ch == 0) {
-          const float sp = v[0] > 20.0f ? v[0] : log1pf(__expf(v[0]));
-          a.fout[m] = 0.01f * (float)(half_t)sp;
-        }
+        if (ch == 0) store_eta(a, m, e, v[0]);
       } else {
         half_t* dst = a.y + m * a.y_ctot + a.y_coff + co;
         half8 o;
@@ -870,12 +888,9 @@
       if (a.extra && q < a.Cout) v[q] += a.extra[(int64_t)e * a.extra_stride + a.extra_off + q];
     }
     if (a.epi == EPI_HEADS) {
-      *reinterpret_cast<float4*>(a.fout + m * 4) =
-          make_float4((float)(half_t)v[0], (float)(half_t)v[1], (float)(half_t)act_apply(v[2], VIPE_ACT_SIGMOID),
-                      (float)(half_t)act_apply(v[3], VIPE_ACT_SIGMOID));
+      store_heads(a, m, v[0], v[1], v[2], v[3]);
     } else if (a.epi == EPI_ETA) {
-      const float sp = v[0] > 20.0f ? v[0] : log1pf(__expf(v[0]));
-      a.fout[m] = 0.01f * (float)(half_t)sp;
+      store_eta(a, m, e, v[0]);
     } else {
       half_t* dst = a.y + m * a.y_ctot + a.y_coff;
       for (int q = 0; q < a.Cout; ++q) dst[q] = (half_t)act_apply(v[q], a.act);
@@ -1285,13 +1300,14 @@
   return launch_conv(a, as_stream(stream));
 }
 
-VIPE_EXPORT int vipe_conv2d_fused(const void* d_x0, int x0_ctot, int x0_coff, const void* d_x1, int x1_ctot,
-                                  int x1_coff, int split, const void* d_w_packed, const float* d_bias,
-                                  const float* d_extra, int extra_stride, int extra_off, void* d_y, int y_ctot,
-                                  int y_coff, void* d_y2, int y2_ctot, int y2_coff, const void* d_net, int net_ctot,
-                                  int net_coff, const void* d_z, float* d_fout, const void* d_accinit, int ai_ctot,
-                                  int ai_coff, int B, int H, int W, int Cin, int Cout, int KH, int KW, int act, int mode,
-                                  void* stream) {
+}
+
+int vipe_conv2d_fused_tail(const void* d_x0, int x0_ctot, int x0_coff, const void* d_x1, int x1_ctot, int x1_coff, int split,
+                           const void* d_w_packed, const float* d_bias, const float* d_extra, int extra_stride,
+                           int extra_off, void* d_y, int y_ctot, int y_coff, void* d_y2, int y2_ctot, int y2_coff,
+                           const void* d_net, int net_ctot, int net_coff, const void* d_z, float* d_fout,
+                           const void* d_accinit, int ai_ctot, int ai_coff, int B, int H, int W, int Cin, int Cout, int KH,
+                           int KW, int act, int mode, const vipe_conv_tail* tail, void* stream) {
   VIPE_CHECK_ARG(d_x0 && d_w_packed && d_bias);
   VIPE_CHECK_ARG(!d_accinit || (ai_ctot % 4 == 0 && ai_coff % 4 == 0 && ai_coff + Cout <= ai_ctot));
   VIPE_CHECK_ARG(B >= 0 && H > 0 && W > 0 && Cin > 0 && Cout > 0 && (KH & 1) && (KW & 1));
@@ -1323,7 +1339,26 @@
   a.accinit = (const half_t*)d_accinit; a.ai_ctot = ai_ctot; a.ai_coff = ai_coff; a.ai_f32 = ai_f32;
   a.B = B; a.H = H; a.W = W; a.Cin = Cin; a.Cout = Cout; a.KH = KH; a.KW = KW;
   a.act = act; a.epi = mode;
+  if (tail && mode == EPI_HEADS && tail->target) {
+    VIPE_CHECK_ARG(tail->coords1 && tail->weight);
+    a.coords1 = tail->coords1; a.mask = tail->mask; a.target = tail->target; a.weight = tail->weight;
+  }
+  if (tail && mode == EPI_ETA && tail->damping) {
+    VIPE_CHECK_ARG(tail->du);
+    a.du = tail->du; a.damping = tail->damping;
+  }
   return launch_conv(a, as_stream(stream));
 }
 
-}
+VIPE_EXPORT int vipe_conv2d_fused(const void* d_x0, int x0_ctot, int x0_coff, const void* d_x1, int x1_ctot,
+                                  int x1_coff, int split, const void* d_w_packed, const float* d_bias,
+                                  const float* d_extra, int extra_stride, int extra_off, void* d_y, int y_ctot,
+                                  int y_coff, void* d_y2, int y2_ctot, int y2_coff, const void* d_net, int net_ctot,
+                                  int net_coff, const void* d_z, float* d_fout, const void* d_accinit, int ai_ctot,
+                                  int ai_coff, int B, int H, int W, int Cin, int Cout, int KH, int KW, int act, int mode,
+                                  void* stream) {
+  return vipe_conv2d_fused_tail(d_x0, x0_ctot, x0_coff, d_x1, x1_ctot, x1_coff, split, d_w_packed, d_bias, d_extra,
+                                extra_stride, extra_off, d_y, y_ctot, y_coff, d_y2, y2_ctot, y2_coff, d_net, net_ctot,
+                                net_coff, d_z, d_fout, d_accinit, ai_ctot, ai_coff, B, H, W, Cin, Cout, KH, KW, act, mode,
+                                nullptr, stream);
+}
diff --git a/vipe_amd/csrc/update_op.hip b/vipe_amd/csrc/update_op.hip
--- a/vipe_amd/csrc/update_op.hip
+++ b/vipe_amd/csrc/update_op.hip
@@ -30,15 +30,27 @@
   if (i < n_eta) damping[du[i / P] * P + i % P] = eta[i];
 }
 
+int global_context(const vipe_update_weights* wt, const vipe_update_buffers* b, const void* d_net, void* stream) {
+  const int E = b->E, H = b->H, W = b->W;
+  hipStream_t s = as_stream(stream);
+  if (hipMemsetAsync(b->glo, 0, sizeof(float) * 128 * (size_t)E, s) != hipSuccess) return VIPE_EINVAL;
+  const int rc = vipe_conv2d_fused(d_net, 128, 0, nullptr, 0, 0, 128, wt->gw_w, wt->gw_b, nullptr, 0, 0, nullptr, 0, 0, nullptr, 0,
+                                   0, d_net, 128, 0, nullptr, b->glo, nullptr, 0, 0, E, H, W, 128, 128, 1, 1, VIPE_ACT_NONE, 1,
+                                   stream);
+  if (rc != VIPE_OK) return rc;
+  glo_gemm_kernel<<<E, 384, 0, s>>>(b->glo, wt->glo_wT, wt->glo_b, b->extra, 1.0f / (float)(H * W));
+  return VIPE_OK;
+}
+
 }
 
 namespace {
 hipEvent_t* operator_events() {
-  static thread_local hipEvent_t ev[64][4] = {};
+  static thread_local hipEvent_t ev[64][5] = {};
   int d = 0;
   (void)hipGetDevice(&d);
   hipEvent_t* e = ev[d & 63];
-  for (int i = 0; i < 4; ++i)
+  for (int i = 0; i < 5; ++i)
     if (!e[i] && hipEventCreateWithFlags(&e[i], hipEventDisableTiming) != hipSuccess) return nullptr;
   return e;
 }
@@ -88,12 +100,7 @@
   const int Es = b->gate_state;
   const bool staged = Es != 0;
   if (staged) VIPE_CHECK_ARG(Es > 0 && Es <= E && b->pgate && b->pzr && wt->zr_x_w);
-  if (!staged) {
-    if (hipMemsetAsync(b->glo, 0, sizeof(float) * 128 * (size_t)E, s) != hipSuccess) return VIPE_EINVAL;
-    RUN(vipe_conv2d_fused(b->net, 128, 0, nullptr, 0, 0, 128, wt->gw_w, wt->gw_b, nullptr, 0, 0, nullptr, 0, 0, nullptr, 0, 0,
-                          b->net, 128, 0, nullptr, b->glo, nullptr, 0, 0, E, H, W, 128, 128, 1, 1, VIPE_ACT_NONE, 1, stream));
-    glo_gemm_kernel<<<E, 384, 0, s>>>(b->glo, wt->glo_wT, wt->glo_b, b->extra, 1.0f / (float)(H * W));
-  }
+  if (!staged) RUN(global_context(wt, b, b->net, stream));
   if (staged) {
     RUN(vipe_conv2d_fused(b->xbuf, 320, 128, nullptr, 0, 0, 192, wt->zr_x_w, wt->zr_b, b->extra, 384, 0, b->zb, 128, 0, b->rnet,
                           128, 0, b->net, 128, 0, nullptr, nullptr, b->pzr, 256, 0, Es, H, W, 192, 256, 3, 3, VIPE_ACT_NONE,
@@ -122,24 +129,31 @@
     RUN(vipe_conv2d_fused(b->rnet, 128, 0, b->xbuf, 320, 0, 128, wt->q_w, wt->q_b, b->extra, 384, 256, b->net_out, 128, 0, nullptr,
                           0, 0, b->net, 128, 0, b->zb, nullptr, nullptr, 0, 0, E, H, W, 448, 128, 3, 3, VIPE_ACT_NONE, 3, stream));
   }
+  const bool ahead = s2 && b->glo_ahead;
+  if (ahead) {
+    FORK(4);
+    RUN(global_context(wt, b, b->net_out, stream2));
+  }
   RUN(vipe_conv2d_fused(b->net_out, 128, 0, nullptr, 0, 0, 128, wt->heads0_w, wt->heads0_b, nullptr, 0, 0, b->hbuf, 384, 0,
                         nullptr, 0, 0, nullptr, 0, 0, nullptr, nullptr, nullptr, 0, 0, E, H, W, 128, 384, 3, 3, VIPE_ACT_RELU, 0,
                         stream));
   const bool two_tails = s2 && b->n_src > 0;
   if (two_tails) FORK(2);
-  RUN(vipe_conv2d_fused(b->hbuf, 384, 0, nullptr, 0, 0, 256, wt->heads2_w, wt->heads2_b, nullptr, 0, 0, nullptr, 0, 0, nullptr, 0,
-                        0, nullptr, 0, 0, nullptr, b->dw, nullptr, 0, 0, E, H, W, 256, 4, 3, 3, VIPE_ACT_NONE, 4,
-                        two_tails ? stream2 : stream));
+  const vipe_conv_tail tail = {b->coords1, b->mask, b->target, b->weight, b->du, b->damping};
+  RUN(vipe_conv2d_fused_tail(b->hbuf, 384, 0, nullptr, 0, 0, 256, wt->heads2_w, wt->heads2_b, nullptr, 0, 0, nullptr, 0, 0,
+                             nullptr, 0, 0, nullptr, 0, 0, nullptr, b->dw, nullptr, 0, 0, E, H, W, 256, 4, 3, 3, VIPE_ACT_NONE, 4,
+                             &tail, two_tails ? stream2 : stream));
   if (b->n_src > 0) {
     VIPE_CHECK_ARG(b->order && b->rowptr && b->agg && b->a2 && b->eta);
     RUN(vipe_segment_mean_nhwc_f16(b->hbuf, 384, 256, b->order, b->rowptr, b->agg, b->n_src, (int64_t)H * W, 128, stream));
     RUN(vipe_conv2d_fused(b->agg, 128, 0, nullptr, 0, 0, 128, wt->agg2_w, wt->agg2_b, nullptr, 0, 0, b->a2, 128, 0, nullptr, 0, 0,
                           nullptr, 0, 0, nullptr, nullptr, nullptr, 0, 0, b->n_src, H, W, 128, 128, 3, 3, VIPE_ACT_RELU, 0,
                           stream));
-    RUN(vipe_conv2d_fused(b->a2, 128, 0, nullptr, 0, 0, 128, wt->eta_w, wt->eta_b, nullptr, 0, 0, nullptr, 0, 0, nullptr, 0, 0,
-                          nullptr, 0, 0, nullptr, b->eta, nullptr, 0, 0, b->n_src, H, W, 128, 1, 3, 3, VIPE_ACT_NONE, 5, stream));
-  }
-  if (two_tails) JOIN(3);
+    RUN(vipe_conv2d_fused_tail(b->a2, 128, 0, nullptr, 0, 0, 128, wt->eta_w, wt->eta_b, nullptr, 0, 0, nullptr, 0, 0, nullptr, 0,
+                               0, nullptr, 0, 0, nullptr, b->eta, nullptr, 0, 0, b->n_src, H, W, 128, 1, 3, 3, VIPE_ACT_NONE, 5,
+                               &tail, stream));
+  }
+  if (two_tails || ahead) JOIN(3);
 #undef FORK
 #undef JOIN
 #undef RUN
@@ -152,14 +166,10 @@
   if (b->E == 0) return VIPE_OK;
   VIPE_CHECK_ARG(d_net && (!(parts & 1) || (b->glo && b->extra)) && (!(parts & 2) || (b->pgate && b->pzr && wt->zr_n_w)));
   const int E = b->E, H = b->H, W = b->W;
-  hipStream_t s = as_stream(stream);
   int rc;
   if (parts & 1) {
-    if (hipMemsetAsync(b->glo, 0, sizeof(float) * 128 * (size_t)E, s) != hipSuccess) return VIPE_EINVAL;
-    rc = vipe_conv2d_fused(d_net, 128, 0, nullptr, 0, 0, 128, wt->gw_w, wt->gw_b, nullptr, 0, 0, nullptr, 0, 0, nullptr, 0, 0,
-                           d_net, 128, 0, nullptr, b->glo, nullptr, 0, 0, E, H, W, 128, 128, 1, 1, VIPE_ACT_NONE, 1, stream);
+    rc = global_context(wt, b, d_net, stream);
     if (rc != VIPE_OK) return rc;
-    glo_gemm_kernel<<<E, 384, 0, s>>>(b->glo, wt->glo_wT, wt->glo_b, b->extra, 1.0f / (float)(H * W));
   }
   if (parts & 2) {
     rc = vipe_conv2d_fused(d_net, 128, 0, nullptr, 0, 0, 128, wt->zr_n_w, wt->zr_b, nullptr, 0, 0, nullptr, 256, 0, nullptr, 0,
diff --git a/vipe_amd/ext/slam_ext.py b/vipe_amd/ext/slam_ext.py
--- a/vipe_amd/ext/slam_ext.py
+++ b/vipe_amd/ext/slam_ext.py
@@ -1,5 +1,6 @@
 
 import ctypes
+import os
 
 import torch
 
@@ -78,7 +79,8 @@
                                    E, n_src, ht, wd, stream_ptr(coords1)), "update_finish")
 
 
-BA_OPT_ONE_CHAIN, BA_OPT_GENERAL_ACCUMULATE = 1, 2
+BA_OPT_ONE_CHAIN, BA_OPT_GENERAL_ACCUMULATE, BA_OPT_SEPARATE_GLUE = 1, 2, 4
+SEPARATE_GLUE = os.environ.get("VIPE_AMD_SEPARATE_GLUE", "0") == "1"
 PROFILE_EVENTS = None
 PLAN_REUSE = True
 
@@ -100,7 +102,8 @@
                  pose_damping=float(pose_damping), pose_ep=float(pose_ep), motion_only=int(motion_only),
                  limited_disp=int(limited_disp), optimize_intrinsics=int(optimize_intrinsics),
                  optimize_rig_rotation=int(optimize_rig_rotation), camera=CAMERA_CODE[camera], alpha=float(alpha),
-                 weight_scale=0.001, intr_factor=8.0, reuse_plan=0, path_hint=0, solver_options=int(solver_options))
+                 weight_scale=0.001, intr_factor=8.0, reuse_plan=0, path_hint=0,
+                 solver_options=int(solver_options) | (BA_OPT_SEPARATE_GLUE if SEPARATE_GLUE else 0))
     if overlap is not None:
         p.overlap_stream, p.overlap_fn, p.overlap_user = overlap
     if profile_events is None:
diff --git a/vipe_amd/slam/factor_graph.py b/vipe_amd/slam/factor_graph.py
--- a/vipe_amd/slam/factor_graph.py
+++ b/vipe_amd/slam/factor_graph.py
@@ -180,6 +180,7 @@
         self._side = None
         self.gate_overlap_min_edges = int(os.environ.get("VIPE_AMD_GATE_OVERLAP_MIN_EDGES", "64"))
         self.gate_overlap_mode = "gated"
+        self.glo_ahead = os.environ.get("VIPE_AMD_GLO_AHEAD", "0") == "1"
         self.gate_overlap_share = 0.5
         self.gate_overlap_fractions = [0.4, 0.4, 0.2]
         self.target_inac = torch.zeros([1, 0, ht, wd, 2], device=device, dtype=torch.float)
@@ -458,11 +459,14 @@
         eng = self.update_op.engine(self.device)
         corr = self.corr.lookup_deferred(coords1)
         up = {"want_upmask": True} if self.upsample else {}
+        overlap = self.pgate is not None and E_act >= self.gate_overlap_min_edges
+        if not slam_ext.SEPARATE_GLUE:
+            up["finish"] = (coords1, P["mask"], self.target, self.weight, P["du"], self.damping)
+            up["glo_ahead"] = overlap and self.gate_overlap_mode == "gated" and self.glo_ahead
         self.net_n, dw, eta, upmask = eng.forward_nhwc(self.net_n, self.xbuf, corr, motn, ix=P["dix"], n_src=P["n_src"],
                                                        net_out=self._net_spare(), csr=P["csr"], pgate=self.pgate,
                                                        gate_state=self._gate_state, **up)
         self._gate_state = None
-        overlap = self.pgate is not None and E_act >= self.gate_overlap_min_edges
         ba_overlap = None
         if overlap:
             main = torch.cuda.current_stream(self.device)
@@ -471,15 +475,17 @@
             self._side.wait_stream(main)
             n_staged = max(1, int(round(self.gate_overlap_share * E_act)))
             if self.gate_overlap_mode == "gated":
-                with torch.cuda.stream(self._side):
-                    eng.hidden_gate_state(self.net_n, self.pgate, parts=1)
+                if not eng.last_glo_ahead:
+                    with torch.cuda.stream(self._side):
+                        eng.hidden_gate_state(self.net_n, self.pgate, parts=1)
                 fr = self.gate_overlap_fractions if len(self.gate_overlap_fractions) == itrs else None
                 gate_state, ov = eng.gate_state_job(self.net_n, self.pgate, fractions=fr, n_staged=n_staged)
                 ba_overlap = ov(self._side)
             else:
                 with torch.cuda.stream(self._side):
                     gate_state = eng.hidden_gate_state(self.net_n, self.pgate, n_staged=n_staged)
-        slam_ext.update_finish(coords1, dw, P["mask"], self.target, self.weight, eta, P["du"], self.damping)
+        if not eng.last_finish_fused:
+            slam_ext.update_finish(coords1, dw, P["mask"], self.target, self.weight, eta, P["du"], self.damping)
         if use_inactive:
             key = ("inac", t0)
             if key not in P:
diff --git a/vipe_amd/slam/update_engine.py b/vipe_amd/slam/update_engine.py
--- a/vipe_amd/slam/update_engine.py
+++ b/vipe_amd/slam/update_engine.py
@@ -47,6 +47,7 @@
         self._op_side = None
         self.op_side_min_edges = int(os.environ.get("VIPE_AMD_OP_SIDE_MIN_EDGES", "64"))
         self._gate_gen = 0
+        self.last_glo_ahead = self.last_finish_fused = False
         self._pack_all()
 
     def _pack_all(self):
@@ -195,8 +196,9 @@
 
     @torch.no_grad()
     def forward_nhwc(self, net, xbuf, corr, motn, ix=None, n_src=None, net_out=None, want_upmask=False, csr=None,
-                     pgate=None, native=True, gate_state=None):
+                     pgate=None, native=True, gate_state=None, glo_ahead=False, finish=None):
         E, H, W, _ = net.shape
+        self.last_glo_ahead = self.last_finish_fused = False
         if not self.gate_state_matches(gate_state, net, pgate):
             gate_state = None
         if gate_state is None:
@@ -212,7 +214,7 @@
             net_out = torch.empty_like(net)
         if native:
             return self._forward_native(net, xbuf, corr, motn, ix, n_src, net_out, want_upmask, csr, pgate,
-                                        (c1, f1, zb, rnet, hbuf, dw, glo), gate_state)
+                                        (c1, f1, zb, rnet, hbuf, dw, glo), gate_state, glo_ahead, finish)
         if isinstance(corr, tuple):
             from ..ext import droid_net_ext
             droid_net_ext.corr_lookup_conv1x1(corr[1], corr[2], self.corr0.packed, self.corr0.bias, c1, act="relu",
@@ -269,7 +271,7 @@
         return net_out, dw, eta, upmask
 
     def _forward_native(self, net, xbuf, corr, motn, ix, n_src, net_out, want_upmask, csr, pgate, scratch,
-                        gate_state=None):
+                        gate_state=None, glo_ahead=False, finish=None):
         c1, f1, zb, rnet, hbuf, dw, glo = scratch
         E, H, W, _ = net.shape
         extra = self._buf("extra", (E, 384), torch.float32)
@@ -290,9 +292,14 @@
         two_streams = E >= self.op_side_min_edges
         if two_streams and self._op_side is None:
             self._op_side = torch.cuda.Stream(device=self.device)
+        glo_ahead = bool(glo_ahead and two_streams)
+        if finish is not None and (ix is None or finish[4] is None or finish[5] is None):
+            finish = tuple(finish[:4]) + (None, None)
         key = tuple(0 if t is None else t.data_ptr() for t in tensors) + (E, H, W, n_src or 0, two_streams,
                                                                          0 if pzr is None else pzr.data_ptr(),
-                                                                         0 if pzr is None else int(gate_state["n_staged"]))
+                                                                         0 if pzr is None else int(gate_state["n_staged"]),
+                                                                         glo_ahead) + \
+            tuple(0 if t is None else t.data_ptr() for t in (finish or ()))
         b = self._bdesc.get(key)
         if b is None:
             if len(self._bdesc) > 16:
@@ -320,9 +327,14 @@
                 b.pzr, b.gate_state = pzr.data_ptr(), int(gate_state["n_staged"])
             if two_streams:
                 b.side_stream = self._op_side.cuda_stream
+            b.glo_ahead = int(glo_ahead)
+            if finish is not None:
+                for name, t in zip(("coords1", "mask", "target", "weight", "du", "damping"), finish):
+                    setattr(b, name, None if t is None else t.data_ptr())
             self._bdesc[key] = b
         check(lib().vipe_update_operator(ctypes.addressof(self._wdesc), ctypes.addressof(b), stream_ptr(net)),
               "update_operator")
+        self.last_glo_ahead, self.last_finish_fused = glo_ahead, finish is not None
         upmask = None
         if want_upmask and ix is not None:
             upmask = torch.empty((n_src, H, W, 576), dtype=torch.float16, device=self.device)
```

After: 263.1. About the same (-0.3%).
